# ruc98/Distributed-Data-Parallel-ML-Training

Hardware: AMD Instinct MI355X
Metric: images/sec (whole node) VGG-11 CIFAR-10 (higher is better)
Workload: dtype bf16; 1 GPU; model=vgg11, global_batch=256, per_gpu_batch=256, parallelism=dp1, hipgraph=True, buckets=1, grad_comm=fp32, comm=inline, optimizer=SGD(lr=0.1, momentum=0.9, wd=1e-4) fused

## Files before the change

distributed-data-parallel-ml-training_amd/csrc/bind.cpp:

```cpp
#include <hip/hip_runtime.h>
#include <pybind11/pybind11.h>
#include <pybind11/stl.h>

#include <stdexcept>
#include <string>
#include <tuple>
#include <vector>

#include "runtime/comm.h"

namespace py = pybind11;
using ddp_amd::BucketSpec;
using ddp_amd::RcclComm;
using ddp_amd::Reducer;

#include "kernels/api.h"

template <typename T>
static T* P(uintptr_t v) { return reinterpret_cast<T*>(v); }
static hipStream_t S(uintptr_t v) { return reinterpret_cast<hipStream_t>(v); }
static void check(int rc, const char* what) {
  if (rc != 0) {
    std::string msg = std::string(what) + " failed: ";
    msg += (rc > 0) ? hipGetErrorString((hipError_t)rc) : "invalid arguments";
// ... 200 lines not shown
  });
  m.def("conv_dgrad", [](py::tuple g, uintptr_t dy, uintptr_t wt, uintptr_t dx, uintptr_t ws,
                         size_t ws_elems, int splits, uintptr_t st, int accumulate, py::object bn,
                         py::object bna, uintptr_t acc_dy, uintptr_t acc_mask) {
    auto c = geom(g);
    if (acc_mask) {
      check(ddp_conv_dgrad_acc(&c, P<void>(dy), P<void>(wt), P<void>(dx), P<float>(ws), ws_elems,
                               splits, P<void>(acc_dy), P<unsigned char>(acc_mask), S(st)),
            "conv_dgrad_acc");
      return false;
    }
    if (bn.is_none()) {
      check(ddp_conv_dgrad(&c, P<void>(dy), P<void>(wt), P<void>(dx), P<float>(ws), ws_elems,
                           splits, accumulate, S(st)), "conv_dgrad");
      return false;
    }
    ddp_amd::BnBwdFuse f{};
    const ddp_amd::BnBwdFuse* fp = bn_fuse(bn, &f);
    ddp_amd::BnBwdApply ap{};
    const ddp_amd::BnBwdApply* app = bn_apply(bna, &ap);
    int done = 0;
    check(ddp_conv_dgrad_bn(&c, P<void>(dy), P<void>(wt), P<void>(dx), P<float>(ws), ws_elems,
                            splits, fp, app, &done, S(st)), "conv_dgrad_bn");
    return done == 1;
  }, py::arg("g"), py::arg("dy"), py::arg("wt"), py::arg("dx"), py::arg("ws"),
     py::arg("ws_elems"), py::arg("splits"), py::arg("stream"), py::arg("accumulate") = 0,
     py::arg("bn") = py::none(), py::arg("bna") = py::none(), py::arg("acc_dy") = 0,
     py::arg("acc_mask") = 0);
  m.def("conv_bwd_pair", [](py::tuple g, uintptr_t dy, uintptr_t wc, uintptr_t dx, uintptr_t x,
                            uintptr_t dw, uintptr_t ws, size_t ws_elems, uintptr_t st,
                            py::object bn, py::object bna) {
    auto c = geom(g);
    ddp_amd::BnBwdApply ap{};
    const ddp_amd::BnBwdApply* app = bn_apply(bna, &ap);
    int done = 0;
    ddp_amd::BnBwdFuse f{};
    const ddp_amd::BnBwdFuse* fp = bn_fuse(bn, &f);
    check(ddp_conv_bwd_pair(&c, P<void>(dy), P<void>(wc), P<void>(dx), P<void>(x), P<float>(dw),
                            P<float>(ws), ws_elems, fp, app, &done, S(st)), "conv_bwd_pair");
    return done;
  }, py::arg("g"), py::arg("dy"), py::arg("wc"), py::arg("dx"), py::arg("x"), py::arg("dw"),
     py::arg("ws"), py::arg("ws_elems"), py::arg("stream"), py::arg("bn") = py::none(),
     py::arg("bna") = py::none());
  m.def("sgd_fuse_register", [](uintptr_t dw, uintptr_t p, uintptr_t buf, uintptr_t wc, float lr,
                                float momentum, float wd, float grad_scale, int nesterov,
                                int clear, uintptr_t sched) {
    ddp_amd::SgdFuse f{P<float>(p), P<float>(buf), P<unsigned short>(wc), lr, momentum, wd,
                       grad_scale, nesterov, P<const ddp_amd::LrSched>(sched)};
    ddp_sgd_fuse_register(P<float>(dw), dw ? &f : nullptr, clear);
  }, py::arg("dw"), py::arg("p") = 0, py::arg("buf") = 0, py::arg("wc") = 0, py::arg("lr") = 0.f,
     py::arg("momentum") = 0.f, py::arg("wd") = 0.f, py::arg("grad_scale") = 1.f,
     py::arg("nesterov") = 0, py::arg("clear") = 0, py::arg("sched") = 0);
  m.def("sgd_fuse_begin", []() { ddp_sgd_fuse_begin(); });
  m.def("sgd_fuse_taken", []() {
    std::vector<uintptr_t> v(256);
    int n = ddp_sgd_fuse_taken(v.data(), (int)v.size());
    if (n > (int)v.size()) {
      v.resize(n);
      n = ddp_sgd_fuse_taken(v.data(), n);
    }
    v.resize(n);
    return v;
  });
  m.def("sgd_fuse_taken_master", []() {
    std::vector<uintptr_t> v(256);
    int n = ddp_sgd_fuse_taken_master(v.data(), (int)v.size());
    if (n > (int)v.size()) {
      v.resize(n);
      n = ddp_sgd_fuse_taken_master(v.data(), n);
    }
    v.resize(n);
    return v;
  });
  m.def("conv_dense2x2_set", [](int on) { ddp_conv_dense2x2_set(on); });
  m.def("conv_dense2x2_ok", [](py::tuple g) {
    auto c = geom(g);
    return ddp_conv_dense2x2_ok(&c) != 0;
  });
  m.def("conv_pair_mode", [](int mode, int items) { ddp_conv_pair_mode(mode, items); },
        py::arg("mode"), py::arg("items") = 0);
  m.def("conv_pair_force", [](int sd, int sw, int tile) { ddp_conv_pair_force(sd, sw, tile); },
        py::arg("splits_dg"), py::arg("splits_wg"), py::arg("tile") = 0);
  m.def("conv_wgrad", [](py::tuple g, uintptr_t dy, uintptr_t x, uintptr_t dw, uintptr_t ws,
                         size_t ws_elems, int splits, uintptr_t st, int final_) {
    auto c = geom(g);
    if (final_)
      check(ddp_conv_wgrad_final(&c, P<void>(dy), P<void>(x), P<float>(dw), P<float>(ws),
                                 ws_elems, splits, S(st)), "conv_wgrad");
    else
      check(ddp_conv_wgrad(&c, P<void>(dy), P<void>(x), P<float>(dw), P<float>(ws), ws_elems,
                           splits, S(st)), "conv_wgrad");
  }, py::arg("g"), py::arg("dy"), py::arg("x"), py::arg("dw"), py::arg("ws"), py::arg("ws_elems"),
     py::arg("splits"), py::arg("stream"), py::arg("final") = 0);

  m.def("bn_act_fwd", [](int N, int H, int W, int C, int pool, int relu, float eps, uintptr_t z,
                         uintptr_t res, uintptr_t stats, uintptr_t gamma, uintptr_t beta,
                         uintptr_t out, uintptr_t st, uintptr_t running_mean,
                         uintptr_t running_var, float momentum, int use_running, uintptr_t coef,
                         uintptr_t mask, uintptr_t rstats, uintptr_t rgamma, uintptr_t rbeta,
                         uintptr_t rcoef, uintptr_t rrunning_mean, uintptr_t rrunning_var,
                         float reps, float rmomentum) {
    ddp_amd::BnArgs a{};
    a.coef = P<float>(coef);
    a.mask = P<unsigned char>(mask);
    a.N = N; a.H = H; a.W = W; a.C = C; a.pool = pool; a.relu = relu; a.eps = eps;
    a.z = P<unsigned short>(z); a.res = P<unsigned short>(res); a.stats = P<float>(stats);
// ... 127 lines not shown
                         int dlogits_bf16, uintptr_t st) {
    check(ddp_softmax_ce(P<void>(logits), bf16, P<long long>(labels), B, J, P<float>(loss_sum),
                         P<int>(correct), P<void>(dlogits), dlogits_bf16, S(st)), "softmax_ce");
  });

  m.def("sgd", [](uintptr_t p, uintptr_t g, uintptr_t buf, size_t n, float lr, float momentum,
                  float wd, float grad_scale, int nesterov, uintptr_t st, uintptr_t sched) {
    check(ddp_sgd(P<float>(p), P<float>(g), P<float>(buf), n, lr, momentum, wd, grad_scale,
                  nesterov, P<const ddp_amd::LrSched>(sched), S(st)), "sgd");
  }, py::arg("p"), py::arg("g"), py::arg("buf"), py::arg("n"), py::arg("lr"), py::arg("momentum"),
     py::arg("wd"), py::arg("grad_scale"), py::arg("nesterov"), py::arg("stream"),
     py::arg("sched") = 0);
  m.def("conv_options", [](int stages) { ddp_conv_options(stages); }, py::arg("stages") = 2);
  m.def("conv_tune_set", [](int mode, int M, int N, int K, int tile, int splits, int stages) {
    ddp_conv_tune_set(mode, M, N, K, tile, splits, stages);
  }, py::arg("mode"), py::arg("M"), py::arg("N"), py::arg("K"), py::arg("tile"),
     py::arg("splits"), py::arg("stages") = 0);
  m.def("conv_tune_clear", []() { ddp_conv_tune_clear(); });
  m.def("conv_wgrad_pm_set", [](int on) { ddp_conv_wgrad_pm_set(on); });
  m.def("conv_rows_pm_set", [](int on) { ddp_conv_rows_pm_set(on); });
  m.def("bn_fold_bwd_mb", [](int mb) { ddp_bn_fold_bwd_mb(mb); });
  m.def("bn_fold_grid", [](int blocks) { ddp_bn_fold_grid(blocks); });
  m.def("conv_pair_tune_set", [](int M, int N, int K, int hw, int tile, int sd, int sw) {
    ddp_conv_pair_tune_set(M, N, K, hw, tile, sd, sw);
  });
  m.def("conv_force_tile", [](int t, int stages) { ddp_conv_force_tile(t, stages); },
        py::arg("tile_plus_one"), py::arg("stages") = 0);
#ifdef DDP_CONV_STAMPS
  m.def("conv_stamps_set", [](uintptr_t buf, int cap) { ddp_conv_stamps_set(P<void>(buf), cap); });
#endif
  m.def("pack_conv_weights", [](std::vector<std::tuple<uintptr_t, uintptr_t, uintptr_t, int, int,
                                                       int, int, int, int>> descs, uintptr_t st) {
    std::vector<ddp_amd::PackDesc> d;
    for (auto& t : descs) {
      ddp_amd::PackDesc x;
      x.p = P<float>(std::get<0>(t));
      x.wc = P<unsigned short>(std::get<1>(t));
      x.wt = P<unsigned short>(std::get<2>(t));
      x.K = std::get<3>(t); x.Cr = std::get<4>(t); x.C = std::get<5>(t);
      x.R = std::get<6>(t); x.S = std::get<7>(t);
      x.krsc = std::get<8>(t);
      d.push_back(x);
    }
    check(ddp_pack_conv_weights(d.data(), (int)d.size(), S(st)), "pack_conv_weights");
  });
  m.def("sgd_pack", [](uintptr_t items, int n_items, uintptr_t descs, uintptr_t p, uintptr_t g,
                       uintptr_t buf, float lr, float momentum, float wd, float grad_scale,
                       int nesterov, uintptr_t st, int zero_grad, uintptr_t counter, int delta,
                       uintptr_t skip, uintptr_t shadow, uintptr_t slot, uintptr_t done,
                       uintptr_t signal, uintptr_t sched, int sched_advance, uintptr_t lars_side,
                       uintptr_t lars_tensors, uintptr_t lars_partial, uintptr_t lars_trust,
                       float lars_eta, float lars_eps, uintptr_t clip_partial, int clip_chunks,
                       float clip_max_norm, float clip_eps, int clip_flags,
                       uintptr_t clip_stats) {
    check(ddp_sgd_pack(P<void>(items), n_items, P<long long>(descs), P<float>(p), P<float>(g),
                       P<float>(buf), lr, momentum, wd, grad_scale, nesterov, zero_grad,
                       P<int>(counter), delta, P<const unsigned>(skip), P<unsigned short>(shadow),
                       P<float>(slot), P<unsigned>(done), P<unsigned>(signal),
                       P<ddp_amd::LrSched>(sched), sched_advance, P<void>(lars_side),
                       P<void>(lars_tensors), P<void>(lars_partial), P<float>(lars_trust),
                       lars_eta, lars_eps, P<const float>(clip_partial), clip_chunks,
                       clip_max_norm, clip_eps, clip_flags, P<float>(clip_stats), S(st)),
          "sgd_pack");
  }, py::arg("items"), py::arg("n_items"), py::arg("descs"), py::arg("p"), py::arg("g"),
     py::arg("buf"), py::arg("lr"), py::arg("momentum"), py::arg("wd"), py::arg("grad_scale"),
     py::arg("nesterov"), py::arg("stream"), py::arg("zero_grad") = 0, py::arg("counter") = 0,
     py::arg("delta") = 0, py::arg("skip") = 0, py::arg("shadow") = 0, py::arg("slot") = 0,
     py::arg("done") = 0, py::arg("signal") = 0, py::arg("sched") = 0,
     py::arg("sched_advance") = 0, py::arg("lars_side") = 0, py::arg("lars_tensors") = 0,
     py::arg("lars_partial") = 0, py::arg("lars_trust") = 0, py::arg("lars_eta") = 0.f,
     py::arg("lars_eps") = 0.f, py::arg("clip_partial") = 0, py::arg("clip_chunks") = 0,
     py::arg("clip_max_norm") = 0.f, py::arg("clip_eps") = 0.f, py::arg("clip_flags") = 0,
     py::arg("clip_stats") = 0);
  m.def("grad_sumsq", [](uintptr_t items, int n_items, uintptr_t g, float grad_scale,
                         uintptr_t partial, uintptr_t st) {
    check(ddp_grad_sumsq(P<void>(items), n_items, P<float>(g), grad_scale, P<float>(partial),
                         S(st)), "grad_sumsq");
  }, py::arg("items"), py::arg("n_items"), py::arg("grad"), py::arg("grad_scale"),
     py::arg("partial"), py::arg("stream"));
  m.def("lars_norms", [](uintptr_t items, int n_items, uintptr_t p, uintptr_t g, float grad_scale,
                         uintptr_t partial, uintptr_t st) {
    check(ddp_lars_norms(P<void>(items), n_items, P<float>(p), P<float>(g), grad_scale,
                         P<void>(partial), S(st)), "lars_norms");
  }, py::arg("items"), py::arg("n_items"), py::arg("p"), py::arg("g"), py::arg("grad_scale"),
     py::arg("partial"), py::arg("stream"));
  m.def("shard_tail", [](uintptr_t segs, int n_segs, uintptr_t src, uintptr_t dst,
                         std::vector<std::tuple<uintptr_t, uintptr_t, uintptr_t, int, int, int,
                                                int, int, int>> descs,
                         uintptr_t done, uintptr_t signal, uintptr_t skip, uintptr_t st) {
    std::vector<ddp_amd::PackDesc> d;
    for (auto& t : descs) {
      ddp_amd::PackDesc x;
      x.p = P<float>(std::get<0>(t));
      x.wc = P<unsigned short>(std::get<1>(t));
      x.wt = P<unsigned short>(std::get<2>(t));
      x.K = std::get<3>(t); x.Cr = std::get<4>(t); x.C = std::get<5>(t);
      x.R = std::get<6>(t); x.S = std::get<7>(t);
      x.krsc = std::get<8>(t);
      d.push_back(x);
    }
    check(ddp_shard_tail(P<void>(segs), n_segs, P<float>(src), P<float>(dst), d.data(),
                         (int)d.size(), P<unsigned>(done), P<unsigned>(signal),
                         P<const unsigned>(skip), S(st)), "shard_tail");
  });
  m.def("seg_copy_f32", [](uintptr_t table, int n, uintptr_t src, uintptr_t dst, uintptr_t st) {
    check(ddp_seg_copy_f32(P<void>(table), n, P<float>(src), P<float>(dst), S(st)), "seg_copy_f32");
  });
  m.def("sgd_tile_dims", [](int RS) {
    int tk, tc;
    ddp_sgd_tile_dims(RS, &tk, &tc);
    return std::make_pair(tk, tc);
  });
  m.def("sgd_tile_limit", []() { return ddp_sgd_tile_limit(); });
  m.def("counter_add", [](uintptr_t c, int delta, uintptr_t st, uintptr_t sched, int sched_mode) {
    check(ddp_counter_add(P<int>(c), delta, P<ddp_amd::LrSched>(sched), sched_mode, S(st)),
          "counter_add");
  }, py::arg("c"), py::arg("delta"), py::arg("stream"), py::arg("sched") = 0,
     py::arg("sched_mode") = 0);

  m.def("synth_generate", [](uintptr_t images, uintptr_t labels, int n, int pix_per_img,
                             unsigned int seed, int classes, uintptr_t st) {
    check(ddp_synth_generate(P<unsigned char>(images), P<int>(labels), n, pix_per_img, seed,
                             classes, S(st)), "synth_generate");
  });
  m.def("augment", [](uintptr_t images, uintptr_t labels, uintptr_t indices, uintptr_t cursor,
                      int L, int B, int H, int W, int Cp, int pad, int flip, unsigned int seed,
// ... 173 lines not shown
```

distributed-data-parallel-ml-training_amd/csrc/kernels/api.h:

```cpp
#pragma once
#include <hip/hip_runtime.h>
#include <stddef.h>
#include <stdint.h>

namespace ddp_amd {

#ifdef DDP_AMD_DETERMINISTIC
constexpr int kStatRep = 4096;
constexpr bool kDeterministic = true;
#else
constexpr int kStatRep = 16;
constexpr bool kDeterministic = false;
#endif

struct ConvGeom {
  int N, H, W, C;
  int K;
  int R, S, stride, pad;
  int P, Q;
  int Creal;
  int wkrsc;
};

struct BnArgs {
// ... 158 lines not shown
int ddp_conv_tr_would_serve(const ddp_amd::ConvGeom* g, size_t ws_elems, int in_mode);
void ddp_conv_tr_set(int mode, int M, int K, int C, int H, int bm, int bn, int splits, int stages);
int ddp_conv_tr_geometry(int BM, int N, int H, int W, int* out7);
int ddp_linear_head_bwd_bn(const float* dl, const float* W, const void* x, int B, int F, int J,
                           const float* gscale, const ddp_amd::BnBwdFuse* bn,
                           const ddp_amd::BnBwdApply* ba, float* dW, float* db, hipStream_t st);
void ddp_conv_bn_fuse_rows(int rows);
int ddp_conv_dgrad(const ddp_amd::ConvGeom* g, const void* dy, const void* wt, void* dx,
                   float* ws, size_t ws_elems, int splits, int accumulate, hipStream_t st);
int ddp_conv_dgrad_acc(const ddp_amd::ConvGeom* g, const void* dy, const void* wt, void* dx,
                       float* ws, size_t ws_elems, int splits, const void* acc_dy,
                       const unsigned char* acc_mask, hipStream_t st);
int ddp_conv_dgrad_bn(const ddp_amd::ConvGeom* g, const void* dy, const void* wt, void* dx,
                      float* ws, size_t ws_elems, int splits, const ddp_amd::BnBwdFuse* bn,
                      const ddp_amd::BnBwdApply* ba, int* bn_done, hipStream_t st);
int ddp_conv_wgrad(const ddp_amd::ConvGeom* g, const void* dy, const void* x, float* dw,
                   float* ws, size_t ws_elems, int splits, hipStream_t st);
int ddp_bn_act_fwd(const ddp_amd::BnArgs* a, hipStream_t st);
int ddp_bn_act_bwd(const ddp_amd::BnArgs* a, hipStream_t st);
int ddp_bn_act_fwd_res(const ddp_amd::BnArgs* a, const ddp_amd::BnArgs* r, hipStream_t st);
int ddp_bn_act_bwd_res(const ddp_amd::BnArgs* a, hipStream_t st);
int ddp_bn_bwd_local_ok(int N, int H, int W, int C, int pool);
void ddp_bn_bwd_local_set(long long max_loads);
int ddp_bn_pool_linear_ce_fwd(const ddp_amd::HeadBnIn* bn, const float* W, const float* b,
                              const long long* labels, int B, int F, int J, float* dlogits,
                              float* loss_sum, int* correct, float* loss_acc, hipStream_t st);
int ddp_linear_ce_fwd(const void* x, const float* W, const float* b, const long long* labels,
                      int B, int F, int J, float* logits, float* dlogits, float* loss_sum,
                      int* correct, float* loss_acc, hipStream_t st);
int ddp_linear_bwd(const float* dlogits, const void* x, const float* W, int B, int F, int J,
                   const float* gscale, void* dx, float* dW, float* db, hipStream_t st);
int ddp_softmax_ce(const void* logits, int logits_bf16, const long long* labels, int B, int J,
                   float* loss_sum, int* correct, void* dlogits, int dlogits_bf16,
                   hipStream_t st);
int ddp_sgd(float* p, const float* g, float* buf, size_t n, float lr, float momentum, float wd,
            float grad_scale, int nesterov, const ddp_amd::LrSched* sched, hipStream_t st);
int ddp_conv_fwd_smallk(const ddp_amd::ConvGeom* g, const void* x, const void* wc,
                        const float* bias, void* y, float* stats, hipStream_t st);
void ddp_conv_options(int stages);
void ddp_conv_epi_stage_set(int on);
int ddp_bn_pool3_fwd(const ddp_amd::BnArgs* a, unsigned char* idx, hipStream_t st);
int ddp_bn_pool3_bwd(const ddp_amd::BnArgs* a, const unsigned char* idx, hipStream_t st);
void ddp_conv_pair_mode(int mode, int items);
void ddp_sgd_fuse_register(float* dw, const ddp_amd::SgdFuse* f, int clear);
void ddp_sgd_fuse_begin();
int ddp_l0_ok(const ddp_amd::ConvGeom* g);
int ddp_l0_fwd(const ddp_amd::ConvGeom* g, const ddp_amd::L0Io* io, hipStream_t st);
int ddp_l0_bwd(const ddp_amd::ConvGeom* g, const ddp_amd::L0Io* io, hipStream_t st);
int ddp_conv_wgrad_final(const ddp_amd::ConvGeom* g, const void* dy, const void* x, float* dw,
                         float* ws, size_t ws_elems, int splits, hipStream_t st);
int ddp_sgd_fuse_taken(uintptr_t* out, int cap);
int ddp_sgd_fuse_take_final(const float* dw, ddp_amd::SgdFuse* out);
int ddp_sgd_fuse_taken_master(uintptr_t* out, int cap);
void ddp_conv_pair_force(int splits_dg, int splits_wg, int tile);
int ddp_conv_bwd_pair(const ddp_amd::ConvGeom* g, const void* dy, const void* wc, void* dx,
                      const void* x, float* dw, float* ws, size_t ws_elems,
                      const ddp_amd::BnBwdFuse* bn, const ddp_amd::BnBwdApply* ba, int* bn_done,
                      hipStream_t st);
void ddp_conv_tune_set(int mode, int M, int N, int K, int tile, int splits, int stages);
void ddp_conv_pair_tune_set(int M, int N, int K, int hw, int tile, int sd, int sw);
void ddp_conv_wgrad_pm_set(int on);
void ddp_conv_rows_pm_set(int on);
void ddp_bn_fold_bwd_mb(int mb);
void ddp_bn_fold_grid(int blocks);
int ddp_conv_dense2x2_ok(const ddp_amd::ConvGeom* g);
void ddp_conv_dense2x2_set(int on);
void ddp_conv_tune_clear();
void ddp_conv_force_tile(int tile_plus_one, int stages);
#ifdef DDP_CONV_STAMPS
void ddp_conv_stamps_set(void* buf, int cap);
#endif
int ddp_pack_conv_weights(const ddp_amd::PackDesc* descs, int n, hipStream_t st);
int ddp_sgd_pack(const void* items, int n_items, const long long* descs, float* p, float* g,
                 float* buf, float lr, float momentum, float wd, float grad_scale, int nesterov,
                 int zero_grad, int* counter, int delta, const unsigned* skip,
                 unsigned short* shadow, float* slot, unsigned* done, unsigned* signal,
                 ddp_amd::LrSched* sched, int sched_advance, const void* lars_side,
                 const void* lars_tensors, const void* lars_partial, float* lars_trust,
                 float lars_eta, float lars_eps, const float* clip_partial, int clip_chunks,
                 float clip_max_norm, float clip_eps, int clip_flags, float* clip_stats,
                 hipStream_t st);
int ddp_grad_sumsq(const void* items, int n_items, const float* g, float grad_scale,
                   float* partial, hipStream_t st);
int ddp_lars_norms(const void* items, int n_items, const float* p, const float* g,
                   float grad_scale, void* partial, hipStream_t st);
int ddp_shard_tail(const void* segs, int n_segs, const float* src, float* dst,
                   const ddp_amd::PackDesc* pack, int n_pack, unsigned* done, unsigned* signal,
                   const unsigned* skip, hipStream_t st);
void ddp_sgd_tile_dims(int RS, int* TK, int* TC);
int ddp_sgd_tile_limit();
int ddp_counter_add(int* c, int delta, ddp_amd::LrSched* sched, int sched_mode, hipStream_t st);
int ddp_synth_generate(unsigned char* images, int* labels, int n, int pix_per_img,
                       unsigned int seed, int classes, hipStream_t st);
int ddp_augment(const ddp_amd::AugArgs* a, hipStream_t st);
int ddp_nchw_to_nhwc(const float* x, int N, int C, int H, int W, int Cp, void* out,
                     hipStream_t st);
int ddp_maxpool_fwd(const void* x, int N, int H, int W, int C, int KH, int KW, int stride,
                    int pad, int Ho, int Wo, void* y, void* idx, hipStream_t st);
int ddp_maxpool_bwd(const void* dy, const void* idx, int N, int H, int W, int C, int KH, int KW,
                    int stride, int pad, int Ho, int Wo, void* dx, hipStream_t st);
int ddp_avgpool_fwd(const void* x, int N, int HW, int C, void* y, hipStream_t st);
int ddp_avgpool_bwd(const void* dy, int N, int HW, int C, void* dx, hipStream_t st);
int ddp_colsum(const void* dl, int B, int J, float* db, hipStream_t st);
int ddp_mean_ws(const float* in, size_t n, int ws, float* out, hipStream_t st);
int ddp_scale(float* x, size_t n, float s, hipStream_t st);
int ddp_copy_bytes(void* dst, const void* src, size_t n, hipStream_t st);
int ddp_fill_bytes(void* dst, int value, size_t n, hipStream_t st);
int ddp_comm_standin(float* x, size_t n, int blocks, float usec, float scale, int passes,
                     hipStream_t st);
int ddp_flag_signal(unsigned* flag, hipStream_t st);
int ddp_flag_wait(const unsigned* flag, unsigned* expected, unsigned* err, float timeout_s,
                  hipStream_t st);
int ddp_pack_bf16(const float* x, size_t n, unsigned short* y, hipStream_t st);
int ddp_seg_copy_f32(const void* table, int n, const float* src, float* dst, hipStream_t st);
int ddp_unpack_bf16(const unsigned short* y, size_t n, float* x, hipStream_t st);
}
```

distributed-data-parallel-ml-training_amd/csrc/kernels/bn_act.hip:

```cpp
#include "common.h"
#include "api.h"

#include <algorithm>
#include <cstdio>
#include <cstdlib>

namespace ddp_amd {

enum { kSc = 0, kSh = 1, kMu = 2, kIs = 3, kK1 = 4, kK2 = 5 };

__device__ __forceinline__ void ld8f(const float* p, float* v) {
  const float4 a = reinterpret_cast<const float4*>(p)[0];
  const float4 b = reinterpret_cast<const float4*>(p)[1];
  v[0] = a.x; v[1] = a.y; v[2] = a.z; v[3] = a.w;
  v[4] = b.x; v[5] = b.y; v[6] = b.z; v[7] = b.w;
}

__device__ __forceinline__ void finalize_fwd_ch(const BnArgs& a, int c) {
  float mu, is;
  if (a.use_running) {
    mu = a.running_mean[c];
    is = rsqrtf(a.running_var[c] + a.eps);
  } else {
    const float M = (float)a.N * a.H * a.W;
    float s1 = 0.f, s2 = 0.f;
#pragma unroll
    for (int r = 0; r < kStatRep; ++r) {
      s1 += a.stats[r * 2 * a.C + c];
      s2 += a.stats[r * 2 * a.C + a.C + c];
    }
    mu = s1 / M;
    const float var = fmaxf(s2 / M - mu * mu, 0.f);
    is = rsqrtf(var + a.eps);
    if (a.running_mean) {
      const float unbiased = M > 1.f ? var * M / (M - 1.f) : var;
      a.running_mean[c] = (1.f - a.momentum) * a.running_mean[c] + a.momentum * mu;
      a.running_var[c] = (1.f - a.momentum) * a.running_var[c] + a.momentum * unbiased;
    }
  }
  const float sc = a.gamma[c] * is;
  a.coef[kSc * a.C + c] = sc;
  a.coef[kSh * a.C + c] = a.beta[c] - mu * sc;
  a.coef[kMu * a.C + c] = mu;
  a.coef[kIs * a.C + c] = is;
}

__global__ __launch_bounds__(256) void bn_finalize_fwd_kernel(BnArgs a) {
  const int c = blockIdx.x * blockDim.x + threadIdx.x;
  if (c < a.C) finalize_fwd_ch(a, c);
}

__global__ __launch_bounds__(256) void bn_finalize_fwd2_kernel(BnArgs a, BnArgs r) {
  const int c = blockIdx.x * blockDim.x + threadIdx.x;
  if (c < a.C) finalize_fwd_ch(blockIdx.y ? r : a, c);
// ... 182 lines not shown
    const size_t pp = L.ok[it] ? p : 0;
    L.mb[it] = 0;
    const int wo = (int)(pp % Wo);
    const int ho = (int)((pp / Wo) % Ho);
    const int n = (int)(pp / ((size_t)Wo * Ho));
    L.dv[it] = ld8(a.dout + pp * a.C + cg * 8);
#pragma unroll
    for (int d = 0; d < NP; ++d) {
      const int h = POOL ? 2 * ho + (d >> 1) : ho, w = POOL ? 2 * wo + (d & 1) : wo;
      const size_t off = (((size_t)n * a.H + h) * a.W + w) * a.C + cg * 8;
      L.off[it][d] = off;
      L.zv[it][d] = ld8(a.z + off);
      if (MASK) L.mb[it] = a.mask[off / 8];
      if (RBN || (!MASK && !POOL && a.res)) L.rv[it][POOL ? 0 : d] = ld8(a.res + off);
    }
  }
}

template <bool POOL, bool MASK = false>
__device__ __forceinline__ void bwd_compute(const BnArgs& a, const u16x8& dv, const u16x8* zv,
                                            const u16x8* rv, unsigned mb, const float* sc,
                                            const float* sh, const float* mu, const float* is,
                                            float (*xh)[8], float (*dyb)[8]) {
  constexpr int NP = POOL ? 4 : 1;
  float best[8], yv[NP][8];
  int arg[8];
#pragma unroll
  for (int e = 0; e < 8; ++e) { best[e] = -INFINITY; arg[e] = 0; }
#pragma unroll
  for (int d = 0; d < NP; ++d) {
#pragma unroll
    for (int e = 0; e < 8; ++e) {
      const float zf = bf2f(zv[d][e]);
      float y = zf * sc[e] + sh[e];
      if (!POOL && !MASK && a.res) y += bf2f(rv[POOL ? 0 : d][e]);
      xh[d][e] = (zf - mu[e]) * is[e];
      yv[d][e] = y;
      if (POOL) {
        const float yr = a.relu ? fmaxf(y, 0.f) : y;
        if (yr > best[e] || yr != yr) { best[e] = yr; arg[e] = d; }
      }
    }
  }
#pragma unroll
  for (int d = 0; d < NP; ++d)
#pragma unroll
    for (int e = 0; e < 8; ++e) {
      const float g = (!POOL || arg[e] == d) ? bf2f(dv[e]) : 0.f;
      const bool pos = MASK ? ((mb >> e) & 1u) != 0 : yv[d][e] > 0.f;
      dyb[d][e] = (a.relu && !pos) ? 0.f : g;
    }
}

template <bool POOL, int IPT, bool MASK = false, bool STRIDE = false, bool RBN = false>
__global__ __launch_bounds__(256) void bn_act_bwd_reduce_kernel(BnArgs a) {
  constexpr int NS = RBN ? 3 : 2;
  constexpr int NP = POOL ? 4 : 1;
  __shared__ float red[8 * 256];
  DDP_DEVICE_CHECK(a.C % 8 == 0 && (!POOL || (a.H % 2 == 0 && a.W % 2 == 0)));
  const int G = a.C / 8;
  const int Gb = a.red_gb ? a.red_gb : (G < 256 ? G : 256);
  const int Ho = POOL ? a.H / 2 : a.H, Wo = POOL ? a.W / 2 : a.W;
  const size_t npix = (size_t)a.N * Ho * Wo;
  const int cg_base = blockIdx.y * Gb;
  const int cgl = threadIdx.x % Gb;
  const int prow = threadIdx.x / Gb, prows = 256 / Gb;
  const int c0 = (cg_base + cgl) * 8;
  const size_t per_blk = (size_t)prows * IPT;
  const size_t nbx = STRIDE ? (npix + per_blk - 1) / per_blk : (size_t)blockIdx.x + 1;
  BwdItems<POOL, IPT> L;
  bwd_load<POOL, IPT, MASK, RBN>(a, L, (size_t)blockIdx.x * per_blk + prow, prows, npix,
                                 cg_base + cgl, Ho, Wo);
  float sc[8], sh[8], mu[8], is[8], rmu[8], ris[8];
  ld8f(a.coef + kSc * a.C + c0, sc);
  ld8f(a.coef + kSh * a.C + c0, sh);
  ld8f(a.coef + kMu * a.C + c0, mu);
  ld8f(a.coef + kIs * a.C + c0, is);
  if (RBN) {
    ld8f(a.rcoef + kMu * a.C + c0, rmu);
    ld8f(a.rcoef + kIs * a.C + c0, ris);
  }
  float acc[NS][8];
#pragma unroll
  for (int k = 0; k < NS; ++k)
#pragma unroll
    for (int e = 0; e < 8; ++e) acc[k][e] = 0.f;
  for (size_t bb = blockIdx.x;;) {
#pragma unroll
    for (int it = 0; it < IPT; ++it) {
      if (!L.ok[it]) continue;
      float xh[NP][8], dyb[NP][8];
      bwd_compute<POOL, MASK>(a, L.dv[it], L.zv[it], L.rv[it], L.mb[it], sc, sh, mu, is, xh, dyb);
#pragma unroll
      for (int d = 0; d < NP; ++d) {
#pragma unroll
        for (int e = 0; e < 8; ++e) {
          acc[0][e] += dyb[d][e];
          acc[1][e] += dyb[d][e] * xh[d][e];
          if (RBN) acc[NS - 1][e] += dyb[d][e] * ((bf2f(L.rv[it][0][e]) - rmu[e]) * ris[e]);
        }
      }
    }
    bb += gridDim.x;
    if (!STRIDE || bb >= nbx) break;
    bwd_load<POOL, IPT, MASK, RBN>(a, L, bb * per_blk + prow, prows, npix, cg_base + cgl, Ho, Wo);
  }
  float* rep = a.sums + stat_rep(blockIdx.x) * 2 * a.C;
  const int tid = threadIdx.x;
#pragma unroll
  for (int k = 0; k < NS; ++k) {
    if (k) __syncthreads();
#pragma unroll
    for (int e = 0; e < 8; ++e) red[e * 256 + tid] = acc[k][e];
    __syncthreads();
    float* dst = k < 2 ? rep + k * a.C : a.rsums + stat_rep(blockIdx.x) * 2 * a.C + a.C;
    for (int idx = tid; idx < Gb * 8; idx += 256) {
      const int g = idx / 8, e = idx % 8;
      float s = 0.f;
      for (int r = 0; r < prows; ++r) s += red[e * 256 + r * Gb + g];
      atomicAdd(dst + (cg_base + g) * 8 + e, stat_val(s, blockIdx.x));
    }
  }
}

template <bool POOL, int IPT, bool FOLD = false, bool MASK = false, bool STRIDE = false,
          bool RBN = false>
__global__ __launch_bounds__(256) void bn_act_bwd_apply_kernel(BnArgs a) {
  constexpr int NP = POOL ? 4 : 1;
  const int G = a.C / 8;
  const int Gb = G < 256 ? G : 256;
  const int Ho = POOL ? a.H / 2 : a.H, Wo = POOL ? a.W / 2 : a.W;
  const size_t npix = (size_t)a.N * Ho * Wo;
  const int cg_base = blockIdx.y * Gb;
  const int cgl = threadIdx.x % Gb;
  const int prow = threadIdx.x / Gb, prows = 256 / Gb;
  const int c0 = (cg_base + cgl) * 8;
  const size_t per_blk = (size_t)prows * IPT;
  const size_t nbx = (npix + per_blk - 1) / per_blk;
  BwdItems<POOL, IPT> L;
  bwd_load<POOL, IPT, MASK, RBN>(a, L, (size_t)blockIdx.x * per_blk + prow, prows, npix,
                                 cg_base + cgl, Ho, Wo);
  float sc[8], sh[8], mu[8], is[8], k1[8], k2[8], rsc[8], rmu[8], ris[8], rk2[8];
  if (RBN) {
    ld8f(a.rcoef + kSc * a.C + c0, rsc);
    ld8f(a.rcoef + kMu * a.C + c0, rmu);
    ld8f(a.rcoef + kIs * a.C + c0, ris);
    ld8f(a.rcoef + kK2 * a.C + c0, rk2);
  }
  ld8f(a.coef + kSc * a.C + c0, sc);
  ld8f(a.coef + kSh * a.C + c0, sh);
  ld8f(a.coef + kMu * a.C + c0, mu);
  ld8f(a.coef + kIs * a.C + c0, is);
  if (FOLD) {
    __shared__ __attribute__((aligned(16))) float kk[2][2048];
    const int nch = Gb * 8;
    const float inv_m = 1.f / ((float)a.N * a.H * a.W);
    for (int q = threadIdx.x * 4; q < 2 * nch; q += 1024) {
      const int which = q / nch, cl = q - which * nch;
      const float* src = a.sums + which * a.C + cg_base * 8 + cl;
      float4 t = *reinterpret_cast<const float4*>(src);
#pragma unroll
      for (int r = 1; r < kStatRep; ++r) {
        const float4 v = *reinterpret_cast<const float4*>(src + (size_t)r * 2 * a.C);
        t.x += v.x; t.y += v.y; t.z += v.z; t.w += v.w;
      }
      const float tv[4] = {t.x, t.y, t.z, t.w};
#pragma unroll
      for (int e = 0; e < 4; ++e) {
        kk[which][cl + e] = tv[e] * inv_m;
        if (blockIdx.x == 0) {
          const int c = cg_base * 8 + cl + e;
          a.coef[(which ? kK2 : kK1) * a.C + c] = tv[e] * inv_m;
          float* dst = which ? a.dgamma : a.dbeta;
          if (dst) dst[c] += tv[e];
        }
      }
    }
    __syncthreads();
#pragma unroll
    for (int e = 0; e < 8; ++e) {
      k1[e] = kk[0][cgl * 8 + e];
      k2[e] = kk[1][cgl * 8 + e];
    }
  } else {
    ld8f(a.coef + kK1 * a.C + c0, k1);
    ld8f(a.coef + kK2 * a.C + c0, k2);
  }
  for (size_t bb = blockIdx.x;;) {
#pragma unroll
    for (int it = 0; it < IPT; ++it) {
      if (!L.ok[it]) continue;
      float xh[NP][8], dyb[NP][8];
      bwd_compute<POOL, MASK>(a, L.dv[it], L.zv[it], L.rv[it], L.mb[it], sc, sh, mu, is, xh, dyb);
#pragma unroll
      for (int d = 0; d < NP; ++d) {
        u16x8 o, r;
#pragma unroll
        for (int e = 0; e < 8; ++e) {
          o[e] = f2bf(sc[e] * (dyb[d][e] - k1[e] - xh[d][e] * k2[e]));
          if (RBN) {
            const float xr = (bf2f(L.rv[it][0][e]) - rmu[e]) * ris[e];
            r[e] = f2bf(rsc[e] * (dyb[d][e] - k1[e] - xr * rk2[e]));
          } else {
            r[e] = f2bf(dyb[d][e]);
          }
        }
        st8(a.dz + L.off[it][d], o);
        if (RBN) st8(a.rdz + L.off[it][d], r);
        else if (a.dres) st8(a.dres + L.off[it][d], r);
      }
    }
    bb += gridDim.x;
    if (!STRIDE || bb >= nbx) break;
    bwd_load<POOL, IPT, MASK, RBN>(a, L, bb * per_blk + prow, prows, npix, cg_base + cgl, Ho, Wo);
  }
}

template <bool POOL, int IPT, int NT, bool MASK = false>
__global__ __launch_bounds__(NT) void bn_act_bwd_local_kernel(BnArgs a) {
  constexpr int NP = POOL ? 4 : 1;
  constexpr int NW = NT / kWave;
  __shared__ float red[NW][16];
  __shared__ float fin[16];
  const int cg = blockIdx.x;
  const int c0 = cg * 8;
  const int Ho = POOL ? a.H / 2 : a.H, Wo = POOL ? a.W / 2 : a.W;
  const size_t npix = (size_t)a.N * Ho * Wo;
  BwdItems<POOL, IPT> L;
  bwd_load<POOL, IPT, MASK>(a, L, threadIdx.x, NT, npix, cg, Ho, Wo);
  float sc[8], sh[8], mu[8], is[8];
  ld8f(a.coef + kSc * a.C + c0, sc);
  ld8f(a.coef + kSh * a.C + c0, sh);
  ld8f(a.coef + kMu * a.C + c0, mu);
  ld8f(a.coef + kIs * a.C + c0, is);
  float s1[8], s2[8];
#pragma unroll
  for (int e = 0; e < 8; ++e) { s1[e] = 0.f; s2[e] = 0.f; }
#pragma unroll
  for (int it = 0; it < IPT; ++it) {
    if (!L.ok[it]) continue;
    float xh[NP][8], dyb[NP][8];
    bwd_compute<POOL, MASK>(a, L.dv[it], L.zv[it], L.rv[it], L.mb[it], sc, sh, mu, is, xh, dyb);
#pragma unroll
    for (int d = 0; d < NP; ++d)
#pragma unroll
      for (int e = 0; e < 8; ++e) {
        s1[e] += dyb[d][e];
        s2[e] += dyb[d][e] * xh[d][e];
      }
  }
  const int wave = threadIdx.x / kWave, lane = threadIdx.x % kWave;
#pragma unroll
  for (int e = 0; e < 8; ++e) {
    const float t1 = wave_sum(s1[e]), t2 = wave_sum(s2[e]);
    if (lane == 0) { red[wave][e] = t1; red[wave][8 + e] = t2; }
  }
  __syncthreads();
  if (threadIdx.x < 16) {
    float t = 0.f;
#pragma unroll
    for (int w = 0; w < NW; ++w) t += red[w][threadIdx.x];
    fin[threadIdx.x] = t;
    const int e = threadIdx.x & 7;
    const float inv_m = 1.f / ((float)a.N * a.H * a.W);
    if (threadIdx.x < 8) {
      a.coef[kK1 * a.C + c0 + e] = t * inv_m;
      if (a.dbeta) a.dbeta[c0 + e] += t;
    } else {
      a.coef[kK2 * a.C + c0 + e] = t * inv_m;
      if (a.dgamma) a.dgamma[c0 + e] += t;
    }
  }
  __syncthreads();
  const float inv_m = 1.f / ((float)a.N * a.H * a.W);
  float k1[8], k2[8];
#pragma unroll
  for (int e = 0; e < 8; ++e) { k1[e] = fin[e] * inv_m; k2[e] = fin[8 + e] * inv_m; }
// ... 260 lines not shown
}

extern "C" int ddp_bn_act_fwd(const BnArgs* args, hipStream_t st) {
  BnArgs a = *args;
  a.rcoef = nullptr;
  if (a.C % 8 || a.coef == nullptr) return -1;
  if (a.pool && (a.res || a.mask)) return -1;
  const int Ho = a.pool ? a.H / 2 : a.H, Wo = a.pool ? a.W / 2 : a.W;
  const size_t items = (size_t)a.N * Ho * Wo * (a.C / 8);
  if (a.pool) {
    if (items >= 256 * 2048) launch_fwd<true, 2>(a, items, st);
    else launch_fwd<true, 1>(a, items, st);
  } else {
    if (items >= 256 * 4096) launch_fwd<false, 4>(a, items, st);
    else launch_fwd<false, 1>(a, items, st);
  }
  return (int)hipGetLastError();
}

static size_t kBwdBlocks = 1024;

static size_t g_fold_bwd_mb = 32;
static size_t fold_bwd_bytes() { return g_fold_bwd_mb << 20; }
extern "C" void ddp_bn_fold_bwd_mb(int mb) { g_fold_bwd_mb = (size_t)(mb < 0 ? 0 : mb); }

static unsigned kReduceGrid = 2048;

static int kReduceGb = 32;
static void reduce_split(const BnArgs& a, int Gb, int chunks, int* rGb, int* rchunks) {
  const int G = a.C / 8;
  *rGb = Gb;
  *rchunks = chunks;
  if (kReduceGb > 0 && Gb > kReduceGb && 256 % kReduceGb == 0 && G % kReduceGb == 0) {
    *rGb = kReduceGb;
    *rchunks = G / kReduceGb;
  }
}

static unsigned reduce_grid_x(unsigned bx, int chunks) {
  unsigned rx = kReduceGrid ? std::min(bx, std::max(1u, kReduceGrid / (unsigned)chunks)) : bx;
  if (kDeterministic) rx = std::min(rx, std::max(1u, (unsigned)kStatRep / (unsigned)chunks));
  return rx;
}

template <int IPT>
static void launch_bwd_res(const BnArgs& a, size_t npix, int Gb, int chunks, hipStream_t st) {
  const unsigned bx = blocks_for(npix, (size_t)(256 / Gb) * IPT);
  BnArgs ra = a;
  int rGb, rch;
  reduce_split(a, Gb, chunks, &rGb, &rch);
  ra.red_gb = rGb;
  const unsigned rbx = blocks_for(npix, (size_t)(256 / rGb) * IPT);
  const unsigned rx = reduce_grid_x(rbx, rch);
  if (rx < rbx)
    hipLaunchKernelGGL((bn_act_bwd_reduce_kernel<false, IPT, true, true, true>), dim3(rx, rch),
                       dim3(256), 0, st, ra);
  else
    hipLaunchKernelGGL((bn_act_bwd_reduce_kernel<false, IPT, true, false, true>), dim3(rbx, rch),
                       dim3(256), 0, st, ra);
  hipLaunchKernelGGL(bn_finalize_bwd_res_kernel, dim3(blocks_for(a.C, 256)), dim3(256), 0, st, a);
  hipLaunchKernelGGL((bn_act_bwd_apply_kernel<false, IPT, false, true, false, true>),
                     dim3(bx, chunks), dim3(256), 0, st, a);
}

template <bool POOL, int IPT, bool MASK>
static void launch_bwd_m(const BnArgs& a, size_t npix, int Gb, int chunks, hipStream_t st) {
  const unsigned bx = blocks_for(npix, (size_t)(256 / Gb) * IPT);
  if (!a.sums_ready) {
    BnArgs ra = a;
    int rGb, rch;
    reduce_split(a, Gb, chunks, &rGb, &rch);
    ra.red_gb = rGb;
    const unsigned rbx = blocks_for(npix, (size_t)(256 / rGb) * IPT);
    const unsigned rx = reduce_grid_x(rbx, rch);
    if (rx < rbx)
      hipLaunchKernelGGL((bn_act_bwd_reduce_kernel<POOL, IPT, MASK, true>), dim3(rx, rch),
                         dim3(256), 0, st, ra);
    else
      hipLaunchKernelGGL((bn_act_bwd_reduce_kernel<POOL, IPT, MASK, false>), dim3(rbx, rch),
                         dim3(256), 0, st, ra);
  }
  const size_t per_block = (size_t)kStatRep * 2 * (size_t)Gb * 8 * sizeof(float);
  const size_t fold_bytes = (size_t)bx * chunks * per_block;
  if (!kDeterministic && fold_bwd_bytes() > 0 && fold_bytes <= fold_bwd_bytes()) {
    hipLaunchKernelGGL((bn_act_bwd_apply_kernel<POOL, IPT, true, MASK, false>), dim3(bx, chunks),
                       dim3(256), 0, st, a);
    return;
  }
  const unsigned cx = std::min(bx, fold_fwd_grid() / (unsigned)chunks);
  if (!kDeterministic && fold_bwd_bytes() > 0 && cx * chunks >= 1024 &&
      (size_t)cx * chunks * per_block <= kFoldGridBytes) {
    hipLaunchKernelGGL((bn_act_bwd_apply_kernel<POOL, IPT, true, MASK, true>), dim3(cx, chunks),
                       dim3(256), 0, st, a);
    return;
  }
  hipLaunchKernelGGL(bn_finalize_bwd_kernel, dim3(blocks_for(a.C, 256)), dim3(256), 0, st, a);
  hipLaunchKernelGGL((bn_act_bwd_apply_kernel<POOL, IPT, false, MASK, false>), dim3(bx, chunks),
                     dim3(256), 0, st, a);
}

template <bool POOL, int IPT>
static void launch_bwd(const BnArgs& a, size_t npix, int Gb, int chunks, hipStream_t st) {
  if constexpr (!POOL) {
    if (a.rcoef) return launch_bwd_res<IPT>(a, npix, Gb, chunks, st);
    if (a.mask) return launch_bwd_m<POOL, IPT, true>(a, npix, Gb, chunks, st);
  }
  launch_bwd_m<POOL, IPT, false>(a, npix, Gb, chunks, st);
}

static int kLocalMaxLoads = 8;
constexpr int kLocalThreads = 256;
static bool local_cfg(const BnArgs& a, int* ipt) {
  if (a.C % 8 || (a.pool && a.res)) return false;
  const int Ho = a.pool ? a.H / 2 : a.H, Wo = a.pool ? a.W / 2 : a.W;
  const size_t npix = (size_t)a.N * Ho * Wo;
  const int per_item = 1 + (a.pool ? 4 : 1) + (a.res ? 1 : 0);
  for (int i = 1; i <= 8; i *= 2) {
    if ((size_t)kLocalThreads * i < npix) continue;
    if (a.pool && i > 4) return false;
    if (i * per_item > kLocalMaxLoads) return false;
    *ipt = i;
    return true;
  }
  return false;
}

template <bool POOL, bool MASK>
static void launch_local_m(const BnArgs& a, int ipt, hipStream_t st) {
  const dim3 grid(a.C / 8), block(kLocalThreads);
  if (ipt == 1) hipLaunchKernelGGL((bn_act_bwd_local_kernel<POOL, 1, kLocalThreads, MASK>), grid, block, 0, st, a);
  else if (ipt == 2) hipLaunchKernelGGL((bn_act_bwd_local_kernel<POOL, 2, kLocalThreads, MASK>), grid, block, 0, st, a);
  else if (ipt == 4) hipLaunchKernelGGL((bn_act_bwd_local_kernel<POOL, 4, kLocalThreads, MASK>), grid, block, 0, st, a);
  else if constexpr (!POOL) hipLaunchKernelGGL((bn_act_bwd_local_kernel<POOL, 8, kLocalThreads, MASK>), grid, block, 0, st, a);
}

template <bool POOL>
static void launch_local(const BnArgs& a, int ipt, hipStream_t st) {
  if constexpr (!POOL) {
    if (a.mask) return launch_local_m<POOL, true>(a, ipt, st);
  }
  launch_local_m<POOL, false>(a, ipt, st);
}

extern "C" void ddp_bn_bwd_local_set(long long max_loads) {
  BnArgs a{};
  int ipt;
  (void)local_cfg(a, &ipt);
  kLocalMaxLoads = (int)std::max(0LL, max_loads);
}

extern "C" int ddp_bn_bwd_local_ok(int N, int H, int W, int C, int pool) {
  BnArgs a{};
  a.N = N; a.H = H; a.W = W; a.C = C; a.pool = pool;
  int ipt;
  return local_cfg(a, &ipt) ? 1 : 0;
}

static int launch_reduce_chain(const BnArgs& a, hipStream_t st) {
  const int G = a.C / 8;
  const int Gb = G < 256 ? G : 256;
  if ((Gb < 256 && 256 % Gb) || (G > 256 && G % 256)) return -1;
  const int chunks = (G + Gb - 1) / Gb;
  const int Ho = a.pool ? a.H / 2 : a.H, Wo = a.pool ? a.W / 2 : a.W;
  const size_t npix = (size_t)a.N * Ho * Wo;
  const size_t per1 = (size_t)(256 / Gb);
  const size_t blocks1 = (npix + per1 - 1) / per1 * chunks;
  int ipt = 1;
  if (blocks1 > 2 * kBwdBlocks)
    while (ipt < 4 && blocks1 / ipt > kBwdBlocks) ipt *= 2;
  if (a.pool) {
    if (ipt >= 4) launch_bwd<true, 4>(a, npix, Gb, chunks, st);
    else if (ipt == 2) launch_bwd<true, 2>(a, npix, Gb, chunks, st);
    else launch_bwd<true, 1>(a, npix, Gb, chunks, st);
  } else {
    if (ipt >= 4) launch_bwd<false, 4>(a, npix, Gb, chunks, st);
    else if (ipt == 2) launch_bwd<false, 2>(a, npix, Gb, chunks, st);
    else launch_bwd<false, 1>(a, npix, Gb, chunks, st);
  }
  return (int)hipGetLastError();
}

extern "C" int ddp_bn_act_bwd_res(const BnArgs* args, hipStream_t st) {
  const BnArgs a = *args;
  if (!res_shape_ok(a) || a.mask == nullptr || a.sums == nullptr || a.rsums == nullptr ||
      a.dz == nullptr || a.rdz == nullptr || a.sums_ready)
    return -1;
// ... 59 lines not shown
```

distributed-data-parallel-ml-training_amd/csrc/kernels/conv_igemm.hip:

```cpp
#include "common.h"
#include "api.h"
#include "linear_blocks.h"
#include <algorithm>
#include <map>
#include <set>
#include <cstdlib>

namespace ddp_amd {

enum { MODE_FWD = 0, MODE_DGRAD = 1, MODE_WGRAD = 2 };

typedef short v4i16 __attribute__((ext_vector_type(4)));
typedef short short8_t __attribute__((ext_vector_type(8)));
typedef __attribute__((address_space(3))) v4i16 lds_v4i16;

__global__ __launch_bounds__(256) void zero16_kernel(uint4* __restrict__ p, size_t n16) {
  for (size_t i = blockIdx.x * 256ull + threadIdx.x; i < n16; i += (size_t)gridDim.x * 256)
    p[i] = (uint4){0u, 0u, 0u, 0u};
}

__device__ __forceinline__ void ld8f_conv(const float* p, float* v) {
  const float4 a = reinterpret_cast<const float4*>(p)[0];
  const float4 b = reinterpret_cast<const float4*>(p)[1];
  v[0] = a.x; v[1] = a.y; v[2] = a.z; v[3] = a.w;
  v[4] = b.x; v[5] = b.y; v[6] = b.z; v[7] = b.w;
}

struct ConvArgs {
  ConvGeom g;
  const unsigned short* a;
  const unsigned short* b;
  unsigned short* out;
  float* dw;
  float* ws;
  const float* bias;
  float* stats;
  int Mg, Ng, Kg;
  int splits;
  int ksteps_per_split;
  int phase;
  int pa, pb, Hp, Wp, r0, s0, Rt, St, qa, qb;
  int accumulate;
  int a_bytes, b_bytes;
  FastDiv dPQ, dQ;
  int has_bnf;
  BnBwdFuse bnf;
  const BnFwdFuse* bnfwd;
  int* bnfwd_done;
  const BnBwdApply* bnapply;
  int* bnapply_done;
  int epi_stage;
  int d2x2;
  int d2C, d2K;
  int no_finish;
  const unsigned short* acc_dy;
// ... 981 lines not shown
    const unsigned long long st2 = stamp_now();
#endif
    epilogue(row0, col0, zsplit, args.splits > 1);
#ifdef DDP_CONV_STAMPS
    stamp_put(args.stamps, (unsigned)MODE, st0, st1, st2, stamp_now());
#endif
    if (item + nblk < nitems) wait_dma_barrier<0>();
  }
  if constexpr (XSTAT) {
    if (MODE == MODE_FWD && run_col >= 0)
      flush_stats(run_col, *reinterpret_cast<float(*)[8]>(run_s),
                  *reinterpret_cast<float(*)[8]>(run_ss));
  }
}

#ifndef DDP_CONV_WAVES_PER_EU
#define DDP_CONV_WAVES_PER_EU 2
#endif
template <int MODE, int BM, int BN, int NST, int BNF = 0, bool XSTAT = false>
__global__ __launch_bounds__(256) __attribute__((amdgpu_waves_per_eu(DDP_CONV_WAVES_PER_EU)))
void conv_igemm_kernel(ConvArgs args) {
  extern __shared__ __attribute__((aligned(16))) unsigned short smem[];
  conv_igemm_body<MODE, BM, BN, NST, BNF, XSTAT>(args, smem, blockIdx.x, gridDim.x);
}

template <int MODE, int BM, int BN, int NST>
__global__ __launch_bounds__(256) __attribute__((amdgpu_waves_per_eu(2)))
void conv_igemm_bnf2_kernel(ConvArgs args) {
  extern __shared__ __attribute__((aligned(16))) unsigned short smem[];
  conv_igemm_body<MODE, BM, BN, NST, 2>(args, smem, blockIdx.x, gridDim.x);
}

template <int BM, int BN, int NST, int BNF, bool SGDM = false>
__global__ __launch_bounds__(256) void conv_bwd_pair_kernel(ConvArgs dg, ConvArgs wg, int n_dg) {
  __shared__ __attribute__((aligned(16))) unsigned short smem[ConvSmem<BM, BN, NST>::elems];
  if ((int)blockIdx.x < n_dg)
    conv_igemm_body<MODE_DGRAD, BM, BN, NST, BNF>(dg, smem, blockIdx.x, n_dg);
  else
    conv_igemm_body<MODE_WGRAD, BM, BN, NST, 0, false, SGDM>(wg, smem, blockIdx.x - n_dg,
                                                           gridDim.x - n_dg);
}
struct RowMap {
  int stride, Hp, Wp, H, W, pa, pb;
};

__device__ __forceinline__ size_t map_row(const RowMap& m, int row) {
  if (m.stride == 0) return row;
  const int hw = m.Hp * m.Wp;
  const int n = row / hw, rem = row - n * hw;
  const int i = rem / m.Wp, j = rem - i * m.Wp;
  return ((size_t)n * m.H + m.pa + m.stride * i) * m.W + m.pb + m.stride * j;
}

constexpr int kSlabBatch = 8;
__device__ __forceinline__ void sum_slabs8(const float* p, size_t slab, int z0, int z1, float* v) {
  for (int zb = z0; zb < z1; zb += kSlabBatch) {
    float4 a[kSlabBatch], b[kSlabBatch];
#pragma unroll
    for (int u = 0; u < kSlabBatch; ++u) {
      if (zb + u < z1) {
        const float4* src = reinterpret_cast<const float4*>(p + (size_t)(zb + u) * slab);
        a[u] = src[0];
        b[u] = src[1];
      }
    }
#pragma unroll
    for (int u = 0; u < kSlabBatch; ++u) {
      if (zb + u < z1) {
        v[0] += a[u].x; v[1] += a[u].y; v[2] += a[u].z; v[3] += a[u].w;
        v[4] += b[u].x; v[5] += b[u].y; v[6] += b[u].z; v[7] += b[u].w;
      }
    }
  }
}

struct FinishArgs {
  const float* ws;
  int splits;
  unsigned short* out;
  const float* bias;
  float* stats;
  int Mg, Ng;
  RowMap rmap;
  int accumulate;
  BnBwdFuse bnf;
  int H, W;
  const unsigned short* acc_dy;
  const unsigned char* acc_mask;
};

template <bool BNF>
__device__ __forceinline__ void splitk_finish_body(const FinishArgs& fa, float* red_, int bx,
                                                   int by, int gx) {
  const float* ws = fa.ws;
  const int splits = fa.splits, Mg = fa.Mg, Ng = fa.Ng, accumulate = fa.accumulate;
  const int H = fa.H, W = fa.W;
  unsigned short* out = fa.out;
  const float* bias = fa.bias;
  float* stats = fa.stats;
  const RowMap rmap = fa.rmap;
  const BnBwdFuse& bnf = fa.bnf;
  float (*red)[8][256] = reinterpret_cast<float (*)[8][256]>(red_);
  constexpr bool has_bnf = BNF;
  const int G = Ng / 8;
  const int Gb = G < 256 ? G : 256;
  const int cgl = threadIdx.x % Gb, prow = threadIdx.x / Gb, prows = 256 / Gb;
  const int cg = by * Gb + cgl;
// ... 414 lines not shown
    for (int j = 0; j < 16; ++j) {
      if (j < J) {
        const float d = dl[(size_t)row * J + j] * g;
#pragma unroll
        for (int e = 0; e < 8; ++e) v[r][e] += d * w[j][e];
      }
    }
  }
  bnbwd_from_dx<RPT, true>(bn, ba, B, F, 1, 1, v, wred, half, lane, c0);
}

template <int RPT>
__global__ __launch_bounds__(256) void linear_head_bwd_kernel(const float* __restrict__ dl,
                                                              const float* __restrict__ Wt,
                                                              const unsigned short* __restrict__ x,
                                                              int B, int F, int J,
                                                              const float* gscale, BnBwdFuse bn,
                                                              BnBwdApply ba, float* dW, float* db,
                                                              int ndx, int nfx) {
  if ((int)blockIdx.x < ndx) {
    linear_dx_bnbwd_body<RPT>(dl, Wt, B, F, J, gscale, bn, ba, blockIdx.x);
  } else {
    const int t = blockIdx.x - ndx;
    linear_dw_block(dl, x, B, F, J, gscale, dW, db, t % nfx, t / nfx);
  }
}

constexpr int kWgFinishGroup = kDeterministic ? (1 << 30) : 32;
__global__ __launch_bounds__(256) void wgrad_finish_kernel(const float* ws, int splits, int K,
                                                           int R, int S, int C, int Creal,
                                                           float* dw) {
  extern __shared__ __attribute__((aligned(16))) float row[];
  const int k = blockIdx.x;
  const int RS = R * S, RSC = RS * C;
  const size_t slab = (size_t)K * RSC;
  const int z0 = blockIdx.y * kWgFinishGroup, z1 = min(splits, z0 + kWgFinishGroup);
  for (int j = threadIdx.x; j < RSC; j += blockDim.x) {
    float v = 0.f;
    for (int z = z0; z < z1; ++z) v += ws[z * slab + (size_t)k * RSC + j];
    row[j] = v;
  }
  __syncthreads();
  float* out = dw + (size_t)k * Creal * RS;
  const bool single = gridDim.y == 1;
  for (int c = threadIdx.x; c < Creal; c += blockDim.x) {
    for (int rs = 0; rs < RS; ++rs) {
      const float v = row[rs * C + c];
      if (single) out[c * RS + rs] += v;
      else atomicAdd(out + c * RS + rs, v);
    }
  }
}

__device__ __forceinline__ float sgd_step1(float p, float g, float& b, const SgdFuse& h,
                                           float lr) {
  return sgd_update1(p, g, b, lr, h.momentum, h.wd, h.grad_scale, h.nesterov);
}

constexpr int kWgFinishGroupKrsc = kDeterministic ? (1 << 30) : 16;
__device__ __forceinline__ void wgrad_finish_krsc_body(const float* __restrict__ ws, int splits,
                                                       int K, int RS, int C, int Creal,
                                                       float* __restrict__ dw, int bx, int by,
                                                       int gx, int gy, const SgdFuse& sg) {
  const size_t slab = (size_t)K * RS * C;
  const size_t n4 = slab / 4;
  const int z0 = by * kWgFinishGroupKrsc, z1 = min(splits, z0 + kWgFinishGroupKrsc);
  const bool single = gy == 1;
  const bool opt = single && sg.p != nullptr;
  const float lr = opt ? sched_lr_block(sg.sched, sg.lr) : sg.lr;
  for (size_t i = bx * (size_t)blockDim.x + threadIdx.x; i < n4;
       i += (size_t)gx * blockDim.x) {
    float4 v = reinterpret_cast<const float4*>(ws + z0 * slab)[i];
    for (int zb = z0 + 1; zb < z1; zb += kSlabBatch) {
      float4 a[kSlabBatch];
#pragma unroll
      for (int u = 0; u < kSlabBatch; ++u)
        if (zb + u < z1) a[u] = reinterpret_cast<const float4*>(ws + (size_t)(zb + u) * slab)[i];
#pragma unroll
      for (int u = 0; u < kSlabBatch; ++u)
        if (zb + u < z1) { v.x += a[u].x; v.y += a[u].y; v.z += a[u].z; v.w += a[u].w; }
    }
    const float vv[4] = {v.x, v.y, v.z, v.w};
    if (opt) {
      if (Creal == C) {
        float4 pv = reinterpret_cast<float4*>(sg.p)[i];
        float4 bv = reinterpret_cast<float4*>(sg.buf)[i];
        pv.x = sgd_step1(pv.x, v.x, bv.x, sg, lr);
        pv.y = sgd_step1(pv.y, v.y, bv.y, sg, lr);
        pv.z = sgd_step1(pv.z, v.z, bv.z, sg, lr);
        pv.w = sgd_step1(pv.w, v.w, bv.w, sg, lr);
        reinterpret_cast<float4*>(sg.p)[i] = pv;
        reinterpret_cast<float4*>(sg.buf)[i] = bv;
        uint2 pk;
        pk.x = (unsigned)f2bf(pv.x) | ((unsigned)f2bf(pv.y) << 16);
        pk.y = (unsigned)f2bf(pv.z) | ((unsigned)f2bf(pv.w) << 16);
        *reinterpret_cast<uint2*>(sg.wc + i * 4) = pk;
      } else {
        const size_t e = i * 4;
        const int c = (int)(e % C);
        const size_t krs = e / C;
#pragma unroll
        for (int t = 0; t < 4; ++t) {
          if (c + t >= Creal) continue;
          const size_t mi = krs * Creal + c + t;
          float b = sg.buf[mi];
          const float np = sgd_step1(sg.p[mi], vv[t], b, sg, lr);
          sg.p[mi] = np;
          sg.buf[mi] = b;
          sg.wc[e + t] = f2bf(np);
        }
      }
      continue;
    }
    if (Creal == C) {
      if (single) {
        float4* o = reinterpret_cast<float4*>(dw) + i;
        float4 d = *o;
        d.x += v.x; d.y += v.y; d.z += v.z; d.w += v.w;
        *o = d;
      } else {
#pragma unroll
        for (int t = 0; t < 4; ++t) unsafeAtomicAdd(dw + i * 4 + t, vv[t]);
      }
    } else {
      const size_t e = i * 4;
      const int c = (int)(e % C);
      const size_t krs = e / C;
#pragma unroll
      for (int t = 0; t < 4; ++t) {
        if (c + t >= Creal) continue;
        if (single) dw[krs * Creal + c + t] += vv[t];
        else unsafeAtomicAdd(dw + krs * Creal + c + t, vv[t]);
      }
    }
  }
}

__global__ __launch_bounds__(256) void wgrad_finish_krsc_kernel(const float* __restrict__ ws,
                                                                int splits, int K, int RS, int C,
                                                                int Creal, float* __restrict__ dw,
                                                                SgdFuse sg) {
  wgrad_finish_krsc_body(ws, splits, K, RS, C, Creal, dw, blockIdx.x, blockIdx.y, gridDim.x,
                         gridDim.y, sg);
}

struct WgFinishArgs {
  const float* ws;
  int splits, K, RS, C, Creal;
  float* dw;
  int gx, gy;
  SgdFuse sgd;
};

template <bool BNF>
__global__ __launch_bounds__(256) void bwd_pair_finish_kernel(FinishArgs fa, int dgx, int dgy,
                                                              WgFinishArgs wa) {
  __shared__ float red[2 * 8 * 256];
  const int b = blockIdx.x;
  if (b < dgx * dgy) {
    splitk_finish_body<BNF>(fa, red, b % dgx, b / dgx, dgx);
  } else {
    const int w = b - dgx * dgy;
    wgrad_finish_krsc_body(wa.ws, wa.splits, wa.K, wa.RS, wa.C, wa.Creal, wa.dw, w % wa.gx,
                           w / wa.gx, wa.gx, wa.gy, wa.sgd);
  }
}

}

using namespace ddp_amd;

#ifdef DDP_CONV_STAMPS
namespace ddp_amd {
ConvStampBuf g_conv_stamps{nullptr, 0};
}
extern "C" void ddp_conv_stamps_set(void* buf, int cap) {
  g_conv_stamps = ConvStampBuf{(unsigned*)buf, buf ? std::max(0, cap) : 0};
}
#endif

static bool fits_buffer(size_t elems) { return elems * 2 < (size_t)kOOB; }

static int g_stages = 2;
constexpr int kNumCUs = 256;
static int g_epi_stage = 1;
static bool epi_stage_enabled() { return g_epi_stage != 0; }
extern "C" void ddp_conv_epi_stage_set(int on) { g_epi_stage = on ? 1 : 0; }

static int pick_splits(int tiles, int ksteps, size_t slab, const ConvArgs& a, size_t ws_elems) {
  if (a.splits > 0) return std::max(1, std::min(a.splits, ksteps));

  if (a.ws == nullptr) return 1;
  int s = (512 + tiles - 1) / tiles;
  s = std::max(1, std::min(s, ksteps / 4));
  s = (int)std::min<size_t>((size_t)s, std::max<size_t>(1, ws_elems / slab));
  return s;
}

static double tile_cost(int BM, int BN, const ConvArgs& a, size_t ws_elems, int* splits_out) {
  const int tiles = ((a.Mg + BM - 1) / BM) * ((a.Ng + BN - 1) / BN);
  const int ksteps = (a.Kg + 63) / 64;
  const size_t slab = (size_t)a.Mg * a.Ng;
  const int splits = pick_splits(tiles, ksteps, slab, a, ws_elems);
  *splits_out = splits;
  const double eff = (BM == 128 && BN == 128) ? 1.0 : ((BM == 64 && BN == 64) ? 0.55 : 0.8);
// ... 115 lines not shown
    a.w_dp = wsame ? (BK / g.Q) % g.P : 0;
  }
#ifdef DDP_CONV_STAMPS
  a.stamps = g_conv_stamps;
#endif
  return tiles * splits;
}

static bool needs_finish(int mode, const ConvArgs& a) {
  (void)mode;
  return a.splits > 1;
}

static int finish_rows_per_thread(int Mg, int rows_per_block) {
  return (Mg + rows_per_block - 1) / rows_per_block <= 128 ? 1 : 2;
}

static void dg_finish_grid(const ConvArgs& a, int* bx_out, int* chunks_out) {
  const int G = a.Ng / 8;
  const int Gb = G < 256 ? G : 256;
  const int chunks = (G + Gb - 1) / Gb;
  const int rows_per_block = std::max(1, 256 / Gb);
  const int rpt = finish_rows_per_thread(a.Mg, rows_per_block);
  int bx = (a.Mg + rows_per_block * rpt - 1) / (rows_per_block * rpt);
  *bx_out = std::max(1, std::min(bx, 2048 / chunks + 1));
  *chunks_out = chunks;
}

static FinishArgs finish_args(int mode, const ConvArgs& a) {
  RowMap rm{0, 0, 0, 0, 0, 0, 0};
  if (a.phase) rm = RowMap{a.g.stride, a.Hp, a.Wp, a.g.H, a.g.W, a.pa, a.pb};
  const bool fwd = mode == MODE_FWD;
  return FinishArgs{a.ws, a.splits, a.out, fwd ? a.bias : nullptr, fwd ? a.stats : nullptr,
                    a.Mg, a.Ng, rm, a.accumulate, a.bnf, a.g.H, a.g.W, a.acc_dy, a.acc_mask};
}

static std::map<const float*, SgdFuse> g_sgd_reg;
static std::set<const float*> g_sgd_taken;
static std::set<const float*> g_sgd_master;
static SgdFuse sgd_fuse_master(const float* dw) {
  if (g_sgd_reg.empty()) return SgdFuse{};
  auto it = g_sgd_reg.find(dw);
  if (it == g_sgd_reg.end()) return SgdFuse{};
  g_sgd_master.insert(dw);
  return it->second;
}
static bool g_sgd_allow = false;
static SgdFuse sgd_fuse_for(const float* dw, int groups) {
  if (!g_sgd_allow || groups != 1 || g_sgd_reg.empty()) return SgdFuse{};
  auto it = g_sgd_reg.find(dw);
  if (it == g_sgd_reg.end()) return SgdFuse{};
  g_sgd_taken.insert(dw);
  return it->second;
}

static WgFinishArgs wg_finish_args(const ConvArgs& a) {
  const size_t n4 = (size_t)a.Mg * a.Ng / 4;
  const int groups = (a.splits + kWgFinishGroupKrsc - 1) / kWgFinishGroupKrsc;
  const int bx = (int)std::min<size_t>((n4 + 255) / 256, std::max(1, 2048 / groups));
  return WgFinishArgs{a.ws, a.splits, a.g.K, a.g.R * a.g.S, a.g.C, a.g.Creal, a.dw, bx, groups,
                      sgd_fuse_for(a.dw, groups)};
}

static int g_bn_fuse_rows = 128;
static int bn_fuse_max_rows() { return g_bn_fuse_rows; }
static int bn_bwd_fuse_max_rows() { return bn_fuse_max_rows(); }

static bool bnbwd_fusable(const ConvArgs& a) {
  return a.has_bnf && a.bnapply && a.splits > 1 && !a.phase && !a.accumulate &&
         a.Mg <= bn_bwd_fuse_max_rows() && a.Mg <= kBnBwdFuseMaxRows && a.Ng % 16 == 0 &&
         a.g.stride == 1 &&
         (!a.bnf.pool || (a.bnf.Hz == 2 * a.g.H && a.bnf.Wz == 2 * a.g.W)) &&
         (a.bnf.pool || (a.bnf.Hz == a.g.H && a.bnf.Wz == a.g.W));
}

template <int RPT, bool POOL>
__global__ __launch_bounds__(256) void bwd_pair_finish_bnbwd_kernel(FinishArgs fa, BnBwdApply ba,
                                                                    int dgx, WgFinishArgs wa) {
  __shared__ float wred[4][2][8];
  const int b = blockIdx.x;
  if (b < dgx) {
    finish_bnbwd_body<RPT, POOL>(fa, ba, wred, b);
  } else {
    const int w = b - dgx;
    wgrad_finish_krsc_body(wa.ws, wa.splits, wa.K, wa.RS, wa.C, wa.Creal, wa.dw, w % wa.gx,
                           w / wa.gx, wa.gx, wa.gy, wa.sgd);
  }
}

template <int RPT, bool POOL>
static void launch_bnbwd_t(const FinishArgs& fa, const BnBwdApply& ba, int dgx,
                           const WgFinishArgs* wa, hipStream_t st) {
  if (wa)
    hipLaunchKernelGGL((bwd_pair_finish_bnbwd_kernel<RPT, POOL>), dim3(dgx + wa->gx * wa->gy),
                       dim3(256), 0, st, fa, ba, dgx, *wa);
  else
    hipLaunchKernelGGL((splitk_finish_bnbwd_kernel<RPT, POOL>), dim3(dgx), dim3(256), 0, st, fa, ba);
}

static bool launch_finish_bnbwd(const ConvArgs& a, hipStream_t st, const WgFinishArgs* wa) {
  if (!bnbwd_fusable(a)) return false;
  const FinishArgs fa = finish_args(MODE_DGRAD, a);
  const BnBwdApply& ba = *a.bnapply;
  const int dgx = a.Ng / 16, rpt = (a.Mg + 127) / 128;
  if (a.bnf.pool) {
    if (rpt <= 1) launch_bnbwd_t<1, true>(fa, ba, dgx, wa, st);
    else if (rpt <= 2) launch_bnbwd_t<2, true>(fa, ba, dgx, wa, st);
    else launch_bnbwd_t<4, true>(fa, ba, dgx, wa, st);
  } else {
    if (rpt <= 1) launch_bnbwd_t<1, false>(fa, ba, dgx, wa, st);
    else if (rpt <= 2) launch_bnbwd_t<2, false>(fa, ba, dgx, wa, st);
    else launch_bnbwd_t<4, false>(fa, ba, dgx, wa, st);
  }
  if (a.bnapply_done) *a.bnapply_done = 1;
  return true;
}

static bool launch_finish_bnfwd(const ConvArgs& a, hipStream_t st) {
  const BnFwdFuse& bf = *a.bnfwd;
  if (a.Mg > kBnFwdFuseMaxRows || a.Mg > bn_fuse_max_rows() || a.Ng % 16 || a.accumulate ||
      a.phase)
    return false;
  if (bf.P * bf.Q <= 0 || a.Mg % (bf.P * bf.Q)) return false;
  if (bf.pool && (bf.P % 2 || bf.Q % 2)) return false;
  const FinishArgs fa = finish_args(MODE_FWD, a);
  const dim3 grid(a.Ng / 16);
  const size_t lds = bf.pool ? (size_t)a.Mg * 16 * sizeof(float) : 0;
  static const bool attr = [] {
    (void)hipFuncSetAttribute(reinterpret_cast<const void*>(splitk_finish_bnfwd_kernel<8>),
                              hipFuncAttributeMaxDynamicSharedMemorySize,
                              kBnFwdFuseMaxRows * 16 * sizeof(float));
    return true;
  }();
  (void)attr;
  const int rpt = (a.Mg + 127) / 128;
  if (rpt <= 1) hipLaunchKernelGGL(splitk_finish_bnfwd_kernel<1>, grid, dim3(256), lds, st, fa, bf);
  else if (rpt <= 2) hipLaunchKernelGGL(splitk_finish_bnfwd_kernel<2>, grid, dim3(256), lds, st, fa, bf);
  else if (rpt <= 4) hipLaunchKernelGGL(splitk_finish_bnfwd_kernel<4>, grid, dim3(256), lds, st, fa, bf);
  else hipLaunchKernelGGL(splitk_finish_bnfwd_kernel<8>, grid, dim3(256), lds, st, fa, bf);
  if (a.bnfwd_done) *a.bnfwd_done = 1;
  return true;
}

template <int MODE>
static void launch_finish(const ConvArgs& a, hipStream_t st) {
  if (!needs_finish(MODE, a)) return;
  if (MODE == MODE_WGRAD && a.g.wkrsc) {
    const WgFinishArgs w = wg_finish_args(a);
    hipLaunchKernelGGL(wgrad_finish_krsc_kernel, dim3(w.gx, w.gy), dim3(256), 0, st, a.ws,
                       a.splits, a.g.K, a.g.R * a.g.S, a.g.C, a.g.Creal, a.dw, w.sgd);
  } else if (MODE == MODE_WGRAD) {
    const int groups = (a.splits + kWgFinishGroup - 1) / kWgFinishGroup;
    const size_t lds = sizeof(float) * a.g.R * a.g.S * a.g.C;
    hipLaunchKernelGGL(wgrad_finish_kernel, dim3(a.g.K, groups), dim3(256), lds, st, a.ws,
                       a.splits, a.g.K, a.g.R, a.g.S, a.g.C, a.g.Creal, a.dw);
  } else {
    if (MODE == MODE_FWD && a.bnfwd && launch_finish_bnfwd(a, st)) return;
    if (MODE == MODE_DGRAD && a.has_bnf && a.bnapply && launch_finish_bnbwd(a, st, nullptr)) return;
    int bx, chunks;
    dg_finish_grid(a, &bx, &chunks);
    const FinishArgs fa = finish_args(MODE, a);
    if (MODE == MODE_DGRAD && a.has_bnf)
      hipLaunchKernelGGL(splitk_finish_kernel<true>, dim3(bx, chunks), dim3(256), 0, st, fa);
    else
      hipLaunchKernelGGL(splitk_finish_kernel<false>, dim3(bx, chunks), dim3(256), 0, st, fa);
  }
}

template <int MODE, int BM, int BN>
static void launch_cfg(ConvArgs& a, int splits, hipStream_t st, int nst_req = 0) {
  const int items = prepare_cfg<MODE, BM, BN>(a, splits);
  constexpr int kStageBytes = (BM + BN) * 64 * 2;
  constexpr int kMaxStages = kStageBytes * 4 <= 163840 ? 4 : (kStageBytes * 3 <= 163840 ? 3 : 2);
  int nst = nst_req >= 2 && nst_req <= 4 ? nst_req : stages_for(BM, BN);
  nst = std::min(nst, kMaxStages);
  if constexpr (kMaxStages >= 4) {
    if (nst == 4) { launch_gemm<MODE, BM, BN, 4>(a, items, st); goto launched; }
  }
  if constexpr (kMaxStages >= 3) {
    if (nst == 3) { launch_gemm<MODE, BM, BN, 3>(a, items, st); goto launched; }
  }
  launch_gemm<MODE, BM, BN, 2>(a, items, st);
launched:
  if (!a.no_finish) launch_finish<MODE>(a, st);
}

struct TuneKey {
  int mode, M, N, K;
  int hw = 0;
  bool operator<(const TuneKey& o) const {
    if (mode != o.mode) return mode < o.mode;
    if (M != o.M) return M < o.M;
    if (N != o.N) return N < o.N;
    if (K != o.K) return K < o.K;
    return hw < o.hw;
  }
};
struct TuneVal {
  int tile, splits, stages;
};
static std::map<TuneKey, TuneVal> g_tuned;
static std::map<TuneKey, TuneVal> g_pair_tuned;
static int g_pair_force_dg = 0, g_pair_force_wg = 0;
// ... 113 lines not shown
  a.d2x2 = 1;
  a.d2C = g->C;
  a.d2K = g->K;
  a.a_bytes = (int)(2 * (size_t)g->N * a.Kg);
  a.b_bytes = (int)(2 * (size_t)g->K * 9 * g->C);
}
static int dense2x2_splits(const ConvArgs& a, size_t ws_elems) {
  const int tiles = ((a.Mg + 63) / 64) * ((a.Ng + 63) / 64), ksteps = a.Kg / 64;
  int sp = std::max(2, std::min((512 + tiles - 1) / tiles, ksteps / 4));
  const size_t slab = (size_t)a.Mg * a.Ng;
  if ((size_t)sp * slab > ws_elems) sp = (int)(ws_elems / slab);
  return sp >= 2 ? sp : 0;
}
static ConvArgs finish_view(const ConvArgs& a, const ConvGeom* g, int mode) {
  if (!a.d2x2) return a;
  ConvArgs f = a;
  f.g = *g;
  f.d2x2 = 0;
  f.Mg = g->N * g->P * g->Q;
  f.Ng = mode == MODE_FWD ? g->K : g->C;
  f.Kg = 9 * (mode == MODE_FWD ? g->C : g->K);
  return f;
}

static int conv_fwd_dense(const ConvGeom* g, const void* x, const void* wc, const float* bias,
                          void* y, float* stats, float* ws, size_t ws_elems, const BnFwdFuse* bn,
                          int* bn_done, hipStream_t st) {
  if (!ddp_conv_dense2x2_ok(g) || ws == nullptr) return -1;
  ConvArgs a{};
  dense2x2_args(a, g, MODE_FWD);
  a.a = (const unsigned short*)x;
  a.b = (const unsigned short*)wc;
  a.out = (unsigned short*)y;
  a.ws = ws;
  a.splits = dense2x2_splits(a, ws_elems);
  if (a.splits < 2) return -1;
  a.no_finish = 1;
  launch_mode<MODE_FWD>(a, ws_elems, st);
  ConvArgs f = finish_view(a, g, MODE_FWD);
  f.no_finish = 0;
  f.bias = bias;
  f.stats = stats;
  if (bn && f.Mg <= kBnFwdFuseMaxRows) {
    f.bnfwd = bn;
    f.bnfwd_done = bn_done;
  }
  launch_finish<MODE_FWD>(f, st);
  return (int)hipGetLastError();
}

extern "C" int ddp_conv_fwd(const ConvGeom* g, const void* x, const void* wc, const float* bias,
                            void* y, float* stats, float* ws, size_t ws_elems, int splits,
                            hipStream_t st) {
  if (g->C % 8 || g->K % 8) return -1;
  {
    const int r = conv_fwd_dense(g, x, wc, bias, y, stats, ws, ws_elems, nullptr, nullptr, st);
    if (r >= 0) return r;
  }
  ConvArgs a{};
  a.g = *g;
  a.a = (const unsigned short*)x;
  a.b = (const unsigned short*)wc;
  a.out = (unsigned short*)y;
  a.ws = ws;
  a.bias = bias;
  a.stats = stats;
  a.Mg = g->N * g->P * g->Q;
  a.Ng = g->K;
  a.Kg = g->R * g->S * g->C;
  a.splits = splits;
  const size_t xa = (size_t)g->N * g->H * g->W * g->C, wb = (size_t)a.Ng * a.Kg;
  if (!fits_buffer(xa) || !fits_buffer(wb) || !fits_buffer((size_t)a.Mg * a.Ng)) return -2;
  a.a_bytes = (int)(2 * xa);
  a.b_bytes = (int)(2 * wb);
  launch_mode<MODE_FWD>(a, ws_elems, st);
  return (int)hipGetLastError();
}

extern "C" int ddp_linear_head_bwd_bn(const float* dl, const float* W, const void* x, int B,
                                      int F, int J, const float* gscale, const BnBwdFuse* bn,
                                      const BnBwdApply* ba, float* dW, float* db, hipStream_t st) {
  if (!bn || !ba || !dl || !W || !x || !dW) return -1;
  if (J < 1 || J > 16 || F % 16 || B < 1 || B > 512 || !bn->pool || bn->Hz != 2 || bn->Wz != 2)
    return 0;
  const int ndx = F / 16, nfx = (F + 63) / 64, nry = (B + kDwRows - 1) / kDwRows;
  const dim3 grid(ndx + nfx * nry);
  const unsigned short* xb = (const unsigned short*)x;
  if (B <= 128) hipLaunchKernelGGL(linear_head_bwd_kernel<1>, grid, dim3(256), 0, st, dl, W, xb, B, F, J, gscale, *bn, *ba, dW, db, ndx, nfx);
  else if (B <= 256) hipLaunchKernelGGL(linear_head_bwd_kernel<2>, grid, dim3(256), 0, st, dl, W, xb, B, F, J, gscale, *bn, *ba, dW, db, ndx, nfx);
  else hipLaunchKernelGGL(linear_head_bwd_kernel<4>, grid, dim3(256), 0, st, dl, W, xb, B, F, J, gscale, *bn, *ba, dW, db, ndx, nfx);
  const int e = (int)hipGetLastError();
  return e ? 2 + e : 1;
}

extern "C" void ddp_conv_bn_fuse_rows(int rows) { g_bn_fuse_rows = std::max(0, rows); }

extern "C" int ddp_conv_fwd_bn(const ConvGeom* g, const void* x, const void* wc, const float* bias,
                               void* z, float* stats, float* ws, size_t ws_elems,
                               const BnFwdFuse* bn, hipStream_t st) {
  constexpr bool enabled = true;
  if (g->C % 8 || g->K % 8) return -1;
  int done = 0;
  {
    const int r = conv_fwd_dense(g, x, wc, bias, z, stats, ws, ws_elems, enabled ? bn : nullptr,
                                 &done, st);
    if (r > 0) return 2 + r;
    if (r == 0) return done;
  }
  ConvArgs a{};
  a.g = *g;
  a.a = (const unsigned short*)x;
  a.b = (const unsigned short*)wc;
  a.out = (unsigned short*)z;
  a.ws = ws;
  a.bias = bias;
  a.stats = stats;
  a.Mg = g->N * g->P * g->Q;
  a.Ng = g->K;
  a.Kg = g->R * g->S * g->C;
  const size_t xa = (size_t)g->N * g->H * g->W * g->C, wb = (size_t)a.Ng * a.Kg;
  if (!fits_buffer(xa) || !fits_buffer(wb) || !fits_buffer((size_t)a.Mg * a.Ng)) return -2;
  a.a_bytes = (int)(2 * xa);
  a.b_bytes = (int)(2 * wb);
  if (enabled && bn && a.Mg <= kBnFwdFuseMaxRows) {
    a.bnfwd = bn;
    a.bnfwd_done = &done;
  }
  launch_mode<MODE_FWD>(a, ws_elems, st);
  const int e = (int)hipGetLastError();
  return e ? 2 + e : done;
}

extern "C" int ddp_conv_fwd_finish(const ConvGeom* g, float* ws, int splits, const float* bias,
                                   void* z, float* stats, const BnFwdFuse* bn, int* bn_done,
                                   hipStream_t st) {
  ConvArgs a{};
  a.g = *g;
  a.out = (unsigned short*)z;
  a.ws = ws;
  a.bias = bias;
  a.stats = stats;
  a.Mg = g->N * g->P * g->Q;
  a.Ng = g->K;
  a.Kg = g->R * g->S * g->C;
  a.splits = splits;
  if (bn && a.Mg <= kBnFwdFuseMaxRows) {
    a.bnfwd = bn;
    a.bnfwd_done = bn_done;
  }
  launch_finish<MODE_FWD>(a, st);
  return (int)hipGetLastError();
}

static int conv_dgrad_impl(const ConvGeom* g, const void* dy, const void* wc, void* dx,
                           float* ws, size_t ws_elems, int splits, int accumulate,
                           const BnBwdFuse* bn, const BnBwdApply* ba, int* bn_done,
                           hipStream_t st, const void* acc_dy = nullptr,
                           const unsigned char* acc_mask = nullptr) {
  if (bn_done) *bn_done = 0;
  if (g->C % 8 || g->K % 8) return -1;
  if (bn && bn->code) return -3;
  if (bn && (accumulate || g->stride != 1)) return -3;
  if (acc_mask && (!accumulate || !acc_dy || g->stride != 1)) return -3;
  if (!accumulate && ddp_conv_dense2x2_ok(g) && ws != nullptr) {
    ConvArgs d{};
    dense2x2_args(d, g, MODE_DGRAD);
    d.a = (const unsigned short*)dy;
    d.b = (const unsigned short*)wc;
    d.out = (unsigned short*)dx;
    d.ws = ws;
    d.splits = bn ? dense2x2_splits(d, ws_elems) : splits;
    if (!bn || d.splits >= 2) {
      d.no_finish = 1;
      launch_mode<MODE_DGRAD>(d, ws_elems, st);
      if (d.splits > 1) {
        ConvArgs f = finish_view(d, g, MODE_DGRAD);
        f.no_finish = 0;
        if (bn) {
          f.has_bnf = 1;
          f.bnf = *bn;
          f.bnapply = ba;
          f.bnapply_done = bn_done;
        }
        launch_finish<MODE_DGRAD>(f, st);
      }
      return (int)hipGetLastError();
    }
  }
  ConvArgs a{};
  a.accumulate = accumulate;
  a.acc_dy = (const unsigned short*)acc_dy;
  a.acc_mask = acc_mask;
  if (bn) {
    a.has_bnf = 1;
    a.bnf = *bn;
    a.bnapply = ba;
    a.bnapply_done = bn_done;
  }
  a.g = *g;
  a.a = (const unsigned short*)dy;
  a.b = (const unsigned short*)wc;
  a.out = (unsigned short*)dx;
  a.ws = ws;
  a.Ng = g->C;
  a.splits = splits;
  const size_t dya = (size_t)g->N * g->P * g->Q * g->K, wb = (size_t)g->K * g->R * g->S * g->C;
  if (!fits_buffer(dya) || !fits_buffer(wb) || !fits_buffer((size_t)g->N * g->H * g->W * g->C))
    return -2;
  a.a_bytes = (int)(2 * dya);
  a.b_bytes = (int)(2 * wb);
  if (g->stride == 1) {
// ... 10 lines not shown
      if ((r0 >= g->R || s0 >= g->S) && pa < g->H && pb < g->W) zero_fill = true;
    }
  if (zero_fill && !accumulate) {
    const size_t n16 = (size_t)g->N * g->H * g->W * g->C / 8;
    const unsigned nb = (unsigned)std::min<size_t>((n16 + 255) / 256, 8192);
    hipLaunchKernelGGL(zero16_kernel, dim3(std::max(1u, nb)), dim3(256), 0, st,
                       reinterpret_cast<uint4*>(dx), n16);
  }
  for (int pa = 0; pa < sd; ++pa) {
    for (int pb = 0; pb < sd; ++pb) {
      ConvArgs p = a;
      p.phase = 1;
      p.pa = pa;
      p.pb = pb;
      p.r0 = (pa + g->pad) % sd;
      p.s0 = (pb + g->pad) % sd;
      p.Rt = p.r0 < g->R ? (g->R - p.r0 + sd - 1) / sd : 0;
      p.St = p.s0 < g->S ? (g->S - p.s0 + sd - 1) / sd : 0;
      p.Hp = pa < g->H ? (g->H - pa + sd - 1) / sd : 0;
      p.Wp = pb < g->W ? (g->W - pb + sd - 1) / sd : 0;
      if (p.Rt * p.St == 0 || p.Hp * p.Wp == 0) continue;
      p.qa = (pa + g->pad - p.r0) / sd;
      p.qb = (pb + g->pad - p.s0) / sd;
      p.Mg = g->N * p.Hp * p.Wp;
      p.Kg = p.Rt * p.St * g->K;
      launch_mode<MODE_DGRAD>(p, ws_elems, st);
    }
  }
  return (int)hipGetLastError();
}

extern "C" int ddp_conv_dgrad(const ConvGeom* g, const void* dy, const void* wc, void* dx,
                              float* ws, size_t ws_elems, int splits, int accumulate,
                              hipStream_t st) {
  return conv_dgrad_impl(g, dy, wc, dx, ws, ws_elems, splits, accumulate, nullptr, nullptr,
                         nullptr, st);
}

extern "C" int ddp_conv_dgrad_acc(const ConvGeom* g, const void* dy, const void* wc, void* dx,
                                  float* ws, size_t ws_elems, int splits, const void* acc_dy,
                                  const unsigned char* acc_mask, hipStream_t st) {
  return conv_dgrad_impl(g, dy, wc, dx, ws, ws_elems, splits, 1, nullptr, nullptr, nullptr, st,
                         acc_dy, acc_mask);
}

extern "C" int ddp_conv_dgrad_bn(const ConvGeom* g, const void* dy, const void* wc, void* dx,
                                 float* ws, size_t ws_elems, int splits, const BnBwdFuse* bn,
                                 const BnBwdApply* ba, int* bn_done, hipStream_t st) {
  return conv_dgrad_impl(g, dy, wc, dx, ws, ws_elems, splits, 0, bn, ba, bn_done, st);
}

extern "C" int ddp_conv_wgrad(const ConvGeom* g, const void* dy, const void* x, float* dw,
                              float* ws, size_t ws_elems, int splits, hipStream_t st) {
  if (g->C % 8 || g->K % 8) return -1;
  ConvArgs a{};
  a.g = *g;
  a.a = (const unsigned short*)dy;
  a.b = (const unsigned short*)x;
  a.dw = dw;
  a.ws = ws;
  if (g->R * g->S == 1) a.g.wkrsc = 1;
  a.Mg = g->K;
  a.Ng = g->R * g->S * g->C;
  a.Kg = g->N * g->P * g->Q;
  a.splits = splits;
  const size_t dya = (size_t)g->N * g->P * g->Q * g->K, xb = (size_t)g->N * g->H * g->W * g->C;
  if (!fits_buffer(dya) || !fits_buffer(xb)) return -2;
  a.a_bytes = (int)(2 * dya);
  a.b_bytes = (int)(2 * xb);
  a.dPQ = make_fastdiv(g->P * g->Q);
  a.dQ = make_fastdiv(g->Q);
  launch_mode<MODE_WGRAD>(a, ws_elems, st);
  return (int)hipGetLastError();
}

static int g_pair_mode = 3;
static int g_pair_items = 1024;
extern "C" void ddp_conv_pair_mode(int m, int items) {
  g_pair_mode = m;
  if (items > 0) g_pair_items = items;
}

constexpr int kPairTiles = 6;
template <int BM, int BN, int NST, bool BNF1, bool SGDM>
static void pair_kernel_launch(const ConvArgs& d, const ConvArgs& w, int itd, int itw,
                               hipStream_t st) {
  hipLaunchKernelGGL((conv_bwd_pair_kernel<BM, BN, NST, BNF1 ? 1 : 0, SGDM>), dim3(itd + itw),
                     dim3(256), 0, st, d, w, itd);
}
template <int BM, int BN, int NST>
static void pair_launch_t(ConvArgs& d, ConvArgs& w, int sd, int sw, float* ws, size_t ws_elems,
                          int* itd_out, int* itw_out, bool* ok_out, const float* dw,
                          bool launch, hipStream_t st) {
  const int itd = prepare_cfg<MODE_DGRAD, BM, BN>(d, std::max(1, sd));
  size_t dneed = needs_finish(MODE_DGRAD, d) ? (size_t)d.splits * d.Mg * d.Ng : 0;
  dneed = (dneed + 63) / 64 * 64;
  w.ws = ws + dneed;
  const int itw = prepare_cfg<MODE_WGRAD, BM, BN>(w, std::max(1, sw));
  const size_t wneed = needs_finish(MODE_WGRAD, w) ? (size_t)w.splits * w.Mg * w.Ng : 0;
  *itd_out = itd;
  *itw_out = itw;
  *ok_out = dneed + wneed <= ws_elems;
  if (!launch || !*ok_out) return;
  if (!needs_finish(MODE_WGRAD, w) && w.g.wkrsc && w.g.Creal == w.g.C) w.sgd = sgd_fuse_master(dw);
  const bool bnf1 = d.has_bnf && d.splits <= 1;
  const bool sgdm = w.sgd.p != nullptr;
  if (bnf1 && sgdm) pair_kernel_launch<BM, BN, NST, true, true>(d, w, itd, itw, st);
  else if (bnf1) pair_kernel_launch<BM, BN, NST, true, false>(d, w, itd, itw, st);
  else if (sgdm) pair_kernel_launch<BM, BN, NST, false, true>(d, w, itd, itw, st);
  else pair_kernel_launch<BM, BN, NST, false, false>(d, w, itd, itw, st);
}

extern "C" int ddp_conv_bwd_pair(const ConvGeom* g, const void* dy, const void* wc, void* dx,
                                 const void* x, float* dw, float* ws, size_t ws_elems,
                                 const BnBwdFuse* bn, const BnBwdApply* ba, int* bn_done,
                                 hipStream_t st) {
  if (bn_done) *bn_done = 0;
  if (!bn) ba = nullptr;
  auto separate = [&]() -> int {
    const BnBwdFuse* bsep = bn && bn->code ? nullptr : bn;
    const int r = conv_dgrad_impl(g, dy, wc, dx, ws, ws_elems, 0, 0, bsep, bsep ? ba : nullptr,
                                  bn_done, st);
    if (r) return r;
    g_sgd_allow = true;
    const int rw = ddp_conv_wgrad(g, dy, x, dw, ws, ws_elems, 0, st);
    g_sgd_allow = false;
    return rw;
  };
  if (g_pair_mode == 0 || g->stride != 1 || g->C % 8 || g->K % 8 || g->Creal != g->C)
    return separate();
  const size_t dya = (size_t)g->N * g->P * g->Q * g->K, wb = (size_t)g->K * g->R * g->S * g->C;
  const size_t xb = (size_t)g->N * g->H * g->W * g->C;
  if (!fits_buffer(dya) || !fits_buffer(wb) || !fits_buffer(xb)) return separate();
  ConvArgs d{};
  d.g = *g;
  if (bn) {
    d.has_bnf = 1;
    d.bnf = *bn;
    d.bnapply = ba;
    d.bnapply_done = bn_done;
  }
  d.a = (const unsigned short*)dy;
  d.b = (const unsigned short*)wc;
  d.out = (unsigned short*)dx;
  d.ws = ws;
  d.Mg = g->N * g->H * g->W;
  d.Ng = g->C;
  d.Kg = g->R * g->S * g->K;
  d.a_bytes = (int)(2 * dya);
  d.b_bytes = (int)(2 * wb);
  ConvArgs w{};
  w.g = *g;
  if (g->R * g->S == 1) w.g.wkrsc = 1;
  w.a = (const unsigned short*)dy;
  w.b = (const unsigned short*)x;
  w.dw = dw;
  w.ws = ws;
  w.Mg = g->K;
  w.Ng = g->R * g->S * g->C;
  w.Kg = g->N * g->P * g->Q;
  w.a_bytes = (int)(2 * dya);
  w.b_bytes = (int)(2 * xb);
  w.dPQ = make_fastdiv(g->P * g->Q);
  w.dQ = make_fastdiv(g->Q);
  bool tuned = false;
  int sd = 1, sw = 1, pt = 1;
  if (g_pair_force_dg > 0 && g_pair_force_wg > 0) {
    tuned = true;
    sd = g_pair_force_dg;
// ... 122 lines not shown
```

distributed-data-parallel-ml-training_amd/csrc/kernels/conv_l0.hip:

```cpp
#include "common.h"
#include "api.h"

#include <algorithm>

namespace ddp_amd {
namespace l0 {

constexpr int kK = 64;
constexpr int kNT = 4;
constexpr int kNKS = 3;

struct Args {
  const unsigned short* x;
  const unsigned short* wc;
  const float* bias;
  int N, H, W, tiles;
  int wb, per_img;
  FastDiv wb_d, per_img_d;
  float eps;
  int relu;
  float* stats;
  const float* gamma;
  const float* beta;
  float* coef;
  unsigned short* y;
  const unsigned short* dy;
  float* sums;
  unsigned short* dz;
  unsigned* code;
  unsigned short* zw;
  float* dgamma;
  float* dbeta;
  float* wg;
};

typedef unsigned short u16x4 __attribute__((ext_vector_type(4)));

__device__ __forceinline__ bf16x8 as_bf(const uint4& v) { return __builtin_bit_cast(bf16x8, v); }

struct Lane {
  int g, rl;
  int ph[kNKS], pw[kNKS];
};

__device__ __forceinline__ Lane lane_setup() {
  Lane ln;
  const int lane = threadIdx.x & 63;
  ln.g = lane >> 4;
  ln.rl = lane & 15;
  const int pr = (ln.rl >> 1) & 1, pc = 2 * (ln.rl >> 2) + (ln.rl & 1);
#pragma unroll
  for (int t = 0; t < kNKS; ++t) {
    const int tap = 4 * t + ln.g;
    const int r = tap / 3, s = tap - r * 3;
// ... 171 lines not shown
    const float mu = s1 / M;
    const float var = fmaxf(s2 / M - mu * mu, 0.f);
    const float is = rsqrtf(var + a.eps);
    const float sc = a.gamma[c] * is, sh = a.beta[c] - mu * sc;
    sm.cf[0][c] = sc;
    sm.cf[1][c] = sh;
    if (blockIdx.x == 0) {
      a.coef[0 * kK + c] = sc;
      a.coef[1 * kK + c] = sh;
      a.coef[2 * kK + c] = mu;
      a.coef[3 * kK + c] = is;
    }
  }
  float bias[kNT], sc[kNT], sh[kNT];
  lane_bias(a, ln.rl, bias);
  __syncthreads();
  lane4(sm.cf[0], ln.rl, sc);
  lane4(sm.cf[1], ln.rl, sh);
  tile_loop<false, false>(a, ln, [&](const Tile& cur, const Ops& op) {
    float z[kNT][4];
    conv_z(sm, op.x, bias, ln.g, ln.rl, z);
    u16x4 o, ow;
    unsigned cw = 0;
#pragma unroll
    for (int j = 0; j < kNT; ++j) {
      float y[4];
#pragma unroll
      for (int v = 0; v < 4; ++v) {
        y[v] = z[j][v] * sc[j] + sh[j];
        if (a.relu) y[v] = __builtin_elementwise_maximum(y[v], 0.f);
      }
      const float m = __builtin_elementwise_maximum(__builtin_elementwise_maximum(y[0], y[1]),
                                                    __builtin_elementwise_maximum(y[2], y[3]));
      unsigned pos = 0xFFu;
      float zs = 0.f;
#pragma unroll
      for (int v = 3; v >= 0; --v) {
        const bool hit = y[v] == m;
        pos = hit ? (unsigned)v : pos;
        zs = hit ? z[j][v] : zs;
      }
      const unsigned cd = pos == 0xFFu ? 0xFFu : (a.relu && !(m > 0.f)) ? 4u : pos;
      cw |= cd << (8 * j);
      o[j] = f2bf(m);
      ow[j] = f2bf(zs);
    }
    const size_t win = window_of(a, cur, ln.g);
    *reinterpret_cast<u16x4*>(a.y + win * kK + 4 * ln.rl) = o;
    *reinterpret_cast<u16x4*>(a.zw + win * kK + 4 * ln.rl) = ow;
    a.code[win * (kK / 4) + code_dword(ln.rl)] = cw;
  });
}

__global__ __launch_bounds__(256) void l0_sums_kernel(Args a, int windows) {
  __shared__ float red[256][33];
  const int tid = threadIdx.x, g = tid & 3;
  float mu[kNT][4], is[kNT][4], s1[kNT][4] = {}, s2[kNT][4] = {};
#pragma unroll
  for (int j = 0; j < kNT; ++j)
#pragma unroll
    for (int v = 0; v < 4; ++v) {
      const int c = j * 16 + 4 * g + v;
      mu[j][v] = a.coef[2 * kK + c];
      is[j][v] = a.coef[3 * kK + c];
    }
  for (int w = blockIdx.x * 64 + (tid >> 2); w < windows; w += gridDim.x * 64) {
    const uint4 cq = *reinterpret_cast<const uint4*>(a.code + (size_t)w * (kK / 4) + g * 4);
    const unsigned cw[kNT] = {cq.x, cq.y, cq.z, cq.w};
    u16x4 dv[kNT], zv[kNT];
#pragma unroll
    for (int j = 0; j < kNT; ++j) {
      dv[j] = *reinterpret_cast<const u16x4*>(a.dy + (size_t)w * kK + j * 16 + 4 * g);
      zv[j] = *reinterpret_cast<const u16x4*>(a.zw + (size_t)w * kK + j * 16 + 4 * g);
    }
#pragma unroll
    for (int j = 0; j < kNT; ++j)
#pragma unroll
      for (int v = 0; v < 4; ++v) {
        const float d = ((cw[j] >> (8 * v)) & 0xFFu) < 4u ? bf2f(dv[j][v]) : 0.f;
        s1[j][v] += d;
        s2[j][v] += d * ((bf2f(zv[j][v]) - mu[j][v]) * is[j][v]);
      }
  }
#pragma unroll
  for (int j = 0; j < kNT; ++j)
#pragma unroll
    for (int v = 0; v < 4; ++v) {
      red[tid][j * 4 + v] = s1[j][v];
      red[tid][16 + j * 4 + v] = s2[j][v];
    }
  __syncthreads();
  if (tid < 2 * kK) {
    const int k = tid / kK, c = tid - k * kK;
    const int gg = (c & 15) >> 2, e = k * 16 + (c >> 4) * 4 + (c & 3);
    float t = 0.f;
    for (int i = 0; i < 64; ++i) t += red[4 * i + gg][e];
    atomicAdd(a.sums + stat_rep(blockIdx.x) * 2 * kK + k * kK + c, stat_val(t, blockIdx.x));
  }
}

typedef short v4i16 __attribute__((ext_vector_type(4)));
constexpr int kWgN = 28;
constexpr int kWgSlab = kK * kWgN;
struct alignas(16) WgStage {
  unsigned short xp[4 * 10][4];
};
template <bool ON> struct WgLds { WgStage w[4]; };
template <> struct WgLds<false> {};

template <int APPLY>
__device__ __forceinline__ void l0_bwd_body(const Args& a) {
  static_assert(APPLY == 1 || APPLY == 2, "dz is stored or chained into the weight gradient");
  constexpr bool WG = APPLY == 2;
  __shared__ Smem sm;
  __shared__ WgLds<WG> wl;
  const Lane ln = lane_setup();
  const int g = ln.g, rl = ln.rl, wib = threadIdx.x >> 6;
  f32x4 dwacc[kNT][2];
  int xoff[2] = {0, 0};
  int pidx[kNKS] = {0, 0, 0};
  if (WG) {
#pragma unroll
    for (int jt = 0; jt < kNT; ++jt)
#pragma unroll
      for (int nt = 0; nt < 2; ++nt) dwacc[jt][nt] = (f32x4){0.f, 0.f, 0.f, 0.f};
#pragma unroll
    for (int nt = 0; nt < 2; ++nt) {
      const int n = nt * 16 + rl;
      const int tap = n < 27 ? n / 3 : 0, c = n < 27 ? n - tap * 3 : 3;
      const int tr = tap / 3, ts = tap - tr * 3;
      xoff[nt] = ((tr * 10) + 2 * g + ts) * 4 + c;
    }
#pragma unroll
    for (int t = 0; t < kNKS; ++t)
      pidx[t] = 4 * t + g < 9 ? (ln.ph[t] + 1) * 10 + ln.pw[t] + 1 : -1;
  }
  stage_weights(a, sm);
  if (threadIdx.x < kK) {
    const int c = threadIdx.x;
    const float sc = a.coef[c], mu = a.coef[2 * kK + c], is = a.coef[3 * kK + c];
    const float inv_m = 1.f / ((float)a.N * a.H * a.W);
    float t1 = 0.f, t2 = 0.f;
#pragma unroll
    for (int r = 0; r < kStatRep; ++r) {
      t1 += a.sums[r * 2 * kK + c];
      t2 += a.sums[r * 2 * kK + kK + c];
    }
    const float k1 = t1 * inv_m, k2 = t2 * inv_m;
    sm.cf[0][c] = sc;
    sm.cf[1][c] = -sc * k2 * is;
    sm.cf[2][c] = sc * (k2 * is * mu - k1);
    if (blockIdx.x == 0) {
      a.coef[4 * kK + c] = k1;
      a.coef[5 * kK + c] = k2;
      if (a.dgamma) a.dgamma[c] += t2;
      if (a.dbeta) a.dbeta[c] += t1;
// ... 43 lines not shown
#pragma unroll
        for (int nt = 0; nt < 2; ++nt)
          dwacc[jt][nt] =
              __builtin_amdgcn_mfma_f32_16x16x16bf16_1k(fa, fb[nt], dwacc[jt][nt], 0, 0, 0);
      }
    } else {
      unsigned short* dst =
          a.dz + (((size_t)cur.n * a.H + 2 * cur.hp) * a.W + 8 * cur.cb + 2 * g) * kK + 4 * rl;
#pragma unroll
      for (int v = 0; v < 4; ++v) {
        const u16x4 q = {o[0][v], o[1][v], o[2][v], o[3][v]};
        *reinterpret_cast<u16x4*>(dst + ((size_t)(v >> 1) * a.W + (v & 1)) * kK) = q;
      }
    }
  });
  if constexpr (WG) {
    float* red = reinterpret_cast<float*>(sm.w);
    const int lane = threadIdx.x & 63;
    __syncthreads();
#pragma unroll
    for (int w = 0; w < 4; ++w) {
      if (wib == w) {
#pragma unroll
        for (int jt = 0; jt < kNT; ++jt)
#pragma unroll
          for (int nt = 0; nt < 2; ++nt)
#pragma unroll
            for (int v = 0; v < 4; ++v) {
              const int e = (jt * 2 + nt) * 4 + v;
              float t = dwacc[jt][nt][v];
              if (w > 0) t += red[e * 64 + lane];
              if (w < 3) {
                red[e * 64 + lane] = t;
              } else if (nt * 16 + rl < kWgN) {
                a.wg[(size_t)blockIdx.x * kWgSlab + (4 * (4 * g + v) + jt) * kWgN + nt * 16 + rl] = t;
              }
            }
      }
      if (w < 3) __syncthreads();
    }
  }
}

template <int APPLY>
__global__ __launch_bounds__(256) void l0_bwd_kernel(Args a) {
  l0_bwd_body<APPLY>(a);
}
template <>
__global__ __launch_bounds__(256) __attribute__((amdgpu_waves_per_eu(4, 4))) void l0_bwd_kernel<2>(
    Args a) {
  l0_bwd_body<2>(a);
}

constexpr int kWgBatch = 8;
__global__ __launch_bounds__(256) void l0_wgrad_finish_kernel(const float* __restrict__ ws,
                                                              int nslab, float* __restrict__ dw,
                                                              int wkrsc, SgdFuse sg) {
  __shared__ float4 red[64][4];
  const bool opt = sg.p != nullptr;
  const float lr = opt ? sched_lr_block(sg.sched, sg.lr) : sg.lr;
  const int e = threadIdx.x & 3, s0 = threadIdx.x >> 2;
  const int i4 = blockIdx.x * 4 + e;
  float4 v = make_float4(0.f, 0.f, 0.f, 0.f);
  for (int z = s0; z < nslab; z += 64 * kWgBatch) {
    float4 t[kWgBatch];
#pragma unroll
    for (int u = 0; u < kWgBatch; ++u)
      if (z + 64 * u < nslab)
        t[u] = reinterpret_cast<const float4*>(ws + (size_t)(z + 64 * u) * kWgSlab)[i4];
#pragma unroll
    for (int u = 0; u < kWgBatch; ++u)
      if (z + 64 * u < nslab) { v.x += t[u].x; v.y += t[u].y; v.z += t[u].z; v.w += t[u].w; }
  }
  red[s0][e] = v;
  for (int h = 32; h >= 1; h >>= 1) {
    __syncthreads();
    if (s0 < h) {
      const float4 o = red[s0 + h][e];
      v.x += o.x; v.y += o.y; v.z += o.z; v.w += o.w;
      red[s0][e] = v;
    }
  }
  if (s0 != 0) return;
  const float vv[4] = {v.x, v.y, v.z, v.w};
#pragma unroll
  for (int t = 0; t < 4; ++t) {
    const int idx = i4 * 4 + t, k = idx / kWgN, n = idx - k * kWgN;
    if (n >= 27) continue;
    const int tap = n / 3, c = n - tap * 3;
    if (opt) {
      const int mi = k * 27 + n;
      float b = sg.buf[mi];
      const float np = sgd_update1(sg.p[mi], vv[t], b, lr, sg.momentum, sg.wd, sg.grad_scale,
                                   sg.nesterov);
      sg.p[mi] = np;
      sg.buf[mi] = b;
      sg.wc[(k * 9 + tap) * 8 + c] = f2bf(np);
    } else {
      dw[wkrsc ? k * 27 + n : (k * 3 + c) * 9 + tap] += vv[t];
    }
  }
}

static unsigned grid_for(int tiles) {
  return (unsigned)std::max(1, std::min(1024, (tiles + 3) / 4));
}

}
}

using namespace ddp_amd;

static bool l0_shape_ok(const ConvGeom* g) {
  return g->C == 8 && g->Creal <= 8 && g->K == l0::kK && g->R == 3 && g->S == 3 &&
         g->stride == 1 && g->pad == 1 && g->P == g->H && g->Q == g->W && g->H % 2 == 0 &&
         g->W % 8 == 0 && (size_t)g->N * g->H * g->W * l0::kK < (1ull << 31);
}

extern "C" int ddp_l0_ok(const ConvGeom* g) { return l0_shape_ok(g) ? 1 : 0; }

static l0::Args l0_args(const ConvGeom* g, const L0Io* io) {
  l0::Args a{};
  a.x = (const unsigned short*)io->x;
  a.wc = (const unsigned short*)io->wc;
  a.bias = io->bias;
  a.N = g->N; a.H = g->H; a.W = g->W;
  a.tiles = g->N * (g->H / 2) * (g->W / 8);
  a.wb = g->W / 8;
  a.per_img = (g->H / 2) * a.wb;
  a.wb_d = make_fastdiv(a.wb);
  a.per_img_d = make_fastdiv(a.per_img);
  a.eps = io->eps;
  a.relu = io->relu;
  a.stats = io->stats;
  a.gamma = io->gamma;
  a.beta = io->beta;
  a.coef = io->coef;
  a.y = (unsigned short*)io->y;
  a.dy = (const unsigned short*)io->dy;
  a.sums = io->sums;
  a.dz = (unsigned short*)io->dz;
  a.code = (unsigned*)io->code;
  a.zw = (unsigned short*)io->zw;
  a.dgamma = io->dgamma;
  a.dbeta = io->dbeta;
  return a;
}

extern "C" int ddp_l0_fwd(const ConvGeom* g, const L0Io* io, hipStream_t st) {
  if (!l0_shape_ok(g) || !io->x || !io->wc || !io->stats || !io->gamma || !io->beta ||
      !io->coef || !io->y || !io->code || !io->zw)
    return -1;
  const l0::Args a = l0_args(g, io);
  const unsigned nb = l0::grid_for(a.tiles);
  hipLaunchKernelGGL(l0::l0_stats_kernel, dim3(nb), dim3(256), 0, st, a);
  hipLaunchKernelGGL(l0::l0_fwd_kernel, dim3(nb), dim3(256), 0, st, a);
  return (int)hipGetLastError();
}

extern "C" int ddp_l0_bwd(const ConvGeom* g, const L0Io* io, hipStream_t st) {
  const bool fused = !io->dz && io->dw;
  if (!l0_shape_ok(g) || !io->x || !io->wc || !io->coef || !io->dy || !io->sums ||
      (!io->dz && !io->dw) || !io->code || !io->zw)
    return -1;
  l0::Args a = l0_args(g, io);
  const unsigned nb = l0::grid_for(a.tiles);
  if (fused && (g->Creal != 3 || !io->ws || io->ws_elems < (size_t)nb * l0::kWgSlab)) return -2;
  const int windows = g->N * (g->H / 2) * (g->W / 2);
  const unsigned ns = (unsigned)std::max(1, std::min(512, (windows + 127) / 128));
  if (!io->sums_ready)
    hipLaunchKernelGGL(l0::l0_sums_kernel, dim3(ns), dim3(256), 0, st, a, windows);
  if (!fused) {
    hipLaunchKernelGGL(l0::l0_bwd_kernel<1>, dim3(nb), dim3(256), 0, st, a);
    return (int)hipGetLastError();
  }
  a.wg = io->ws;
  hipLaunchKernelGGL(l0::l0_bwd_kernel<2>, dim3(nb), dim3(256), 0, st, a);
  SgdFuse sg{};
  if (g->wkrsc) ddp_sgd_fuse_take_final(io->dw, &sg);
  hipLaunchKernelGGL(l0::l0_wgrad_finish_kernel, dim3(l0::kWgSlab / 16), dim3(256), 0, st,
                     (const float*)io->ws, (int)nb, io->dw, g->wkrsc, sg);
  return (int)hipGetLastError();
}
```

distributed-data-parallel-ml-training_amd/csrc/kernels/conv_tr.hip:

```cpp
#include "common.h"
#include "api.h"

#include <algorithm>
#include <cstdlib>
#include <map>
#include <tuple>

namespace ddp_amd {
namespace tr {

typedef __attribute__((address_space(3))) void lds_void;

constexpr unsigned kOOB = 0x80000000u;

__device__ __forceinline__ __amdgpu_buffer_rsrc_t make_rsrc(const void* base, int bytes) {
  return __builtin_amdgcn_make_buffer_rsrc(const_cast<void*>(base), (short)0, bytes, 0x00020000);
}

__device__ __forceinline__ void dma(__amdgpu_buffer_rsrc_t rs, unsigned byte_off, unsigned short* lds) {
  __builtin_amdgcn_raw_ptr_buffer_load_lds(rs, (lds_void*)lds, 16, (int)byte_off, 0, 0, 0);
}

template <int N>
__device__ __forceinline__ void wait_dma_barrier() {
// ... 606 lines not shown

extern "C" int ddp_conv_fwd_tr(const ConvGeom* g, const void* x, const void* wc, const float* bias,
                               void* z, float* stats, float* ws, size_t ws_elems,
                               const BnFwdFuse* bn, int* bn_done, const TrFwdIn* in,
                               hipStream_t st) {
  using namespace ddp_amd::tr;
  if (bn_done) *bn_done = 0;
  const int in_mode = in ? (in->pool ? 2 : 1) : 0;
  if (in && (!in->z || !in->stats || !in->gamma || !in->beta || !in->coef || !in->y)) return -1;
  Plan pl;
  if (!plan(g, ws, ws_elems, in_mode, &pl)) return 0;
  const Cfg& c = pl.c;
  const Geo& geo = pl.geo;
  const int N = g->N, H = g->H, W = g->W, C = g->C, K = g->K;
  const size_t M = (size_t)N * H * W;
  Args a{};
  a.N = N; a.H = H; a.W = W; a.C = C; a.K = K;
  a.x = (const unsigned short*)x;
  a.wc = (const unsigned short*)wc;
  a.bias = bias;
  a.z = (unsigned short*)z;
  a.stats = stats;
  a.ws = ws;
  a.splits = pl.splits;
  a.cbps = pl.cbps;
  a.imgs = geo.imgs; a.rows = geo.rows; a.bands = geo.bands;
  a.imgp = geo.imgp; a.plane = geo.plane; a.zslot = geo.zslot;
  a.x_bytes = (int)(2 * M * C);
  a.w_bytes = (int)(2 * (size_t)K * 9 * C);
  a.abuf_elems = geo.abuf;
  a.tiles_m = (int)(M / c.bm);
  a.tiles_n = K / c.bn;
  a.dTiles = make_fastdiv(std::max(1, a.tiles_m * a.tiles_n));
  a.dTilesN = make_fastdiv(std::max(1, a.tiles_n));
  a.dBands = make_fastdiv(std::max(1, geo.bands));
  a.dPw = make_fastdiv((geo.rows + 2) * W);
  a.dW = make_fastdiv(W);
  a.dPerImg = make_fastdiv(geo.rows * W);
  if (in) {
    a.zin = (const unsigned short*)in->z;
    a.in_stats = in->stats;
    a.in_gamma = in->gamma;
    a.in_beta = in->beta;
    a.in_eps = in->eps;
    a.in_relu = in->relu;
    a.in_coef = in->coef;
    a.y_out = (unsigned short*)in->y;
    a.z_bytes = (int)(2 * M * C * (in->pool ? 4 : 1));
  }
#ifdef DDP_CONV_STAMPS
  a.stamps = g_conv_stamps;
#endif
  const int items = a.tiles_m * a.tiles_n * pl.splits;
  if (!launch_stages(c, in_mode, a, geo.nl, items, st)) return 0;
  int e = (int)hipGetLastError();
  if (e) return 2 + e;
  if (pl.splits > 1) {
    e = ddp_conv_fwd_finish(g, ws, pl.splits, bias, z, stats, bn, bn_done, st);
    if (e) return 2 + e;
  }
  return 1;
}

extern "C" int ddp_conv_tr_would_serve(const ConvGeom* g, size_t ws_elems, int in_mode) {
  ddp_amd::tr::Plan pl;
  float dummy;
  if (in_mode < 0) return 0;
  return ddp_amd::tr::plan(g, ws_elems ? &dummy : nullptr, ws_elems, in_mode, &pl) ? 1 : 0;
}

extern "C" int ddp_conv_tr_geometry(int BM, int N, int H, int W, int* out7) {
  const ddp_amd::tr::Geo g = ddp_amd::tr::geometry(BM, N, H, W);
  out7[0] = g.ok; out7[1] = g.imgs; out7[2] = g.rows; out7[3] = g.bands;
  out7[4] = g.imgp; out7[5] = g.plane; out7[6] = g.nl;
  return g.ok ? 1 : 0;
}
```

distributed-data-parallel-ml-training_amd/csrc/kernels/optim.hip:

```cpp
#include "common.h"
#include "api.h"

namespace ddp_amd {

__global__ __launch_bounds__(256) void sgd_kernel(float* __restrict__ p, const float* __restrict__ g,
                                                  float* __restrict__ buf, size_t n, float lr,
                                                  float momentum, float wd, float grad_scale,
                                                  int nesterov, const LrSched* sched) {
  lr = sched_lr_block(sched, lr);
  const size_t n4 = n / 4;
  const size_t stride = (size_t)gridDim.x * blockDim.x;
  for (size_t i = blockIdx.x * (size_t)blockDim.x + threadIdx.x; i < n4; i += stride) {
    float4 pv = reinterpret_cast<float4*>(p)[i];
    const float4 gv = reinterpret_cast<const float4*>(g)[i];
    float4 bv = reinterpret_cast<float4*>(buf)[i];
    float* pp = &pv.x;
    const float* gg = &gv.x;
    float* bb = &bv.x;
#pragma unroll
    for (int e = 0; e < 4; ++e) {
      pp[e] = sgd_update1(pp[e], gg[e], bb[e], lr, momentum, wd, grad_scale, nesterov);
    }
    reinterpret_cast<float4*>(p)[i] = pv;
    reinterpret_cast<float4*>(buf)[i] = bv;
  }
  for (size_t i = n4 * 4 + blockIdx.x * (size_t)blockDim.x + threadIdx.x; i < n; i += stride) {
    p[i] = sgd_update1(p[i], g[i], buf[i], lr, momentum, wd, grad_scale, nesterov);
  }
}

constexpr int kMaxPack = 64;
struct PackTable {
  PackDesc d[kMaxPack];
  int n;
};

__device__ __forceinline__ size_t master_index(const PackDesc& d, int k, int c, int r, int s) {
  return d.krsc ? (((size_t)k * d.R + r) * d.S + s) * d.Cr + c
                : (((size_t)k * d.Cr + c) * d.R + r) * d.S + s;
}

__global__ __launch_bounds__(256) void pack_conv_weights_kernel(PackTable t) {
  const PackDesc d = t.d[blockIdx.y];
  const int rs = d.R * d.S;
  const size_t total = (size_t)d.K * rs * d.C;
  const size_t stride = (size_t)gridDim.x * blockDim.x;
  for (size_t i = blockIdx.x * (size_t)blockDim.x + threadIdx.x; i < total; i += stride) {
    if (d.wc) {
      const int c = (int)(i % d.C);
      const size_t t1 = i / d.C;
      const int s = (int)(t1 % d.S);
      const size_t t2 = t1 / d.S;
      const int r = (int)(t2 % d.R);
      const int k = (int)(t2 / d.R);
// ... 43 lines not shown
  __syncthreads();
  return s_skip != 0u;
}

__device__ __forceinline__ bool last_block_done(unsigned* done) {
  __syncthreads();
  __shared__ unsigned last;
  if (threadIdx.x == 0) {
    __threadfence();
    const unsigned t = __hip_atomic_fetch_add(done, 1u, __ATOMIC_ACQ_REL, __HIP_MEMORY_SCOPE_AGENT);
    last = (t == gridDim.x - 1) ? 1u : 0u;
  }
  __syncthreads();
  return last != 0u;
}

__device__ __forceinline__ void signal_flag(unsigned* done, unsigned* signal) {
  if (threadIdx.x == 0) {
    __hip_atomic_store(done, 0u, __ATOMIC_RELAXED, __HIP_MEMORY_SCOPE_AGENT);
    __hip_atomic_fetch_add(signal, 1u, __ATOMIC_RELEASE, __HIP_MEMORY_SCOPE_AGENT);
  }
}

__device__ __forceinline__ void sched_stage(LrSched* s) {
  const unsigned k = __hip_atomic_load(&s->step, __ATOMIC_RELAXED, __HIP_MEMORY_SCOPE_AGENT);
  __hip_atomic_store(&s->next, k + 1u, __ATOMIC_RELAXED, __HIP_MEMORY_SCOPE_AGENT);
}

template <bool LARS>
__device__ __forceinline__ float sgd1(float p, float g, float& b, const SgdHyper& h, float trust) {
  if constexpr (!LARS) {
    return sgd_update1(p, g, b, h.lr, h.momentum, h.wd, h.grad_scale, h.nesterov);
  } else {
    float d = trust * __builtin_fmaf(h.wd, p, g * h.grad_scale);
    if (h.momentum != 0.f) {
      b = __builtin_fmaf(h.momentum, b, d);
      d = h.nesterov ? __builtin_fmaf(h.momentum, b, d) : b;
    }
    return __builtin_fmaf(-h.lr, d, p);
  }
}

struct GuardState {
  float norm, c;
  int skipped;
  float* stats;
  int count;
};

template <bool LARS, bool GUARD = false>
__device__ void sgd_pack_body(const int4* __restrict__ items, const long long* __restrict__ descs,
                              float* __restrict__ p, float* __restrict__ g,
                              float* __restrict__ buf, const SgdHyper& h, float* tile,
                              float trust, GuardState gd = GuardState{});

__global__ __launch_bounds__(256) void sgd_pack_kernel(const int4* __restrict__ items,
                                                       const long long* __restrict__ descs,
                                                       float* __restrict__ p,
                                                       float* __restrict__ g,
                                                       float* __restrict__ buf, SgdHyper h) {
  __shared__ float tile[kTileElems];
  h.lr = sched_lr_block(h.sched, h.lr);
  if (h.sched_advance && blockIdx.x == 0 && threadIdx.x == 0) sched_stage(h.sched);
  sgd_pack_body<false>(items, descs, p, g, buf, h, tile, 1.f);
  if (h.signal && last_block_done(h.done)) signal_flag(h.done, h.signal);
}

struct LarsArgs {
  const int2* side;
  const int4* tensors;
  const float2* partial;
  float* trust;
  float eta, eps;
};

constexpr int kNormChunk = 8192;

__global__ __launch_bounds__(256) void lars_norms_kernel(const int4* __restrict__ items,
                                                         const float* __restrict__ p,
                                                         const float* __restrict__ g,
                                                         float grad_scale,
                                                         float2* __restrict__ partial) {
  const int4 it = items[blockIdx.x];
  const size_t off = (size_t)(unsigned)it.x;
  const int cnt = it.y, n4 = cnt >> 2;
  const int tid = threadIdx.x;
  const float4* p4 = reinterpret_cast<const float4*>(p + off);
  const float4* g4 = reinterpret_cast<const float4*>(g + off);
  constexpr int kIter = kNormChunk / (256 * 4);
  const float4 z = make_float4(0.f, 0.f, 0.f, 0.f);
  float4 pv[kIter], gv[kIter];
#pragma unroll
  for (int j = 0; j < kIter; ++j) {
    const int i = tid + 256 * j;
    pv[j] = i < n4 ? p4[i] : z;
    gv[j] = i < n4 ? g4[i] : z;
  }
  float sp = 0.f, sg = 0.f;
#pragma unroll
  for (int j = 0; j < kIter; ++j) {
    const float* pp = &pv[j].x;
    const float* gg = &gv[j].x;
#pragma unroll
    for (int e = 0; e < 4; ++e) {
      const float gs = gg[e] * grad_scale;
      sp = __builtin_fmaf(pp[e], pp[e], sp);
      sg = __builtin_fmaf(gs, gs, sg);
    }
  }
  const int t = (n4 << 2) + tid;
  if (t < cnt) {
    const float pt = p[off + t], gs = g[off + t] * grad_scale;
    sp = __builtin_fmaf(pt, pt, sp);
    sg = __builtin_fmaf(gs, gs, sg);
  }
  sp = wave_sum(sp);
  sg = wave_sum(sg);
  __shared__ float2 s_w[4];
  if ((tid & 63) == 0) s_w[tid >> 6] = make_float2(sp, sg);
  __syncthreads();
  if (tid == 0) {
    partial[it.z] = make_float2(((s_w[0].x + s_w[1].x) + s_w[2].x) + s_w[3].x,
                                ((s_w[0].y + s_w[1].y) + s_w[2].y) + s_w[3].y);
  }
}

template <bool GUARD = false>
__device__ __forceinline__ float lars_trust_block(const LarsArgs& a, float wd, float c = 1.f) {
  __shared__ float s_trust;
  if (threadIdx.x < 64) {
    const int2 sd = a.side[blockIdx.x];
    float t = 1.f;
    if (sd.x >= 0) {
      const int4 tn = a.tensors[sd.x];
      if (tn.z) {
        float sp = 0.f, sg = 0.f;
        for (int c = threadIdx.x; c < tn.y; c += 64) {
          const float2 v = a.partial[tn.x + c];
          sp += v.x;
          sg += v.y;
        }
        const float wn = sqrtf(wave_sum(sp));
        float gn = sqrtf(wave_sum(sg));
        if constexpr (GUARD) gn *= c;
        if (wn > 0.f && gn > 0.f) t = a.eta * wn / (gn + wd * wn + a.eps);
      }
      if (sd.y && threadIdx.x == 0) a.trust[sd.x] = t;
    }
    if (threadIdx.x == 0) s_trust = t;
  }
  __syncthreads();
  return s_trust;
}

__global__ __launch_bounds__(256) void lars_pack_kernel(const int4* __restrict__ items,
                                                        const long long* __restrict__ descs,
                                                        float* __restrict__ p,
                                                        float* __restrict__ g,
                                                        float* __restrict__ buf, SgdHyper h,
                                                        LarsArgs la) {
  __shared__ float tile[kTileElems];
  h.lr = sched_lr_block(h.sched, h.lr);
  if (h.sched_advance && blockIdx.x == 0 && threadIdx.x == 0) sched_stage(h.sched);
  const float trust = lars_trust_block(la, h.wd);
  sgd_pack_body<true>(items, descs, p, g, buf, h, tile, trust);
  if (h.signal && last_block_done(h.done)) signal_flag(h.done, h.signal);
}

struct ClipArgs {
  const float* partial;
  int n_chunks;
  float max_norm, eps;
  int flags;
  float* stats;
};

__global__ __launch_bounds__(256) void grad_sumsq_kernel(const int4* __restrict__ items,
                                                         const float* __restrict__ g,
                                                         float grad_scale,
                                                         float* __restrict__ partial) {
  const int4 it = items[blockIdx.x];
  const size_t off = (size_t)(unsigned)it.x;
  const int cnt = it.y, n4 = cnt >> 2;
  const int tid = threadIdx.x;
  const float4* g4 = reinterpret_cast<const float4*>(g + off);
  constexpr int kIter = kNormChunk / (256 * 4);
  float4 gv[kIter];
#pragma unroll
  for (int j = 0; j < kIter; ++j) {
    const int i = tid + 256 * j;
    gv[j] = i < n4 ? g4[i] : make_float4(0.f, 0.f, 0.f, 0.f);
  }
  float sg = 0.f;
#pragma unroll
  for (int j = 0; j < kIter; ++j) {
    const float* gg = &gv[j].x;
#pragma unroll
    for (int e = 0; e < 4; ++e) {
      const float gs = gg[e] * grad_scale;
      sg = __builtin_fmaf(gs, gs, sg);
    }
  }
  const int t = (n4 << 2) + tid;
  if (t < cnt) {
    const float gs = g[off + t] * grad_scale;
    sg = __builtin_fmaf(gs, gs, sg);
  }
  sg = wave_sum(sg);
  __shared__ float s_w[4];
  if ((tid & 63) == 0) s_w[tid >> 6] = sg;
  __syncthreads();
  if (tid == 0) partial[it.z] = ((s_w[0] + s_w[1]) + s_w[2]) + s_w[3];
}

__device__ __forceinline__ GuardState clip_block(const ClipArgs& a) {
  __shared__ float s_norm, s_c;
  __shared__ int s_skipped;
  if (threadIdx.x < 64) {
// ... 5 lines not shown
      const float q = a.max_norm / (norm + a.eps);
      c = q >= 1.f ? 1.f : q;
    }
    if (threadIdx.x == 0) {
      s_norm = norm;
      s_c = c;
      s_skipped = ((a.flags & 2) && !(norm <= 3.402823466e+38f)) ? 1 : 0;
    }
  }
  __syncthreads();
  return GuardState{s_norm, s_c, s_skipped, a.stats, (a.flags & 4) ? 1 : 0};
}

__device__ __forceinline__ void guard_clear(const int4& it, const long long* __restrict__ descs,
                                            float* __restrict__ g) {
  const int tid = threadIdx.x;
  if (it.x == 0 || it.x == 3) {
    float* gp = g + (size_t)(unsigned)it.y;
    for (int i = tid; i < it.z; i += 256) gp[i] = 0.f;
    return;
  }
  if (it.x == 2) {
    float* gp = g + (size_t)descs[12 * it.w] + (unsigned)it.y;
    for (int i = tid; i < it.z; i += 256) gp[i] = 0.f;
    return;
  }
  const long long* d = descs + 12 * it.y;
  const size_t poff = (size_t)d[0];
  const int K = (int)d[1], Cr = (int)d[2], RS = (int)d[4] * (int)d[5];
  int TK, TC;
  tile_dims(RS, &TK, &TC);
  const int k0 = it.z, c0 = it.w;
  const int tk = min(TK, K - k0);
  const int tcr = max(0, min(TC, Cr - c0));
  if (d[8] == 0) {
    const int run = tcr * RS;
    for (int idx = tid; idx < tk * run; idx += 256) {
      const int kl = idx / run, e = idx - kl * run;
      g[poff + (size_t)(k0 + kl) * Cr * RS + (size_t)c0 * RS + e] = 0.f;
    }
  } else {
    for (int idx = tid; idx < tk * RS * tcr; idx += 256) {
      const int cl = idx % tcr, t = idx / tcr;
      const int rs = t % RS, kl = t / RS;
      g[poff + ((size_t)(k0 + kl) * RS + rs) * Cr + c0 + cl] = 0.f;
    }
  }
}

template <bool LARS, bool GUARD>
__device__ void sgd_pack_body(const int4* __restrict__ items, const long long* __restrict__ descs,
                              float* __restrict__ p, float* __restrict__ g,
                              float* __restrict__ buf, const SgdHyper& h, float* tile,
                              float trust, GuardState gd) {
  const int4 it = items[blockIdx.x];
  const int tid = threadIdx.x;
  if (h.counter && blockIdx.x == 0 && tid == 0) atomicAdd(h.counter, h.delta);
  if (block_skip(h.skip)) return;
  if constexpr (GUARD) {
    if (blockIdx.x == 0 && tid == 0) {
      gd.stats[0] = gd.norm;
      gd.stats[1] = gd.c;
      if (gd.skipped && gd.count) {
        unsigned* n = reinterpret_cast<unsigned*>(gd.stats + 2);
        *n = *n + 1u;
      }
    }
    if (gd.skipped && it.x != 4 && it.x != 5) {
      if (h.zero_grad) guard_clear(it, descs, g);
      return;
    }
  }
  if (it.x == 0) {
    const size_t off = (size_t)(unsigned)it.y;
    const int cnt = it.z;
    for (int i = tid * 4; i < cnt; i += 256 * 4) {
      if (i + 4 <= cnt && ((off + i) & 3) == 0) {
        float4 pv = *reinterpret_cast<float4*>(p + off + i);
        const float4 gv = *reinterpret_cast<const float4*>(g + off + i);
        float4 bv = *reinterpret_cast<float4*>(buf + off + i);
        pv.x = sgd1<LARS>(pv.x, gv.x, bv.x, h, trust);
        pv.y = sgd1<LARS>(pv.y, gv.y, bv.y, h, trust);
        pv.z = sgd1<LARS>(pv.z, gv.z, bv.z, h, trust);
        pv.w = sgd1<LARS>(pv.w, gv.w, bv.w, h, trust);
        *reinterpret_cast<float4*>(p + off + i) = pv;
        *reinterpret_cast<float4*>(buf + off + i) = bv;
        if (h.zero_grad) *reinterpret_cast<float4*>(g + off + i) = make_float4(0.f, 0.f, 0.f, 0.f);
      } else {
        for (int e = i; e < min(cnt, i + 4); ++e) {
          float b = buf[off + e];
          p[off + e] = sgd1<LARS>(p[off + e], g[off + e], b, h, trust);
          buf[off + e] = b;
          if (h.zero_grad) g[off + e] = 0.f;
        }
      }
    }
    return;
  }
  if (it.x == 3) {
    const size_t off = (size_t)(unsigned)it.y;
    const int cnt = it.z;
    float* slot = it.w >= 0 && h.slot ? h.slot + it.w : nullptr;
    for (int i = tid * 4; i < cnt; i += 256 * 4) {
      float4 pv = *reinterpret_cast<float4*>(p + off + i);
      const float4 gv = *reinterpret_cast<const float4*>(g + off + i);
      float4 bv = *reinterpret_cast<float4*>(buf + off + i);
      pv.x = sgd1<LARS>(pv.x, gv.x, bv.x, h, trust);
      pv.y = sgd1<LARS>(pv.y, gv.y, bv.y, h, trust);
      pv.z = sgd1<LARS>(pv.z, gv.z, bv.z, h, trust);
      pv.w = sgd1<LARS>(pv.w, gv.w, bv.w, h, trust);
      *reinterpret_cast<float4*>(p + off + i) = pv;
      *reinterpret_cast<float4*>(buf + off + i) = bv;
      if (h.zero_grad) *reinterpret_cast<float4*>(g + off + i) = make_float4(0.f, 0.f, 0.f, 0.f);
// ... 66 lines not shown
    const int run = tcr * RS;
    for (int idx = tid; idx < tk * run; idx += 256) {
      const int kl = idx / run, e = idx - kl * run;
      const size_t gi = poff + (size_t)(k0 + kl) * Cr * RS + (size_t)c0 * RS + e;
      float b = buf[gi];
      const float np = sgd1<LARS>(p[gi], g[gi], b, h, trust);
      p[gi] = np;
      buf[gi] = b;
      if (h.zero_grad) g[gi] = 0.f;
      tile[kl * TC * RS + e] = np;
    }
  } else {
    for (int idx = tid; idx < tk * RS * tcr; idx += 256) {
      const int cl = idx % tcr, t = idx / tcr;
      const int rs = t % RS, kl = t / RS;
      const size_t gi = poff + ((size_t)(k0 + kl) * RS + rs) * Cr + c0 + cl;
      float b = buf[gi];
      const float np = sgd1<LARS>(p[gi], g[gi], b, h, trust);
      p[gi] = np;
      buf[gi] = b;
      if (h.zero_grad) g[gi] = 0.f;
      tile[kl * TC * RS + cl * RS + rs] = np;
    }
  }
  __syncthreads();
  if (wc) {
    for (int idx = tid; idx < tk * RS * tcp; idx += 256) {
      const int cl = idx % tcp, t = idx / tcp;
      const int rs = t % RS, kl = t / RS;
      const float v = cl < tcr ? tile[(kl * TC + cl) * RS + rs] : 0.f;
      wc[((size_t)(k0 + kl) * RS + rs) * C + c0 + cl] = f2bf(v);
    }
  }
  if (wt) {
    for (int idx = tid; idx < tcr * RS * tk; idx += 256) {
      const int kl = idx % tk, t = idx / tk;
      const int rs = t % RS, cl = t / RS;
      wt[((size_t)(c0 + cl) * RS + rs) * K + k0 + kl] = f2bf(tile[(kl * TC + cl) * RS + rs]);
    }
  }
}

__global__ __launch_bounds__(256) void sgd_clip_pack_kernel(const int4* __restrict__ items,
                                                            const long long* __restrict__ descs,
                                                            float* __restrict__ p,
                                                            float* __restrict__ g,
                                                            float* __restrict__ buf, SgdHyper h,
                                                            ClipArgs ca) {
  __shared__ float tile[kTileElems];
  h.lr = sched_lr_block(h.sched, h.lr);
  if (h.sched_advance && blockIdx.x == 0 && threadIdx.x == 0) sched_stage(h.sched);
  const GuardState gd = clip_block(ca);
  h.grad_scale *= gd.c;
  sgd_pack_body<false, true>(items, descs, p, g, buf, h, tile, 1.f, gd);
  if (h.signal && last_block_done(h.done)) signal_flag(h.done, h.signal);
}

__global__ __launch_bounds__(256) void lars_clip_pack_kernel(const int4* __restrict__ items,
                                                             const long long* __restrict__ descs,
                                                             float* __restrict__ p,
                                                             float* __restrict__ g,
                                                             float* __restrict__ buf, SgdHyper h,
                                                             LarsArgs la, ClipArgs ca) {
  __shared__ float tile[kTileElems];
  h.lr = sched_lr_block(h.sched, h.lr);
  if (h.sched_advance && blockIdx.x == 0 && threadIdx.x == 0) sched_stage(h.sched);
  const GuardState gd = clip_block(ca);
  const float trust = gd.skipped ? 1.f : lars_trust_block<true>(la, h.wd, gd.c);
  h.grad_scale *= gd.c;
  sgd_pack_body<true, true>(items, descs, p, g, buf, h, tile, trust, gd);
  if (h.signal && last_block_done(h.done)) signal_flag(h.done, h.signal);
}

constexpr int kMaxTailPack = 4;
struct TailArgs {
  const int4* segs;
  int n_segs;
  const float* src;
  float* dst;
  PackDesc pack[kMaxTailPack];
  int n_pack;
  unsigned* done;
  unsigned* signal;
  const unsigned* skip;
};

__global__ __launch_bounds__(256) void shard_tail_kernel(TailArgs a) {
  const bool skipped = block_skip(a.skip);
  if (!skipped && (int)blockIdx.x < a.n_segs) {
    const int4 e = a.segs[blockIdx.x];
    const float* s = a.src + (size_t)(unsigned)e.x;
    float* d = a.dst + (size_t)(unsigned)e.y;
    for (int i = threadIdx.x; i < e.z; i += 256) d[i] = s[i];
  }
  if (!last_block_done(a.done)) return;
  __threadfence();
  if (!skipped) {
    for (int q = 0; q < a.n_pack; ++q) {
      const PackDesc& d = a.pack[q];
      const int rs = d.R * d.S;
      const int total = d.K * rs * d.C;
      for (int i = threadIdx.x; i < total; i += 256) {
        const int c = i % d.C, t1 = i / d.C;
        const int sx = t1 % d.S, t2 = t1 / d.S;
        const int r = t2 % d.R, k = t2 / d.R;
        const float v = c < d.Cr ? d.p[master_index(d, k, c, r, sx)] : 0.f;
        d.wc[i] = f2bf(v);
      }
    }
    __syncthreads();
    __threadfence();
  }
  if (a.signal) signal_flag(a.done, a.signal);
  else if (threadIdx.x == 0) __hip_atomic_store(a.done, 0u, __ATOMIC_RELAXED, __HIP_MEMORY_SCOPE_AGENT);
}

__global__ void counter_add_kernel(int* c, int delta, LrSched* sched, int sched_mode) {
  if (threadIdx.x != 0 || blockIdx.x != 0) return;
  if (c) *c += delta;
  if (!sched) return;
  if (sched_mode == 1) sched_stage(sched);
  const unsigned k = __hip_atomic_load(&sched->next, __ATOMIC_RELAXED, __HIP_MEMORY_SCOPE_AGENT);
  __hip_atomic_store(&sched->step, k, __ATOMIC_RELAXED, __HIP_MEMORY_SCOPE_AGENT);
}

}

using namespace ddp_amd;

extern "C" int ddp_sgd(float* p, const float* g, float* buf, size_t n, float lr, float momentum,
                       float wd, float grad_scale, int nesterov, const LrSched* sched,
                       hipStream_t st) {
  size_t blocks = (n / 4 + 255) / 256;
  if (blocks > 4096) blocks = 4096;
  if (blocks < 1) blocks = 1;
  hipLaunchKernelGGL(sgd_kernel, dim3((unsigned)blocks), dim3(256), 0, st, p, g, buf, n, lr,
                     momentum, wd, grad_scale, nesterov, sched);
  return (int)hipGetLastError();
}

extern "C" int ddp_pack_conv_weights(const PackDesc* descs, int n, hipStream_t st) {
  for (int base = 0; base < n; base += kMaxPack) {
    PackTable t{};
    t.n = n - base < kMaxPack ? n - base : kMaxPack;
    size_t maxel = 0;
    for (int i = 0; i < t.n; ++i) {
      t.d[i] = descs[base + i];
      const size_t el = (size_t)t.d[i].K * t.d[i].R * t.d[i].S * t.d[i].C;
      if (el > maxel) maxel = el;
    }
    size_t bx = (maxel + 255) / 256;
    if (bx > 512) bx = 512;
    hipLaunchKernelGGL(pack_conv_weights_kernel, dim3((unsigned)bx, t.n), dim3(256), 0, st, t);
  }
  return (int)hipGetLastError();
}

extern "C" int ddp_sgd_pack(const void* items, int n_items, const long long* descs, float* p,
                            float* g, float* buf, float lr, float momentum, float wd,
                            float grad_scale, int nesterov, int zero_grad, int* counter,
                            int delta, const unsigned* skip, unsigned short* shadow, float* slot,
                            unsigned* done, unsigned* signal, LrSched* sched, int sched_advance,
                            const void* lars_side, const void* lars_tensors,
                            const void* lars_partial, float* lars_trust, float lars_eta,
                            float lars_eps, const float* clip_partial, int clip_chunks,
                            float clip_max_norm, float clip_eps, int clip_flags,
                            float* clip_stats, hipStream_t st) {
  SgdHyper h{lr, momentum, wd, grad_scale, nesterov, zero_grad, counter, delta, skip, shadow, slot,
             done, signal, sched, sched && sched_advance ? 1 : 0};
  if (n_items <= 0) return 0;
  if (clip_partial && (!clip_stats || clip_chunks < 0)) return -1;
  ClipArgs ca{clip_partial, clip_chunks, clip_max_norm, clip_eps, clip_flags, clip_stats};
  if (lars_side) {
    if (!lars_tensors || !lars_partial || !lars_trust) return -1;
    LarsArgs la{(const int2*)lars_side, (const int4*)lars_tensors, (const float2*)lars_partial,
                lars_trust, lars_eta, lars_eps};
    if (clip_partial) {
      hipLaunchKernelGGL(lars_clip_pack_kernel, dim3(n_items), dim3(256), 0, st,
                         (const int4*)items, descs, p, g, buf, h, la, ca);
      return (int)hipGetLastError();
    }
    hipLaunchKernelGGL(lars_pack_kernel, dim3(n_items), dim3(256), 0, st, (const int4*)items,
                       descs, p, g, buf, h, la);
    return (int)hipGetLastError();
  }
  if (clip_partial) {
    hipLaunchKernelGGL(sgd_clip_pack_kernel, dim3(n_items), dim3(256), 0, st, (const int4*)items,
                       descs, p, g, buf, h, ca);
    return (int)hipGetLastError();
  }
  hipLaunchKernelGGL(sgd_pack_kernel, dim3(n_items), dim3(256), 0, st, (const int4*)items, descs,
                     p, g, buf, h);
  return (int)hipGetLastError();
}

extern "C" int ddp_grad_sumsq(const void* items, int n_items, const float* g, float grad_scale,
                              float* partial, hipStream_t st) {
  if (n_items <= 0) return 0;
  hipLaunchKernelGGL(grad_sumsq_kernel, dim3(n_items), dim3(256), 0, st, (const int4*)items, g,
                     grad_scale, partial);
  return (int)hipGetLastError();
}

extern "C" int ddp_lars_norms(const void* items, int n_items, const float* p, const float* g,
                              float grad_scale, void* partial, hipStream_t st) {
  if (n_items <= 0) return 0;
  hipLaunchKernelGGL(lars_norms_kernel, dim3(n_items), dim3(256), 0, st, (const int4*)items, p, g,
                     grad_scale, (float2*)partial);
  return (int)hipGetLastError();
}

extern "C" int ddp_shard_tail(const void* segs, int n_segs, const float* src, float* dst,
                              const PackDesc* pack, int n_pack, unsigned* done, unsigned* signal,
                              const unsigned* skip, hipStream_t st) {
  if (n_pack > kMaxTailPack || !done) return -1;
  TailArgs a{};
  a.segs = (const int4*)segs; a.n_segs = n_segs; a.src = src; a.dst = dst;
  for (int i = 0; i < n_pack; ++i) a.pack[i] = pack[i];
  a.n_pack = n_pack; a.done = done; a.signal = signal; a.skip = skip;
  hipLaunchKernelGGL(shard_tail_kernel, dim3(n_segs > 0 ? n_segs : 1), dim3(256), 0, st, a);
  return (int)hipGetLastError();
}

extern "C" void ddp_sgd_tile_dims(int RS, int* TK, int* TC) {
// ... 13 lines not shown
```

distributed-data-parallel-ml-training_amd/ops/common.py:

```python
import os

import torch

from .._ext import load as _load

_NATIVE = None
CONV_STAGES = 2
BWD_PAIR_MODE, BWD_PAIR_ITEMS = 3, 1024


def native():
    global _NATIVE
    if _NATIVE is None:
        _NATIVE = _load()
        _NATIVE.conv_options(CONV_STAGES)
        _NATIVE.conv_pair_mode(BWD_PAIR_MODE, BWD_PAIR_ITEMS)
        load_conv_tuning(_NATIVE)
    return _NATIVE


TUNING_FILE = os.path.join(os.path.dirname(os.path.abspath(__file__)), "conv_tuning.json")




def load_conv_tuning(n=None, path=None):
    import json
    n = n or native()
    n.conv_tune_clear()
    path = path or os.environ.get("DDP_AMD_CONV_TUNING_FILE") or TUNING_FILE
    if os.environ.get("DDP_AMD_CONV_TUNING", "1") == "0" or not os.path.exists(path):
        return 0
    with open(path) as f:
        table = json.load(f)
    for e in table.get("entries", []):
        if int(e["mode"]) == 3 and "H" in e:
            n.conv_pair_tune_set(int(e["M"]), int(e["N"]), int(e["K"]), int(e["H"]) ** 2,
                                 int(e["tile"]), int(e["splits"]), int(e.get("stages", 1)))
            continue
        n.conv_tune_set(int(e["mode"]), int(e["M"]), int(e["N"]), int(e["K"]), int(e["tile"]),
                        int(e["splits"]), int(e.get("stages", 0)))
    n.conv_tr_set(-1, 0, 0, 0, 0, 0, 0, 0)
    for e in table.get("tr_entries", []):
        n.conv_tr_set(2, int(e["M"]), int(e["K"]), int(e["C"]), int(e["H"]), int(e["bm"]),
                      int(e["bn"]), int(e["splits"]), int(e.get("stages", 0)))
    return len(table.get("entries", [])) + len(table.get("tr_entries", []))


def weight_krsc(w):
    if w is None or w.dim() != 4 or w.shape[2] * w.shape[3] == 1 or w.shape[1] == 1:
        return 0
    return int(w.stride(1) == 1)


def ptr(t):
    if t is None:
        return 0
    return t.data_ptr()


def stream_handle(stream=None):
# ... 143 lines not shown
```

distributed-data-parallel-ml-training_amd/optim/sgd.py:

```python
import itertools

import torch

from .arena import arena_for
from .schedule import LRSchedule

_GUARD_SHARDED = ("gradient clipping / non-finite step skipping needs the norm of the whole "
                  "gradient: after a reduce-scatter a rank holds only a shard of it, and a global "
                  "norm would need one more collective; use the replicated update, "
                  "update=\"allreduce\"")


class FusedSGD(torch.optim.SGD):
    needs_whole_tensors = False

    def __init__(self, params, lr=0.1, momentum=0.0, dampening=0.0, weight_decay=0.0,
                 nesterov=False, grad_scale=1.0, max_grad_norm=None, clip_eps=1e-6,
                 skip_nonfinite=False):
        params = list(params)
        super().__init__(params, lr=lr, momentum=momentum, dampening=dampening,
                         weight_decay=weight_decay, nesterov=nesterov)
        self._grad_scale_factor = grad_scale
        self._fused = bool(params) and params[0].is_cuda
        if self._fused:
# ... 161 lines not shown
        return int(self._lr_dev[2].item()) if self._sched_ptr() else self._lr_step

    def current_lr(self):
        if self._schedule is None:
            return float(self.param_groups[0]["lr"])
        return self._schedule.lr_at(self._lr_step)

    def count_step(self):
        if self._schedule is None:
            return
        if self._fused and torch.cuda.is_current_stream_capturing():
            return
        self._lr_step += 1

    def _sched_ptr(self):
        return self._lr_dev.data_ptr() if (self._schedule is not None and self._fused) else 0

    def _sched_kw(self, advance):
        ptr = self._sched_ptr()
        return {"sched": ptr, "sched_advance": int(bool(advance))} if ptr else {}

    def commit_lr_step(self, stream=None):
        if self._sched_ptr():
            from ..ops.common import native, stream_handle
            native().counter_add(0, 0, stream if stream is not None else stream_handle(),
                                 sched=self._sched_ptr(), sched_mode=2)

    def _sched_commit(self, advance, stream):
        if advance and advance != "stage" and self._sched_ptr():
            from ..ops.common import native
            native().counter_add(0, 0, stream, sched=self._sched_ptr(), sched_mode=2)
        if advance:
            self.count_step()

    def _cpu_lr(self):
        if self._schedule is not None:
            self.param_groups[0]["lr"] = self._schedule.lr_at(self._lr_step)
        return float(self.param_groups[0]["lr"])

    def _packs(self):
        return [p._ddp_amd_pack() for p in self.arena.params if hasattr(p, "_ddp_amd_pack")]

    def repack(self):
        descs = self._packs()
        if descs and self.arena.data.is_cuda:
            from ..ops.common import native, stream_handle
            native().pack_conv_weights(descs, stream_handle())

    def register_in_backward(self):
        if self.guarded:
            raise RuntimeError("gradient clipping / non-finite step skipping cannot run in the "
                               "backward: the norm exists only once the whole gradient does "
                               "(TrainStep keeps opt_in_bwd False)")
        from ..ops.common import native
        a, g = self.arena, self.param_groups[0]
        nat = native()
        nat.sgd_fuse_register(0, clear=1)
        self._bwd_index = {}
        base_g, base_p = a.grad.data_ptr(), a.data.data_ptr()
        base_b = self.momentum_buffer.data_ptr()
        sched = {"sched": self._sched_ptr()} if self._sched_ptr() else {}
        for i, p in enumerate(a.params):
            if not hasattr(p, "_ddp_amd_pack"):
                continue
            pp, wc, wt, K, Cr, C, R, S, krsc = p._ddp_amd_pack()
            if wt or not wc or not (krsc or R * S == 1) or pp != base_p + 4 * a.offsets[i]:
                continue
            dw = base_g + 4 * a.offsets[i]
            nat.sgd_fuse_register(dw, pp, base_b + 4 * a.offsets[i], wc, float(g["lr"]),
                                  float(g["momentum"]), float(g["weight_decay"]),
                                  float(self._grad_scale_factor), int(bool(g["nesterov"])),
                                  **sched)
            self._bwd_index[dw] = i
        nat.sgd_fuse_begin()

    def unregister_in_backward(self):
        from ..ops.common import native
        native().sgd_fuse_register(0, clear=1)

    def _fused_in_backward(self):
        from ..ops.common import native
        idx = getattr(self, "_bwd_index", {})
        return frozenset(idx[d] for d in native().sgd_fuse_taken() if d in idx)

    def _master_in_backward(self):
        from ..ops.common import native
        idx = getattr(self, "_bwd_index", {})
        return frozenset(idx[d] for d in native().sgd_fuse_taken_master() if d in idx)

    def _work_table(self, prange=None, exclude=frozenset(), pack_only=frozenset()):
        from ..ops.common import native
        a = self.arena
        key = tuple(self._packs())
        if getattr(self, "_table_key", None) != key:
            self._tables = {}
            self._table_key = key
            descs, per_param = [], [[] for _ in a.params]
            for i, p in enumerate(a.params):
                if not hasattr(p, "_ddp_amd_pack"):
                    continue
                pp, wc, wt, K, Cr, C, R, S, krsc = p._ddp_amd_pack()
                if pp != a.data.data_ptr() + 4 * a.offsets[i] or (R * S > 1 and bool(krsc) != a.krsc[i]):
                    raise RuntimeError("packed conv weight is not a view into the parameter arena")
                d = len(descs)
                descs.append([a.offsets[i], K, Cr, C, R, S, wc, wt, int(krsc), 0, 0, 0])
                n = a.numels[i]
                if not wt and C == Cr and (krsc or R * S == 1) and n % 4 == 0:
                    for s0 in range(0, n, 8192):
                        per_param[i].append([2, s0, min(8192, n - s0), d])
                    continue
                TK, TC = native().sgd_tile_dims(R * S)
                if TK * TC * R * S > native().sgd_tile_limit():
                    self._table_key = None
                    raise ValueError(
                        f"parameter {i} (conv weight {K}x{Cr}x{R}x{S}, operand channels {C}): a "
                        f"{TK} x {TC} tile of a {R}x{S} filter needs {TK * TC * R * S} floats, "
                        f"the re-pack kernel's tile holds {native().sgd_tile_limit()}")
                for k0 in range(0, K, TK):
                    for c0 in range(0, C, TC):
                        per_param[i].append([1, d, k0, c0])
            chunk = 8192
            for i in range(len(a.params)):
                if per_param[i]:
                    continue
                o, n = a.offsets[i], a.numels[i]
                for s in range(0, n, chunk):
                    per_param[i].append([0, o + s, min(chunk, n - s), 0])
            self._per_param = per_param
            dev = a.data.device
            self._descs = torch.tensor(descs if descs else [[0] * 12], dtype=torch.int64, device=dev)
        rng = tuple(prange) if prange is not None else (0, len(a.params))
# ... 88 lines not shown
    def repack_params(self, i0, i1, stream=None):
        descs = [p._ddp_amd_pack() for p in self.arena.params[i0:i1] if hasattr(p, "_ddp_amd_pack")]
        if descs and self.arena.data.is_cuda:
            from ..ops.common import native, stream_handle
            native().pack_conv_weights(descs, stream.cuda_stream if stream is not None
                                       else stream_handle())

    def zero_grad(self, set_to_none=False):
        if self._fused:
            self.arena.zero_grad()
        else:
            super().zero_grad(set_to_none=set_to_none)

    @torch.no_grad()
    def step(self, closure=None, zero_grad=False, counter=None, skip=None, params=None,
             stream=None, fused_taken=False, signal=None, lr_advance=None, norm_done=False):
        if lr_advance is None:
            lr_advance = params is None
        if not self._fused:
            self._cpu_lr()
            if self.guarded:
                if closure is not None:
                    with torch.enable_grad():
                        loss = closure()
                    closure = lambda: loss
                c, skipped = self._cpu_guard(lr_advance)
                if skipped:
                    out = closure() if closure is not None else None
                    if lr_advance:
                        self.count_step()
                    if zero_grad:
                        super().zero_grad(set_to_none=False)
                    return out
                self._cpu_scale_grads(c)
            out = super().step(closure)
            if lr_advance:
                self.count_step()
            if zero_grad:
                super().zero_grad(set_to_none=False)
            return out
        from ..ops.common import native, stream_handle
        s = stream.cuda_stream if stream is not None else stream_handle()
        exclude = pack_only = frozenset()
        if fused_taken:
            if self.guarded:
                raise RuntimeError("gradient guard: no update is taken in the backward")
            pack_only = self._master_in_backward()
            exclude = self._fused_in_backward() | pack_only
        items, n_items, descs = self._work_table(params, exclude, pack_only)
        sched = self._sched_kw(lr_advance)
        if self.guarded and not norm_done:
            self.grad_sumsq(params, stream)
        if n_items == 0:
            if sched.get("sched_advance"):
                native().counter_add(int(counter[0]) if counter else 0,
                                     int(counter[1]) if counter else 0, s,
                                     sched=sched["sched"], sched_mode=1)
                self.count_step()
            elif counter:
                native().counter_add(int(counter[0]), int(counter[1]), s)
            if signal:
                native().flag_signal(int(signal[1]), s)
            return None
        self._update_launch(items, n_items, s, descs=descs, zero_grad=zero_grad, counter=counter,
                            skip=skip, signal=signal, lr_advance=lr_advance)
        return None

    def state_dict(self):
        sd = super().state_dict()
        if self._schedule is not None:
            sd["lr_schedule"] = {"schedule": self._schedule.state_dict(), "step": self._lr_step}
        if self.guarded:
            sd["grad_guard"] = {"skipped": int(self.skipped_steps())}
        if self._fused:
            a = self.arena
            for i, p in enumerate(a.params):
                    sd["state"][i] = {"momentum_buffer": a.shaped(self.momentum_buffer, i).contiguous()}
        return sd

    def load_state_dict(self, sd):
        ls = sd.get("lr_schedule")
        if ls is not None:
            self.set_schedule(LRSchedule.from_state_dict(ls["schedule"]), step=int(ls["step"]))
        saved = sd["param_groups"][0] if sd.get("param_groups") else {}
        if "skip_nonfinite" in saved or "max_grad_norm" in saved:
            self._set_guard(saved.get("max_grad_norm"), saved.get("clip_eps", 1e-6),
                            saved.get("skip_nonfinite", False))
        gg = sd.get("grad_guard")
        if gg is not None and self.guarded:
            if self._guard_dev is not None:
                self._guard_dev.view(torch.int32)[2] = int(gg["skipped"])
            self._guard_cpu[2] = int(gg["skipped"])
        if not self._fused:
            return super().load_state_dict({k: v for k, v in sd.items()
                                            if k not in ("lr_schedule", "grad_guard")})
        a = self.arena
        st = sd.get("state", {})
        for i, p in enumerate(a.params):
            buf = st.get(i, st.get(str(i), {})).get("momentum_buffer")
            if buf is not None:
                a.shaped(self.momentum_buffer, i).copy_(buf.reshape(p.shape))
        for k in ("lr", "momentum", "weight_decay", "nesterov"):
            if sd.get("param_groups"):
                self.param_groups[0][k] = sd["param_groups"][0].get(k, self.param_groups[0][k])
```

Baseline: 379,700 images/s.

## Co-launch deferred conv weight-grad finish blocks with following BN-backward or SGD kernels

Defers the wgrad finish reduction of a conv backward and appends its blocks to the grid of the next BN-backward reduce/apply/local kernel or the SGD pack kernel. Each kernel checks whether its block index falls past its primary work and runs the finish body instead. This removes separate small kernel launches and lets independent tails overlap, filling idle CUs. In exchange it adds template variants, flush points for correctness, and bookkeeping in Python to decide when co-launch is safe.

```diff
diff --git a/distributed-data-parallel-ml-training_amd/csrc/bind.cpp b/distributed-data-parallel-ml-training_amd/csrc/bind.cpp
--- a/distributed-data-parallel-ml-training_amd/csrc/bind.cpp
+++ b/distributed-data-parallel-ml-training_amd/csrc/bind.cpp
@@ -276,6 +276,14 @@
      py::arg("momentum") = 0.f, py::arg("wd") = 0.f, py::arg("grad_scale") = 1.f,
      py::arg("nesterov") = 0, py::arg("clear") = 0, py::arg("sched") = 0);
   m.def("sgd_fuse_begin", []() { ddp_sgd_fuse_begin(); });
+  m.def("conv_finish_defer", [](int on) { ddp_conv_finish_defer(on); });
+  m.def("conv_finish_flush", []() { ddp_conv_finish_flush(); });
+  m.def("conv_finish_stats", []() {
+    long long v[3];
+    ddp_conv_finish_stats(v);
+    return py::make_tuple(v[0], v[1], v[2]);
+  });
+  m.def("conv_finish_pending", []() { return ddp_conv_finish_pending(); });
   m.def("sgd_fuse_taken", []() {
     std::vector<uintptr_t> v(256);
     int n = ddp_sgd_fuse_taken(v.data(), (int)v.size());
@@ -509,7 +517,7 @@
                        uintptr_t lars_tensors, uintptr_t lars_partial, uintptr_t lars_trust,
                        float lars_eta, float lars_eps, uintptr_t clip_partial, int clip_chunks,
                        float clip_max_norm, float clip_eps, int clip_flags,
-                       uintptr_t clip_stats) {
+                       uintptr_t clip_stats, int finish_colaunch) {
     check(ddp_sgd_pack(P<void>(items), n_items, P<long long>(descs), P<float>(p), P<float>(g),
                        P<float>(buf), lr, momentum, wd, grad_scale, nesterov, zero_grad,
                        P<int>(counter), delta, P<const unsigned>(skip), P<unsigned short>(shadow),
@@ -517,7 +525,8 @@
                        P<ddp_amd::LrSched>(sched), sched_advance, P<void>(lars_side),
                        P<void>(lars_tensors), P<void>(lars_partial), P<float>(lars_trust),
                        lars_eta, lars_eps, P<const float>(clip_partial), clip_chunks,
-                       clip_max_norm, clip_eps, clip_flags, P<float>(clip_stats), S(st)),
+                       clip_max_norm, clip_eps, clip_flags, P<float>(clip_stats), finish_colaunch,
+                       S(st)),
           "sgd_pack");
   }, py::arg("items"), py::arg("n_items"), py::arg("descs"), py::arg("p"), py::arg("g"),
      py::arg("buf"), py::arg("lr"), py::arg("momentum"), py::arg("wd"), py::arg("grad_scale"),
@@ -528,7 +537,7 @@
      py::arg("lars_partial") = 0, py::arg("lars_trust") = 0, py::arg("lars_eta") = 0.f,
      py::arg("lars_eps") = 0.f, py::arg("clip_partial") = 0, py::arg("clip_chunks") = 0,
      py::arg("clip_max_norm") = 0.f, py::arg("clip_eps") = 0.f, py::arg("clip_flags") = 0,
-     py::arg("clip_stats") = 0);
+     py::arg("clip_stats") = 0, py::arg("finish_colaunch") = 0);
   m.def("grad_sumsq", [](uintptr_t items, int n_items, uintptr_t g, float grad_scale,
                          uintptr_t partial, uintptr_t st) {
     check(ddp_grad_sumsq(P<void>(items), n_items, P<float>(g), grad_scale, P<float>(partial),
diff --git a/distributed-data-parallel-ml-training_amd/csrc/kernels/api.h b/distributed-data-parallel-ml-training_amd/csrc/kernels/api.h
--- a/distributed-data-parallel-ml-training_amd/csrc/kernels/api.h
+++ b/distributed-data-parallel-ml-training_amd/csrc/kernels/api.h
@@ -234,6 +234,10 @@
 int ddp_sgd_fuse_taken(uintptr_t* out, int cap);
 int ddp_sgd_fuse_take_final(const float* dw, ddp_amd::SgdFuse* out);
 int ddp_sgd_fuse_taken_master(uintptr_t* out, int cap);
+void ddp_conv_finish_defer(int on);
+void ddp_conv_finish_flush();
+void ddp_conv_finish_stats(long long out[3]);
+uintptr_t ddp_conv_finish_pending();
 void ddp_conv_pair_force(int splits_dg, int splits_wg, int tile);
 int ddp_conv_bwd_pair(const ddp_amd::ConvGeom* g, const void* dy, const void* wc, void* dx,
                       const void* x, float* dw, float* ws, size_t ws_elems,
@@ -261,7 +265,7 @@
                  const void* lars_tensors, const void* lars_partial, float* lars_trust,
                  float lars_eta, float lars_eps, const float* clip_partial, int clip_chunks,
                  float clip_max_norm, float clip_eps, int clip_flags, float* clip_stats,
-                 hipStream_t st);
+                 int finish_colaunch, hipStream_t st);
 int ddp_grad_sumsq(const void* items, int n_items, const float* g, float grad_scale,
                    float* partial, hipStream_t st);
 int ddp_lars_norms(const void* items, int n_items, const float* p, const float* g,
diff --git a/distributed-data-parallel-ml-training_amd/csrc/kernels/bn_act.hip b/distributed-data-parallel-ml-training_amd/csrc/kernels/bn_act.hip
--- a/distributed-data-parallel-ml-training_amd/csrc/kernels/bn_act.hip
+++ b/distributed-data-parallel-ml-training_amd/csrc/kernels/bn_act.hip
@@ -1,5 +1,6 @@
 #include "common.h"
 #include "api.h"
+#include "finish_colaunch.h"
 
 #include <algorithm>
 #include <cstdio>
@@ -288,24 +289,43 @@
     }
 }
 
-template <bool POOL, int IPT, bool MASK = false, bool STRIDE = false, bool RBN = false>
-__global__ __launch_bounds__(256) void bn_act_bwd_reduce_kernel(BnArgs a) {
+template <bool CO> struct CoTail {};
+template <> struct CoTail<true> {
+  unsigned gx, gy;
+  WgFinishArgs wa;
+};
+
+template <bool POOL, int IPT, bool MASK = false, bool STRIDE = false, bool RBN = false,
+          bool CO = false>
+__global__ __launch_bounds__(256) void bn_act_bwd_reduce_kernel(BnArgs a, CoTail<CO> co) {
   constexpr int NS = RBN ? 3 : 2;
   constexpr int NP = POOL ? 4 : 1;
   __shared__ float red[8 * 256];
+  unsigned bx, by;
+  if constexpr (CO) {
+    const unsigned b = blockIdx.x, P = co.gx * co.gy;
+    if (b >= P) return wgrad_finish_krsc_co(co.wa, (int)(b - P));
+    bx = b % co.gx; by = b / co.gx;
+  } else {
+    bx = blockIdx.x; by = blockIdx.y;
+  }
+  const auto gx = [&]() -> unsigned {
+    if constexpr (CO) return co.gx;
+    else return gridDim.x;
+  };
   DDP_DEVICE_CHECK(a.C % 8 == 0 && (!POOL || (a.H % 2 == 0 && a.W % 2 == 0)));
   const int G = a.C / 8;
   const int Gb = a.red_gb ? a.red_gb : (G < 256 ? G : 256);
   const int Ho = POOL ? a.H / 2 : a.H, Wo = POOL ? a.W / 2 : a.W;
   const size_t npix = (size_t)a.N * Ho * Wo;
-  const int cg_base = blockIdx.y * Gb;
+  const int cg_base = by * Gb;
   const int cgl = threadIdx.x % Gb;
   const int prow = threadIdx.x / Gb, prows = 256 / Gb;
   const int c0 = (cg_base + cgl) * 8;
   const size_t per_blk = (size_t)prows * IPT;
-  const size_t nbx = STRIDE ? (npix + per_blk - 1) / per_blk : (size_t)blockIdx.x + 1;
+  const size_t nbx = STRIDE ? (npix + per_blk - 1) / per_blk : (size_t)bx + 1;
   BwdItems<POOL, IPT> L;
-  bwd_load<POOL, IPT, MASK, RBN>(a, L, (size_t)blockIdx.x * per_blk + prow, prows, npix,
+  bwd_load<POOL, IPT, MASK, RBN>(a, L, (size_t)bx * per_blk + prow, prows, npix,
                                  cg_base + cgl, Ho, Wo);
   float sc[8], sh[8], mu[8], is[8], rmu[8], ris[8];
   ld8f(a.coef + kSc * a.C + c0, sc);
@@ -321,7 +341,7 @@
   for (int k = 0; k < NS; ++k)
 #pragma unroll
     for (int e = 0; e < 8; ++e) acc[k][e] = 0.f;
-  for (size_t bb = blockIdx.x;;) {
+  for (size_t bb = bx;;) {
 #pragma unroll
     for (int it = 0; it < IPT; ++it) {
       if (!L.ok[it]) continue;
@@ -337,11 +357,11 @@
         }
       }
     }
-    bb += gridDim.x;
+    bb += gx();
     if (!STRIDE || bb >= nbx) break;
     bwd_load<POOL, IPT, MASK, RBN>(a, L, bb * per_blk + prow, prows, npix, cg_base + cgl, Ho, Wo);
   }
-  float* rep = a.sums + stat_rep(blockIdx.x) * 2 * a.C;
+  float* rep = a.sums + stat_rep(bx) * 2 * a.C;
   const int tid = threadIdx.x;
 #pragma unroll
   for (int k = 0; k < NS; ++k) {
@@ -349,32 +369,44 @@
 #pragma unroll
     for (int e = 0; e < 8; ++e) red[e * 256 + tid] = acc[k][e];
     __syncthreads();
-    float* dst = k < 2 ? rep + k * a.C : a.rsums + stat_rep(blockIdx.x) * 2 * a.C + a.C;
+    float* dst = k < 2 ? rep + k * a.C : a.rsums + stat_rep(bx) * 2 * a.C + a.C;
     for (int idx = tid; idx < Gb * 8; idx += 256) {
       const int g = idx / 8, e = idx % 8;
       float s = 0.f;
       for (int r = 0; r < prows; ++r) s += red[e * 256 + r * Gb + g];
-      atomicAdd(dst + (cg_base + g) * 8 + e, stat_val(s, blockIdx.x));
+      atomicAdd(dst + (cg_base + g) * 8 + e, stat_val(s, bx));
     }
   }
 }
 
 template <bool POOL, int IPT, bool FOLD = false, bool MASK = false, bool STRIDE = false,
-          bool RBN = false>
-__global__ __launch_bounds__(256) void bn_act_bwd_apply_kernel(BnArgs a) {
+          bool RBN = false, bool CO = false>
+__global__ __launch_bounds__(256) void bn_act_bwd_apply_kernel(BnArgs a, CoTail<CO> co) {
+  unsigned bx, by;
+  if constexpr (CO) {
+    const unsigned b = blockIdx.x, P = co.gx * co.gy;
+    if (b >= P) return wgrad_finish_krsc_co(co.wa, (int)(b - P));
+    bx = b % co.gx; by = b / co.gx;
+  } else {
+    bx = blockIdx.x; by = blockIdx.y;
+  }
+  const auto gx = [&]() -> unsigned {
+    if constexpr (CO) return co.gx;
+    else return gridDim.x;
+  };
   constexpr int NP = POOL ? 4 : 1;
   const int G = a.C / 8;
   const int Gb = G < 256 ? G : 256;
   const int Ho = POOL ? a.H / 2 : a.H, Wo = POOL ? a.W / 2 : a.W;
   const size_t npix = (size_t)a.N * Ho * Wo;
-  const int cg_base = blockIdx.y * Gb;
+  const int cg_base = by * Gb;
   const int cgl = threadIdx.x % Gb;
   const int prow = threadIdx.x / Gb, prows = 256 / Gb;
   const int c0 = (cg_base + cgl) * 8;
   const size_t per_blk = (size_t)prows * IPT;
   const size_t nbx = (npix + per_blk - 1) / per_blk;
   BwdItems<POOL, IPT> L;
-  bwd_load<POOL, IPT, MASK, RBN>(a, L, (size_t)blockIdx.x * per_blk + prow, prows, npix,
+  bwd_load<POOL, IPT, MASK, RBN>(a, L, (size_t)bx * per_blk + prow, prows, npix,
                                  cg_base + cgl, Ho, Wo);
   float sc[8], sh[8], mu[8], is[8], k1[8], k2[8], rsc[8], rmu[8], ris[8], rk2[8];
   if (RBN) {
@@ -404,7 +436,7 @@
 #pragma unroll
       for (int e = 0; e < 4; ++e) {
         kk[which][cl + e] = tv[e] * inv_m;
-        if (blockIdx.x == 0) {
+        if (bx == 0) {
           const int c = cg_base * 8 + cl + e;
           a.coef[(which ? kK2 : kK1) * a.C + c] = tv[e] * inv_m;
           float* dst = which ? a.dgamma : a.dbeta;
@@ -422,7 +454,7 @@
     ld8f(a.coef + kK1 * a.C + c0, k1);
     ld8f(a.coef + kK2 * a.C + c0, k2);
   }
-  for (size_t bb = blockIdx.x;;) {
+  for (size_t bb = bx;;) {
 #pragma unroll
     for (int it = 0; it < IPT; ++it) {
       if (!L.ok[it]) continue;
@@ -446,19 +478,27 @@
         else if (a.dres) st8(a.dres + L.off[it][d], r);
       }
     }
-    bb += gridDim.x;
+    bb += gx();
     if (!STRIDE || bb >= nbx) break;
     bwd_load<POOL, IPT, MASK, RBN>(a, L, bb * per_blk + prow, prows, npix, cg_base + cgl, Ho, Wo);
   }
 }
 
-template <bool POOL, int IPT, int NT, bool MASK = false>
-__global__ __launch_bounds__(NT) void bn_act_bwd_local_kernel(BnArgs a) {
+template <bool POOL, int IPT, int NT, bool MASK = false, bool CO = false>
+__global__ __launch_bounds__(NT) void bn_act_bwd_local_kernel(BnArgs a, CoTail<CO> co) {
+  unsigned bx;
+  if constexpr (CO) {
+    static_assert(NT == 256, "the carried finish runs in 256-thread blocks");
+    bx = blockIdx.x;
+    if (bx >= co.gx) return wgrad_finish_krsc_co(co.wa, (int)(bx - co.gx));
+  } else {
+    bx = blockIdx.x;
+  }
   constexpr int NP = POOL ? 4 : 1;
   constexpr int NW = NT / kWave;
   __shared__ float red[NW][16];
   __shared__ float fin[16];
-  const int cg = blockIdx.x;
+  const int cg = bx;
   const int c0 = cg * 8;
   const int Ho = POOL ? a.H / 2 : a.H, Wo = POOL ? a.W / 2 : a.W;
   const size_t npix = (size_t)a.N * Ho * Wo;
@@ -825,15 +865,16 @@
   ra.red_gb = rGb;
   const unsigned rbx = blocks_for(npix, (size_t)(256 / rGb) * IPT);
   const unsigned rx = reduce_grid_x(rbx, rch);
+  ddp_conv_finish_flush();
   if (rx < rbx)
     hipLaunchKernelGGL((bn_act_bwd_reduce_kernel<false, IPT, true, true, true>), dim3(rx, rch),
-                       dim3(256), 0, st, ra);
+                       dim3(256), 0, st, ra, CoTail<false>{});
   else
     hipLaunchKernelGGL((bn_act_bwd_reduce_kernel<false, IPT, true, false, true>), dim3(rbx, rch),
-                       dim3(256), 0, st, ra);
+                       dim3(256), 0, st, ra, CoTail<false>{});
   hipLaunchKernelGGL(bn_finalize_bwd_res_kernel, dim3(blocks_for(a.C, 256)), dim3(256), 0, st, a);
   hipLaunchKernelGGL((bn_act_bwd_apply_kernel<false, IPT, false, true, false, true>),
-                     dim3(bx, chunks), dim3(256), 0, st, a);
+                     dim3(bx, chunks), dim3(256), 0, st, a, CoTail<false>{});
 }
 
 template <bool POOL, int IPT, bool MASK>
@@ -846,30 +887,59 @@
     ra.red_gb = rGb;
     const unsigned rbx = blocks_for(npix, (size_t)(256 / rGb) * IPT);
     const unsigned rx = reduce_grid_x(rbx, rch);
-    if (rx < rbx)
+    PendingFinish pf;
+    const bool co = finish_take(st, !MASK ? kFinishKrsc : 0, &pf);
+    if constexpr (!MASK) {
+      if (co) {
+        const unsigned px = rx < rbx ? rx : rbx;
+        const CoTail<true> ct{px, (unsigned)rch, pf.wa};
+        const dim3 grid(px * rch + pf.wa.gx);
+        if (rx < rbx)
+          hipLaunchKernelGGL((bn_act_bwd_reduce_kernel<POOL, IPT, false, true, false, true>), grid,
+                             dim3(256), 0, st, ra, ct);
+        else
+          hipLaunchKernelGGL((bn_act_bwd_reduce_kernel<POOL, IPT, false, false, false, true>),
+                             grid, dim3(256), 0, st, ra, ct);
+      }
+    }
+    if (co) {
+    } else if (rx < rbx)
       hipLaunchKernelGGL((bn_act_bwd_reduce_kernel<POOL, IPT, MASK, true>), dim3(rx, rch),
-                         dim3(256), 0, st, ra);
+                         dim3(256), 0, st, ra, CoTail<false>{});
     else
       hipLaunchKernelGGL((bn_act_bwd_reduce_kernel<POOL, IPT, MASK, false>), dim3(rbx, rch),
-                         dim3(256), 0, st, ra);
+                         dim3(256), 0, st, ra, CoTail<false>{});
   }
   const size_t per_block = (size_t)kStatRep * 2 * (size_t)Gb * 8 * sizeof(float);
   const size_t fold_bytes = (size_t)bx * chunks * per_block;
   if (!kDeterministic && fold_bwd_bytes() > 0 && fold_bytes <= fold_bwd_bytes()) {
+    if (a.sums_ready) {
+      PendingFinish pf;
+      const bool co = finish_take(st, !MASK ? kFinishKrsc : 0, &pf);
+      if constexpr (!MASK) {
+        if (co) {
+          const CoTail<true> ct{bx, (unsigned)chunks, pf.wa};
+          hipLaunchKernelGGL((bn_act_bwd_apply_kernel<POOL, IPT, true, false, false, false, true>),
+                             dim3(bx * chunks + pf.wa.gx), dim3(256), 0, st, a, ct);
+          return;
+        }
+      }
+    }
     hipLaunchKernelGGL((bn_act_bwd_apply_kernel<POOL, IPT, true, MASK, false>), dim3(bx, chunks),
-                       dim3(256), 0, st, a);
+                       dim3(256), 0, st, a, CoTail<false>{});
     return;
   }
+  if (a.sums_ready) ddp_conv_finish_flush();
   const unsigned cx = std::min(bx, fold_fwd_grid() / (unsigned)chunks);
   if (!kDeterministic && fold_bwd_bytes() > 0 && cx * chunks >= 1024 &&
       (size_t)cx * chunks * per_block <= kFoldGridBytes) {
     hipLaunchKernelGGL((bn_act_bwd_apply_kernel<POOL, IPT, true, MASK, true>), dim3(cx, chunks),
-                       dim3(256), 0, st, a);
+                       dim3(256), 0, st, a, CoTail<false>{});
     return;
   }
   hipLaunchKernelGGL(bn_finalize_bwd_kernel, dim3(blocks_for(a.C, 256)), dim3(256), 0, st, a);
   hipLaunchKernelGGL((bn_act_bwd_apply_kernel<POOL, IPT, false, MASK, false>), dim3(bx, chunks),
-                     dim3(256), 0, st, a);
+                     dim3(256), 0, st, a, CoTail<false>{});
 }
 
 template <bool POOL, int IPT>
@@ -901,10 +971,24 @@
 template <bool POOL, bool MASK>
 static void launch_local_m(const BnArgs& a, int ipt, hipStream_t st) {
   const dim3 grid(a.C / 8), block(kLocalThreads);
-  if (ipt == 1) hipLaunchKernelGGL((bn_act_bwd_local_kernel<POOL, 1, kLocalThreads, MASK>), grid, block, 0, st, a);
-  else if (ipt == 2) hipLaunchKernelGGL((bn_act_bwd_local_kernel<POOL, 2, kLocalThreads, MASK>), grid, block, 0, st, a);
-  else if (ipt == 4) hipLaunchKernelGGL((bn_act_bwd_local_kernel<POOL, 4, kLocalThreads, MASK>), grid, block, 0, st, a);
-  else if constexpr (!POOL) hipLaunchKernelGGL((bn_act_bwd_local_kernel<POOL, 8, kLocalThreads, MASK>), grid, block, 0, st, a);
+  PendingFinish pf;
+  const bool co = finish_take(st, !MASK && kLocalThreads == 256 ? kFinishKrsc : 0, &pf);
+  if constexpr (!MASK && kLocalThreads == 256) {
+    if (co) {
+      const CoTail<true> ct{grid.x, 1u, pf.wa};
+      const dim3 cg(grid.x + pf.wa.gx);
+      if (ipt == 1) hipLaunchKernelGGL((bn_act_bwd_local_kernel<POOL, 1, 256, false, true>), cg, block, 0, st, a, ct);
+      else if (ipt == 2) hipLaunchKernelGGL((bn_act_bwd_local_kernel<POOL, 2, 256, false, true>), cg, block, 0, st, a, ct);
+      else if (ipt == 4 || POOL) hipLaunchKernelGGL((bn_act_bwd_local_kernel<POOL, 4, 256, false, true>), cg, block, 0, st, a, ct);
+      else hipLaunchKernelGGL((bn_act_bwd_local_kernel<false, 8, 256, false, true>), cg, block, 0, st, a, ct);
+      return;
+    }
+  }
+  const CoTail<false> no{};
+  if (ipt == 1) hipLaunchKernelGGL((bn_act_bwd_local_kernel<POOL, 1, kLocalThreads, MASK>), grid, block, 0, st, a, no);
+  else if (ipt == 2) hipLaunchKernelGGL((bn_act_bwd_local_kernel<POOL, 2, kLocalThreads, MASK>), grid, block, 0, st, a, no);
+  else if (ipt == 4) hipLaunchKernelGGL((bn_act_bwd_local_kernel<POOL, 4, kLocalThreads, MASK>), grid, block, 0, st, a, no);
+  else if constexpr (!POOL) hipLaunchKernelGGL((bn_act_bwd_local_kernel<POOL, 8, kLocalThreads, MASK>), grid, block, 0, st, a, no);
 }
 
 template <bool POOL>
diff --git a/distributed-data-parallel-ml-training_amd/csrc/kernels/conv_igemm.hip b/distributed-data-parallel-ml-training_amd/csrc/kernels/conv_igemm.hip
--- a/distributed-data-parallel-ml-training_amd/csrc/kernels/conv_igemm.hip
+++ b/distributed-data-parallel-ml-training_amd/csrc/kernels/conv_igemm.hip
@@ -1,6 +1,7 @@
 #include "common.h"
 #include "api.h"
 #include "linear_blocks.h"
+#include "finish_colaunch.h"
 #include <algorithm>
 #include <map>
 #include <set>
@@ -1088,7 +1089,6 @@
   return ((size_t)n * m.H + m.pa + m.stride * i) * m.W + m.pb + m.stride * j;
 }
 
-constexpr int kSlabBatch = 8;
 __device__ __forceinline__ void sum_slabs8(const float* p, size_t slab, int z0, int z1, float* v) {
   for (int zb = z0; zb < z1; zb += kSlabBatch) {
     float4 a[kSlabBatch], b[kSlabBatch];
@@ -1609,90 +1609,6 @@
   }
 }
 
-__device__ __forceinline__ float sgd_step1(float p, float g, float& b, const SgdFuse& h,
-                                           float lr) {
-  return sgd_update1(p, g, b, lr, h.momentum, h.wd, h.grad_scale, h.nesterov);
-}
-
-constexpr int kWgFinishGroupKrsc = kDeterministic ? (1 << 30) : 16;
-__device__ __forceinline__ void wgrad_finish_krsc_body(const float* __restrict__ ws, int splits,
-                                                       int K, int RS, int C, int Creal,
-                                                       float* __restrict__ dw, int bx, int by,
-                                                       int gx, int gy, const SgdFuse& sg) {
-  const size_t slab = (size_t)K * RS * C;
-  const size_t n4 = slab / 4;
-  const int z0 = by * kWgFinishGroupKrsc, z1 = min(splits, z0 + kWgFinishGroupKrsc);
-  const bool single = gy == 1;
-  const bool opt = single && sg.p != nullptr;
-  const float lr = opt ? sched_lr_block(sg.sched, sg.lr) : sg.lr;
-  for (size_t i = bx * (size_t)blockDim.x + threadIdx.x; i < n4;
-       i += (size_t)gx * blockDim.x) {
-    float4 v = reinterpret_cast<const float4*>(ws + z0 * slab)[i];
-    for (int zb = z0 + 1; zb < z1; zb += kSlabBatch) {
-      float4 a[kSlabBatch];
-#pragma unroll
-      for (int u = 0; u < kSlabBatch; ++u)
-        if (zb + u < z1) a[u] = reinterpret_cast<const float4*>(ws + (size_t)(zb + u) * slab)[i];
-#pragma unroll
-      for (int u = 0; u < kSlabBatch; ++u)
-        if (zb + u < z1) { v.x += a[u].x; v.y += a[u].y; v.z += a[u].z; v.w += a[u].w; }
-    }
-    const float vv[4] = {v.x, v.y, v.z, v.w};
-    if (opt) {
-      if (Creal == C) {
-        float4 pv = reinterpret_cast<float4*>(sg.p)[i];
-        float4 bv = reinterpret_cast<float4*>(sg.buf)[i];
-        pv.x = sgd_step1(pv.x, v.x, bv.x, sg, lr);
-        pv.y = sgd_step1(pv.y, v.y, bv.y, sg, lr);
-        pv.z = sgd_step1(pv.z, v.z, bv.z, sg, lr);
-        pv.w = sgd_step1(pv.w, v.w, bv.w, sg, lr);
-        reinterpret_cast<float4*>(sg.p)[i] = pv;
-        reinterpret_cast<float4*>(sg.buf)[i] = bv;
-        uint2 pk;
-        pk.x = (unsigned)f2bf(pv.x) | ((unsigned)f2bf(pv.y) << 16);
-        pk.y = (unsigned)f2bf(pv.z) | ((unsigned)f2bf(pv.w) << 16);
-        *reinterpret_cast<uint2*>(sg.wc + i * 4) = pk;
-      } else {
-        const size_t e = i * 4;
-        const int c = (int)(e % C);
-        const size_t krs = e / C;
-#pragma unroll
-        for (int t = 0; t < 4; ++t) {
-          if (c + t >= Creal) continue;
-          const size_t mi = krs * Creal + c + t;
-          float b = sg.buf[mi];
-          const float np = sgd_step1(sg.p[mi], vv[t], b, sg, lr);
-          sg.p[mi] = np;
-          sg.buf[mi] = b;
-          sg.wc[e + t] = f2bf(np);
-        }
-      }
-      continue;
-    }
-    if (Creal == C) {
-      if (single) {
-        float4* o = reinterpret_cast<float4*>(dw) + i;
-        float4 d = *o;
-        d.x += v.x; d.y += v.y; d.z += v.z; d.w += v.w;
-        *o = d;
-      } else {
-#pragma unroll
-        for (int t = 0; t < 4; ++t) unsafeAtomicAdd(dw + i * 4 + t, vv[t]);
-      }
-    } else {
-      const size_t e = i * 4;
-      const int c = (int)(e % C);
-      const size_t krs = e / C;
-#pragma unroll
-      for (int t = 0; t < 4; ++t) {
-        if (c + t >= Creal) continue;
-        if (single) dw[krs * Creal + c + t] += vv[t];
-        else unsafeAtomicAdd(dw + krs * Creal + c + t, vv[t]);
-      }
-    }
-  }
-}
-
 __global__ __launch_bounds__(256) void wgrad_finish_krsc_kernel(const float* __restrict__ ws,
                                                                 int splits, int K, int RS, int C,
                                                                 int Creal, float* __restrict__ dw,
@@ -1700,14 +1616,6 @@
   wgrad_finish_krsc_body(ws, splits, K, RS, C, Creal, dw, blockIdx.x, blockIdx.y, gridDim.x,
                          gridDim.y, sg);
 }
-
-struct WgFinishArgs {
-  const float* ws;
-  int splits, K, RS, C, Creal;
-  float* dw;
-  int gx, gy;
-  SgdFuse sgd;
-};
 
 template <bool BNF>
 __global__ __launch_bounds__(256) void bwd_pair_finish_kernel(FinishArgs fa, int dgx, int dgy,
@@ -1929,6 +1837,56 @@
   if (it == g_sgd_reg.end()) return SgdFuse{};
   g_sgd_taken.insert(dw);
   return it->second;
+}
+
+static bool g_finish_defer = false;
+static PendingFinish g_finish_pending;
+static long long g_finish_stats[3] = {0, 0, 0};
+
+static void launch_wgrad_finish_krsc(const WgFinishArgs& w, hipStream_t st) {
+  hipLaunchKernelGGL(wgrad_finish_krsc_kernel, dim3(w.gx, w.gy), dim3(256), 0, st, w.ws, w.splits,
+                     w.K, w.RS, w.C, w.Creal, w.dw, w.sgd);
+}
+
+extern "C" void ddp_conv_finish_flush() {
+  if (g_finish_pending.kind == kFinishNone) return;
+  const PendingFinish f = g_finish_pending;
+  g_finish_pending = PendingFinish{};
+  ++g_finish_stats[2];
+  if (f.kind == kFinishKrsc) launch_wgrad_finish_krsc(f.wa, f.st);
+  else l0::finish_launch(f.l0, f.st);
+}
+extern "C" void ddp_conv_finish_defer(int on) {
+  g_finish_defer = on != 0;
+  if (!g_finish_defer) ddp_conv_finish_flush();
+}
+extern "C" uintptr_t ddp_conv_finish_pending() {
+  const PendingFinish& f = g_finish_pending;
+  return reinterpret_cast<uintptr_t>(f.kind == kFinishKrsc ? f.wa.dw
+                                     : f.kind == kFinishL0 ? f.l0.dw : nullptr);
+}
+extern "C" void ddp_conv_finish_stats(long long out[3]) {
+  for (int i = 0; i < 3; ++i) out[i] = g_finish_stats[i];
+}
+
+namespace ddp_amd {
+bool finish_defer_on() { return g_finish_defer; }
+void finish_park(const PendingFinish& f) {
+  ddp_conv_finish_flush();
+  g_finish_pending = f;
+  ++g_finish_stats[0];
+}
+bool finish_take(hipStream_t st, int kinds, PendingFinish* out) {
+  if (g_finish_pending.kind == kFinishNone) return false;
+  if (g_finish_pending.st != st || !(g_finish_pending.kind & kinds)) {
+    ddp_conv_finish_flush();
+    return false;
+  }
+  *out = g_finish_pending;
+  g_finish_pending = PendingFinish{};
+  ++g_finish_stats[1];
+  return true;
+}
 }
 
 static WgFinishArgs wg_finish_args(const ConvArgs& a) {
@@ -2024,8 +1982,15 @@
   if (!needs_finish(MODE, a)) return;
   if (MODE == MODE_WGRAD && a.g.wkrsc) {
     const WgFinishArgs w = wg_finish_args(a);
-    hipLaunchKernelGGL(wgrad_finish_krsc_kernel, dim3(w.gx, w.gy), dim3(256), 0, st, a.ws,
-                       a.splits, a.g.K, a.g.R * a.g.S, a.g.C, a.g.Creal, a.dw, w.sgd);
+    if (g_finish_defer && w.gy == 1 && w.sgd.p != nullptr) {
+      PendingFinish f;
+      f.kind = kFinishKrsc;
+      f.wa = w;
+      f.st = st;
+      finish_park(f);
+      return;
+    }
+    launch_wgrad_finish_krsc(w, st);
   } else if (MODE == MODE_WGRAD) {
     const int groups = (a.splits + kWgFinishGroup - 1) / kWgFinishGroup;
     const size_t lds = sizeof(float) * a.g.R * a.g.S * a.g.C;
@@ -2245,6 +2210,7 @@
 extern "C" int ddp_conv_fwd(const ConvGeom* g, const void* x, const void* wc, const float* bias,
                             void* y, float* stats, float* ws, size_t ws_elems, int splits,
                             hipStream_t st) {
+  ddp_conv_finish_flush();
   if (g->C % 8 || g->K % 8) return -1;
   {
     const int r = conv_fwd_dense(g, x, wc, bias, y, stats, ws, ws_elems, nullptr, nullptr, st);
@@ -2291,6 +2257,7 @@
 extern "C" int ddp_conv_fwd_bn(const ConvGeom* g, const void* x, const void* wc, const float* bias,
                                void* z, float* stats, float* ws, size_t ws_elems,
                                const BnFwdFuse* bn, hipStream_t st) {
+  ddp_conv_finish_flush();
   constexpr bool enabled = true;
   if (g->C % 8 || g->K % 8) return -1;
   int done = 0;
@@ -2350,6 +2317,7 @@
                            const BnBwdFuse* bn, const BnBwdApply* ba, int* bn_done,
                            hipStream_t st, const void* acc_dy = nullptr,
                            const unsigned char* acc_mask = nullptr) {
+  ddp_conv_finish_flush();
   if (bn_done) *bn_done = 0;
   if (g->C % 8 || g->K % 8) return -1;
   if (bn && bn->code) return -3;
@@ -2466,6 +2434,7 @@
 
 extern "C" int ddp_conv_wgrad(const ConvGeom* g, const void* dy, const void* x, float* dw,
                               float* ws, size_t ws_elems, int splits, hipStream_t st) {
+  ddp_conv_finish_flush();
   if (g->C % 8 || g->K % 8) return -1;
   ConvArgs a{};
   a.g = *g;
@@ -2529,6 +2498,7 @@
                                  const void* x, float* dw, float* ws, size_t ws_elems,
                                  const BnBwdFuse* bn, const BnBwdApply* ba, int* bn_done,
                                  hipStream_t st) {
+  ddp_conv_finish_flush();
   if (bn_done) *bn_done = 0;
   if (!bn) ba = nullptr;
   auto separate = [&]() -> int {
diff --git a/distributed-data-parallel-ml-training_amd/csrc/kernels/conv_l0.hip b/distributed-data-parallel-ml-training_amd/csrc/kernels/conv_l0.hip
--- a/distributed-data-parallel-ml-training_amd/csrc/kernels/conv_l0.hip
+++ b/distributed-data-parallel-ml-training_amd/csrc/kernels/conv_l0.hip
@@ -1,5 +1,6 @@
 #include "common.h"
 #include "api.h"
+#include "finish_colaunch.h"
 
 #include <algorithm>
 
@@ -277,8 +278,8 @@
   });
 }
 
-__global__ __launch_bounds__(256) void l0_sums_kernel(Args a, int windows) {
-  __shared__ float red[256][33];
+__device__ __forceinline__ void l0_sums_body(const Args& a, int windows, float (*red)[33],
+                                             unsigned bx, unsigned gx) {
   const int tid = threadIdx.x, g = tid & 3;
   float mu[kNT][4], is[kNT][4], s1[kNT][4] = {}, s2[kNT][4] = {};
 #pragma unroll
@@ -289,7 +290,7 @@
       mu[j][v] = a.coef[2 * kK + c];
       is[j][v] = a.coef[3 * kK + c];
     }
-  for (int w = blockIdx.x * 64 + (tid >> 2); w < windows; w += gridDim.x * 64) {
+  for (int w = bx * 64 + (tid >> 2); w < windows; w += gx * 64) {
     const uint4 cq = *reinterpret_cast<const uint4*>(a.code + (size_t)w * (kK / 4) + g * 4);
     const unsigned cw[kNT] = {cq.x, cq.y, cq.z, cq.w};
     u16x4 dv[kNT], zv[kNT];
@@ -320,13 +321,24 @@
     const int gg = (c & 15) >> 2, e = k * 16 + (c >> 4) * 4 + (c & 3);
     float t = 0.f;
     for (int i = 0; i < 64; ++i) t += red[4 * i + gg][e];
-    atomicAdd(a.sums + stat_rep(blockIdx.x) * 2 * kK + k * kK + c, stat_val(t, blockIdx.x));
-  }
+    atomicAdd(a.sums + stat_rep(bx) * 2 * kK + k * kK + c, stat_val(t, bx));
+  }
+}
+
+__global__ __launch_bounds__(256) void l0_sums_kernel(Args a, int windows) {
+  __shared__ float red[256][33];
+  l0_sums_body(a, windows, red, blockIdx.x, gridDim.x);
+}
+
+__global__ __launch_bounds__(256) void l0_sums_co_kernel(Args a, int windows, unsigned ns,
+                                                         WgFinishArgs wa) {
+  __shared__ float red[256][33];
+  if (blockIdx.x < ns) l0_sums_body(a, windows, red, blockIdx.x, ns);
+  else wgrad_finish_krsc_co(wa, (int)(blockIdx.x - ns));
 }
 
 typedef short v4i16 __attribute__((ext_vector_type(4)));
-constexpr int kWgN = 28;
-constexpr int kWgSlab = kK * kWgN;
+static_assert(kWgSlab == kK * kWgN, "one [kK][kWgN] partial per block");
 struct alignas(16) WgStage {
   unsigned short xp[4 * 10][4];
 };
@@ -476,54 +488,16 @@
   l0_bwd_body<2>(a);
 }
 
-constexpr int kWgBatch = 8;
 __global__ __launch_bounds__(256) void l0_wgrad_finish_kernel(const float* __restrict__ ws,
                                                               int nslab, float* __restrict__ dw,
                                                               int wkrsc, SgdFuse sg) {
   __shared__ float4 red[64][4];
-  const bool opt = sg.p != nullptr;
-  const float lr = opt ? sched_lr_block(sg.sched, sg.lr) : sg.lr;
-  const int e = threadIdx.x & 3, s0 = threadIdx.x >> 2;
-  const int i4 = blockIdx.x * 4 + e;
-  float4 v = make_float4(0.f, 0.f, 0.f, 0.f);
-  for (int z = s0; z < nslab; z += 64 * kWgBatch) {
-    float4 t[kWgBatch];
-#pragma unroll
-    for (int u = 0; u < kWgBatch; ++u)
-      if (z + 64 * u < nslab)
-        t[u] = reinterpret_cast<const float4*>(ws + (size_t)(z + 64 * u) * kWgSlab)[i4];
-#pragma unroll
-    for (int u = 0; u < kWgBatch; ++u)
-      if (z + 64 * u < nslab) { v.x += t[u].x; v.y += t[u].y; v.z += t[u].z; v.w += t[u].w; }
-  }
-  red[s0][e] = v;
-  for (int h = 32; h >= 1; h >>= 1) {
-    __syncthreads();
-    if (s0 < h) {
-      const float4 o = red[s0 + h][e];
-      v.x += o.x; v.y += o.y; v.z += o.z; v.w += o.w;
-      red[s0][e] = v;
-    }
-  }
-  if (s0 != 0) return;
-  const float vv[4] = {v.x, v.y, v.z, v.w};
-#pragma unroll
-  for (int t = 0; t < 4; ++t) {
-    const int idx = i4 * 4 + t, k = idx / kWgN, n = idx - k * kWgN;
-    if (n >= 27) continue;
-    const int tap = n / 3, c = n - tap * 3;
-    if (opt) {
-      const int mi = k * 27 + n;
-      float b = sg.buf[mi];
-      const float np = sgd_update1(sg.p[mi], vv[t], b, lr, sg.momentum, sg.wd, sg.grad_scale,
-                                   sg.nesterov);
-      sg.p[mi] = np;
-      sg.buf[mi] = b;
-      sg.wc[(k * 9 + tap) * 8 + c] = f2bf(np);
-    } else {
-      dw[wkrsc ? k * 27 + n : (k * 3 + c) * 9 + tap] += vv[t];
-    }
-  }
+  wgrad_finish_body(ws, nslab, dw, wkrsc, sg, red, blockIdx.x);
+}
+
+void finish_launch(const FinishArgs& f, hipStream_t st) {
+  hipLaunchKernelGGL(l0_wgrad_finish_kernel, dim3(kWgFinishBlocks), dim3(256), 0, st, f.ws,
+                     f.nslab, f.dw, f.wkrsc, f.sg);
 }
 
 static unsigned grid_for(int tiles) {
@@ -592,17 +566,32 @@
   if (fused && (g->Creal != 3 || !io->ws || io->ws_elems < (size_t)nb * l0::kWgSlab)) return -2;
   const int windows = g->N * (g->H / 2) * (g->W / 2);
   const unsigned ns = (unsigned)std::max(1, std::min(512, (windows + 127) / 128));
-  if (!io->sums_ready)
-    hipLaunchKernelGGL(l0::l0_sums_kernel, dim3(ns), dim3(256), 0, st, a, windows);
+  if (!io->sums_ready) {
+    PendingFinish pf;
+    if (finish_take(st, kFinishKrsc, &pf))
+      hipLaunchKernelGGL(l0::l0_sums_co_kernel, dim3(ns + pf.wa.gx), dim3(256), 0, st, a, windows,
+                         ns, pf.wa);
+    else
+      hipLaunchKernelGGL(l0::l0_sums_kernel, dim3(ns), dim3(256), 0, st, a, windows);
+  }
   if (!fused) {
     hipLaunchKernelGGL(l0::l0_bwd_kernel<1>, dim3(nb), dim3(256), 0, st, a);
     return (int)hipGetLastError();
   }
   a.wg = io->ws;
+  ddp_conv_finish_flush();
   hipLaunchKernelGGL(l0::l0_bwd_kernel<2>, dim3(nb), dim3(256), 0, st, a);
   SgdFuse sg{};
   if (g->wkrsc) ddp_sgd_fuse_take_final(io->dw, &sg);
-  hipLaunchKernelGGL(l0::l0_wgrad_finish_kernel, dim3(l0::kWgSlab / 16), dim3(256), 0, st,
-                     (const float*)io->ws, (int)nb, io->dw, g->wkrsc, sg);
+  const l0::FinishArgs fa{(const float*)io->ws, (int)nb, io->dw, g->wkrsc, sg};
+  if (finish_defer_on() && sg.p != nullptr) {
+    PendingFinish f;
+    f.kind = kFinishL0;
+    f.l0 = fa;
+    f.st = st;
+    finish_park(f);
+  } else {
+    l0::finish_launch(fa, st);
+  }
   return (int)hipGetLastError();
 }
diff --git a/distributed-data-parallel-ml-training_amd/csrc/kernels/conv_tr.hip b/distributed-data-parallel-ml-training_amd/csrc/kernels/conv_tr.hip
--- a/distributed-data-parallel-ml-training_amd/csrc/kernels/conv_tr.hip
+++ b/distributed-data-parallel-ml-training_amd/csrc/kernels/conv_tr.hip
@@ -682,6 +682,7 @@
   a.stamps = g_conv_stamps;
 #endif
   const int items = a.tiles_m * a.tiles_n * pl.splits;
+  ddp_conv_finish_flush();
   if (!launch_stages(c, in_mode, a, geo.nl, items, st)) return 0;
   int e = (int)hipGetLastError();
   if (e) return 2 + e;
diff --git a/distributed-data-parallel-ml-training_amd/csrc/kernels/finish_colaunch.h b/distributed-data-parallel-ml-training_amd/csrc/kernels/finish_colaunch.h
--- /dev/null
+++ b/distributed-data-parallel-ml-training_amd/csrc/kernels/finish_colaunch.h
@@ -0,0 +1,185 @@
+#pragma once
+#include "common.h"
+#include "api.h"
+
+namespace ddp_amd {
+
+constexpr int kSlabBatch = 8;
+
+__device__ __forceinline__ float sgd_step1(float p, float g, float& b, const SgdFuse& h,
+                                           float lr) {
+  return sgd_update1(p, g, b, lr, h.momentum, h.wd, h.grad_scale, h.nesterov);
+}
+
+constexpr int kWgFinishGroupKrsc = kDeterministic ? (1 << 30) : 16;
+__device__ __forceinline__ void wgrad_finish_krsc_body(const float* __restrict__ ws, int splits,
+                                                       int K, int RS, int C, int Creal,
+                                                       float* __restrict__ dw, int bx, int by,
+                                                       int gx, int gy, const SgdFuse& sg) {
+  const size_t slab = (size_t)K * RS * C;
+  const size_t n4 = slab / 4;
+  const int z0 = by * kWgFinishGroupKrsc, z1 = min(splits, z0 + kWgFinishGroupKrsc);
+  const bool single = gy == 1;
+  const bool opt = single && sg.p != nullptr;
+  const float lr = opt ? sched_lr_block(sg.sched, sg.lr) : sg.lr;
+  for (size_t i = bx * (size_t)blockDim.x + threadIdx.x; i < n4;
+       i += (size_t)gx * blockDim.x) {
+    float4 v = reinterpret_cast<const float4*>(ws + z0 * slab)[i];
+    for (int zb = z0 + 1; zb < z1; zb += kSlabBatch) {
+      float4 a[kSlabBatch];
+#pragma unroll
+      for (int u = 0; u < kSlabBatch; ++u)
+        if (zb + u < z1) a[u] = reinterpret_cast<const float4*>(ws + (size_t)(zb + u) * slab)[i];
+#pragma unroll
+      for (int u = 0; u < kSlabBatch; ++u)
+        if (zb + u < z1) { v.x += a[u].x; v.y += a[u].y; v.z += a[u].z; v.w += a[u].w; }
+    }
+    const float vv[4] = {v.x, v.y, v.z, v.w};
+    if (opt) {
+      if (Creal == C) {
+        float4 pv = reinterpret_cast<float4*>(sg.p)[i];
+        float4 bv = reinterpret_cast<float4*>(sg.buf)[i];
+        pv.x = sgd_step1(pv.x, v.x, bv.x, sg, lr);
+        pv.y = sgd_step1(pv.y, v.y, bv.y, sg, lr);
+        pv.z = sgd_step1(pv.z, v.z, bv.z, sg, lr);
+        pv.w = sgd_step1(pv.w, v.w, bv.w, sg, lr);
+        reinterpret_cast<float4*>(sg.p)[i] = pv;
+        reinterpret_cast<float4*>(sg.buf)[i] = bv;
+        uint2 pk;
+        pk.x = (unsigned)f2bf(pv.x) | ((unsigned)f2bf(pv.y) << 16);
+        pk.y = (unsigned)f2bf(pv.z) | ((unsigned)f2bf(pv.w) << 16);
+        *reinterpret_cast<uint2*>(sg.wc + i * 4) = pk;
+      } else {
+        const size_t e = i * 4;
+        const int c = (int)(e % C);
+        const size_t krs = e / C;
+#pragma unroll
+        for (int t = 0; t < 4; ++t) {
+          if (c + t >= Creal) continue;
+          const size_t mi = krs * Creal + c + t;
+          float b = sg.buf[mi];
+          const float np = sgd_step1(sg.p[mi], vv[t], b, sg, lr);
+          sg.p[mi] = np;
+          sg.buf[mi] = b;
+          sg.wc[e + t] = f2bf(np);
+        }
+      }
+      continue;
+    }
+    if (Creal == C) {
+      if (single) {
+        float4* o = reinterpret_cast<float4*>(dw) + i;
+        float4 d = *o;
+        d.x += v.x; d.y += v.y; d.z += v.z; d.w += v.w;
+        *o = d;
+      } else {
+#pragma unroll
+        for (int t = 0; t < 4; ++t) unsafeAtomicAdd(dw + i * 4 + t, vv[t]);
+      }
+    } else {
+      const size_t e = i * 4;
+      const int c = (int)(e % C);
+      const size_t krs = e / C;
+#pragma unroll
+      for (int t = 0; t < 4; ++t) {
+        if (c + t >= Creal) continue;
+        if (single) dw[krs * Creal + c + t] += vv[t];
+        else unsafeAtomicAdd(dw + krs * Creal + c + t, vv[t]);
+      }
+    }
+  }
+}
+
+struct WgFinishArgs {
+  const float* ws;
+  int splits, K, RS, C, Creal;
+  float* dw;
+  int gx, gy;
+  SgdFuse sgd;
+};
+
+__device__ __forceinline__ void wgrad_finish_krsc_co(const WgFinishArgs& wa, int bx) {
+  wgrad_finish_krsc_body(wa.ws, wa.splits, wa.K, wa.RS, wa.C, wa.Creal, wa.dw, bx, 0, wa.gx, 1,
+                         wa.sgd);
+}
+
+namespace l0 {
+
+constexpr int kWgN = 28;
+constexpr int kWgSlab = 64 * kWgN;
+constexpr int kWgBatch = 8;
+constexpr int kWgFinishBlocks = kWgSlab / 16;
+
+struct FinishArgs {
+  const float* ws;
+  int nslab;
+  float* dw;
+  int wkrsc;
+  SgdFuse sg;
+};
+
+__device__ __forceinline__ void wgrad_finish_body(const float* __restrict__ ws, int nslab,
+                                                  float* __restrict__ dw, int wkrsc,
+                                                  const SgdFuse& sg, float4 (*red)[4],
+                                                  unsigned bx) {
+  const bool opt = sg.p != nullptr;
+  const float lr = opt ? sched_lr_block(sg.sched, sg.lr) : sg.lr;
+  const int e = threadIdx.x & 3, s0 = threadIdx.x >> 2;
+  const int i4 = bx * 4 + e;
+  float4 v = make_float4(0.f, 0.f, 0.f, 0.f);
+  for (int z = s0; z < nslab; z += 64 * kWgBatch) {
+    float4 t[kWgBatch];
+#pragma unroll
+    for (int u = 0; u < kWgBatch; ++u)
+      if (z + 64 * u < nslab)
+        t[u] = reinterpret_cast<const float4*>(ws + (size_t)(z + 64 * u) * kWgSlab)[i4];
+#pragma unroll
+    for (int u = 0; u < kWgBatch; ++u)
+      if (z + 64 * u < nslab) { v.x += t[u].x; v.y += t[u].y; v.z += t[u].z; v.w += t[u].w; }
+  }
+  red[s0][e] = v;
+  for (int h = 32; h >= 1; h >>= 1) {
+    __syncthreads();
+    if (s0 < h) {
+      const float4 o = red[s0 + h][e];
+      v.x += o.x; v.y += o.y; v.z += o.z; v.w += o.w;
+      red[s0][e] = v;
+    }
+  }
+  if (s0 != 0) return;
+  const float vv[4] = {v.x, v.y, v.z, v.w};
+#pragma unroll
+  for (int t = 0; t < 4; ++t) {
+    const int idx = i4 * 4 + t, k = idx / kWgN, n = idx - k * kWgN;
+    if (n >= 27) continue;
+    const int tap = n / 3, c = n - tap * 3;
+    if (opt) {
+      const int mi = k * 27 + n;
+      float b = sg.buf[mi];
+      const float np = sgd_update1(sg.p[mi], vv[t], b, lr, sg.momentum, sg.wd, sg.grad_scale,
+                                   sg.nesterov);
+      sg.p[mi] = np;
+      sg.buf[mi] = b;
+      sg.wc[(k * 9 + tap) * 8 + c] = f2bf(np);
+    } else {
+      dw[wkrsc ? k * 27 + n : (k * 3 + c) * 9 + tap] += vv[t];
+    }
+  }
+}
+
+void finish_launch(const FinishArgs& f, hipStream_t st);
+
+}
+
+enum : int { kFinishNone = 0, kFinishKrsc = 1, kFinishL0 = 2 };
+struct PendingFinish {
+  int kind = kFinishNone;
+  WgFinishArgs wa{};
+  l0::FinishArgs l0{};
+  hipStream_t st = nullptr;
+};
+bool finish_defer_on();
+void finish_park(const PendingFinish& f);
+bool finish_take(hipStream_t st, int kinds, PendingFinish* out);
+
+}
diff --git a/distributed-data-parallel-ml-training_amd/csrc/kernels/optim.hip b/distributed-data-parallel-ml-training_amd/csrc/kernels/optim.hip
--- a/distributed-data-parallel-ml-training_amd/csrc/kernels/optim.hip
+++ b/distributed-data-parallel-ml-training_amd/csrc/kernels/optim.hip
@@ -1,5 +1,6 @@
 #include "common.h"
 #include "api.h"
+#include "finish_colaunch.h"
 
 namespace ddp_amd {
 
@@ -149,7 +150,7 @@
 __device__ void sgd_pack_body(const int4* __restrict__ items, const long long* __restrict__ descs,
                               float* __restrict__ p, float* __restrict__ g,
                               float* __restrict__ buf, const SgdHyper& h, float* tile,
-                              float trust, GuardState gd = GuardState{});
+                              float trust, unsigned bx, GuardState gd = GuardState{});
 
 __global__ __launch_bounds__(256) void sgd_pack_kernel(const int4* __restrict__ items,
                                                        const long long* __restrict__ descs,
@@ -159,8 +160,25 @@
   __shared__ float tile[kTileElems];
   h.lr = sched_lr_block(h.sched, h.lr);
   if (h.sched_advance && blockIdx.x == 0 && threadIdx.x == 0) sched_stage(h.sched);
-  sgd_pack_body<false>(items, descs, p, g, buf, h, tile, 1.f);
+  sgd_pack_body<false>(items, descs, p, g, buf, h, tile, 1.f, blockIdx.x);
   if (h.signal && last_block_done(h.done)) signal_flag(h.done, h.signal);
+}
+
+__global__ __launch_bounds__(256) void sgd_pack_co_kernel(const int4* __restrict__ items,
+                                                          const long long* __restrict__ descs,
+                                                          float* __restrict__ p,
+                                                          float* __restrict__ g,
+                                                          float* __restrict__ buf, SgdHyper h,
+                                                          unsigned n_items, l0::FinishArgs fa) {
+  __shared__ __attribute__((aligned(16))) float tile[kTileElems];
+  if (blockIdx.x >= n_items) {
+    l0::wgrad_finish_body(fa.ws, fa.nslab, fa.dw, fa.wkrsc, fa.sg,
+                          reinterpret_cast<float4(*)[4]>(tile), blockIdx.x - n_items);
+    return;
+  }
+  h.lr = sched_lr_block(h.sched, h.lr);
+  if (h.sched_advance && blockIdx.x == 0 && threadIdx.x == 0) sched_stage(h.sched);
+  sgd_pack_body<false>(items, descs, p, g, buf, h, tile, 1.f, blockIdx.x);
 }
 
 struct LarsArgs {
@@ -260,7 +278,7 @@
   h.lr = sched_lr_block(h.sched, h.lr);
   if (h.sched_advance && blockIdx.x == 0 && threadIdx.x == 0) sched_stage(h.sched);
   const float trust = lars_trust_block(la, h.wd);
-  sgd_pack_body<true>(items, descs, p, g, buf, h, tile, trust);
+  sgd_pack_body<true>(items, descs, p, g, buf, h, tile, trust, blockIdx.x);
   if (h.signal && last_block_done(h.done)) signal_flag(h.done, h.signal);
 }
 
@@ -372,13 +390,13 @@
 __device__ void sgd_pack_body(const int4* __restrict__ items, const long long* __restrict__ descs,
                               float* __restrict__ p, float* __restrict__ g,
                               float* __restrict__ buf, const SgdHyper& h, float* tile,
-                              float trust, GuardState gd) {
-  const int4 it = items[blockIdx.x];
+                              float trust, unsigned bx, GuardState gd) {
+  const int4 it = items[bx];
   const int tid = threadIdx.x;
-  if (h.counter && blockIdx.x == 0 && tid == 0) atomicAdd(h.counter, h.delta);
+  if (h.counter && bx == 0 && tid == 0) atomicAdd(h.counter, h.delta);
   if (block_skip(h.skip)) return;
   if constexpr (GUARD) {
-    if (blockIdx.x == 0 && tid == 0) {
+    if (bx == 0 && tid == 0) {
       gd.stats[0] = gd.norm;
       gd.stats[1] = gd.c;
       if (gd.skipped && gd.count) {
@@ -551,7 +569,7 @@
   if (h.sched_advance && blockIdx.x == 0 && threadIdx.x == 0) sched_stage(h.sched);
   const GuardState gd = clip_block(ca);
   h.grad_scale *= gd.c;
-  sgd_pack_body<false, true>(items, descs, p, g, buf, h, tile, 1.f, gd);
+  sgd_pack_body<false, true>(items, descs, p, g, buf, h, tile, 1.f, blockIdx.x, gd);
   if (h.signal && last_block_done(h.done)) signal_flag(h.done, h.signal);
 }
 
@@ -567,7 +585,7 @@
   const GuardState gd = clip_block(ca);
   const float trust = gd.skipped ? 1.f : lars_trust_block<true>(la, h.wd, gd.c);
   h.grad_scale *= gd.c;
-  sgd_pack_body<true, true>(items, descs, p, g, buf, h, tile, trust, gd);
+  sgd_pack_body<true, true>(items, descs, p, g, buf, h, tile, trust, blockIdx.x, gd);
   if (h.signal && last_block_done(h.done)) signal_flag(h.done, h.signal);
 }
 
@@ -664,11 +682,21 @@
                             const void* lars_partial, float* lars_trust, float lars_eta,
                             float lars_eps, const float* clip_partial, int clip_chunks,
                             float clip_max_norm, float clip_eps, int clip_flags,
-                            float* clip_stats, hipStream_t st) {
+                            float* clip_stats, int finish_colaunch, hipStream_t st) {
   SgdHyper h{lr, momentum, wd, grad_scale, nesterov, zero_grad, counter, delta, skip, shadow, slot,
              done, signal, sched, sched && sched_advance ? 1 : 0};
-  if (n_items <= 0) return 0;
+  if (n_items <= 0) {
+    ddp_conv_finish_flush();
+    return 0;
+  }
   if (clip_partial && (!clip_stats || clip_chunks < 0)) return -1;
+  PendingFinish pf;
+  const bool plain = !lars_side && !clip_partial && !signal && finish_colaunch;
+  if (finish_take(st, plain ? kFinishL0 : 0, &pf)) {
+    hipLaunchKernelGGL(sgd_pack_co_kernel, dim3(n_items + l0::kWgFinishBlocks), dim3(256), 0, st,
+                       (const int4*)items, descs, p, g, buf, h, (unsigned)n_items, pf.l0);
+    return (int)hipGetLastError();
+  }
   ClipArgs ca{clip_partial, clip_chunks, clip_max_norm, clip_eps, clip_flags, clip_stats};
   if (lars_side) {
     if (!lars_tensors || !lars_partial || !lars_trust) return -1;
diff --git a/distributed-data-parallel-ml-training_amd/ops/common.py b/distributed-data-parallel-ml-training_amd/ops/common.py
--- a/distributed-data-parallel-ml-training_amd/ops/common.py
+++ b/distributed-data-parallel-ml-training_amd/ops/common.py
@@ -7,6 +7,7 @@
 _NATIVE = None
 CONV_STAGES = 2
 BWD_PAIR_MODE, BWD_PAIR_ITEMS = 3, 1024
+FINISH_COLAUNCH = True
 
 
 def native():
diff --git a/distributed-data-parallel-ml-training_amd/optim/sgd.py b/distributed-data-parallel-ml-training_amd/optim/sgd.py
--- a/distributed-data-parallel-ml-training_amd/optim/sgd.py
+++ b/distributed-data-parallel-ml-training_amd/optim/sgd.py
@@ -237,9 +237,9 @@
             raise RuntimeError("gradient clipping / non-finite step skipping cannot run in the "
                                "backward: the norm exists only once the whole gradient does "
                                "(TrainStep keeps opt_in_bwd False)")
-        from ..ops.common import native
+        from ..ops import common
         a, g = self.arena, self.param_groups[0]
-        nat = native()
+        nat = common.native()
         nat.sgd_fuse_register(0, clear=1)
         self._bwd_index = {}
         base_g, base_p = a.grad.data_ptr(), a.data.data_ptr()
@@ -258,10 +258,18 @@
                                   **sched)
             self._bwd_index[dw] = i
         nat.sgd_fuse_begin()
+        nat.conv_finish_defer(int(bool(common.FINISH_COLAUNCH)))
 
     def unregister_in_backward(self):
         from ..ops.common import native
+        native().conv_finish_defer(0)
         native().sgd_fuse_register(0, clear=1)
+
+    def _finish_colaunch(self, exclude, pack_only):
+        from ..ops.common import native
+        dw = native().conv_finish_pending()
+        i = getattr(self, "_bwd_index", {}).get(dw) if dw else None
+        return int(i is not None and i in exclude and i not in pack_only)
 
     def _fused_in_backward(self):
         from ..ops.common import native
@@ -456,6 +464,7 @@
         if self.guarded and not norm_done:
             self.grad_sumsq(params, stream)
         if n_items == 0:
+            native().conv_finish_flush()
             if sched.get("sched_advance"):
                 native().counter_add(int(counter[0]) if counter else 0,
                                      int(counter[1]) if counter else 0, s,
@@ -466,8 +475,9 @@
             if signal:
                 native().flag_signal(int(signal[1]), s)
             return None
+        co = {"finish_colaunch": 1} if self._finish_colaunch(exclude, pack_only) else {}
         self._update_launch(items, n_items, s, descs=descs, zero_grad=zero_grad, counter=counter,
-                            skip=skip, signal=signal, lr_advance=lr_advance)
+                            skip=skip, signal=signal, lr_advance=lr_advance, **co)
         return None
 
     def state_dict(self):
```

Measured after the change: 381,200 images/s (median of 3 runs). No clear change (+0.4%).
